# jhuggins/viabel

Hardware: AMD Instinct MI355X
Metric: ELBO-gradient evals/sec (D=1024, N_mc=4096) (higher is better)
Workload: dtype f64

## Files before the change

include/viabel_hip.h:

```cpp
#ifndef VIABEL_HIP_H
#define VIABEL_HIP_H

#include <stddef.h>
#include <stdint.h>

#ifdef __cplusplus
extern "C" {
#endif

typedef struct vb_ctx vb_ctx;

#define VB_OK 0
#define VB_ERR_INVALID 1
#define VB_ERR_HIP 2
#define VB_ERR_UNSUPPORTED 3
#define VB_ERR_STATE 4
#define VB_ERR_NUMERIC 5
#define VB_ERR_COMM 6
#define VB_ERR_CALLBACK 7

#define VB_FAMILY_MF_GAUSSIAN 0
#define VB_FAMILY_MF_STUDENT_T 1
#define VB_FAMILY_FULLRANK_GAUSSIAN 2
#define VB_FAMILY_MULTIVARIATE_T 3
#define VB_FAMILY_LOWRANK_GAUSSIAN 4

#define VB_MODEL_GAUSS_DIAG 0
#define VB_MODEL_FUNNEL 1
#define VB_MODEL_GAUSS_FULL 2
#define VB_MODEL_LOGISTIC 3

#define VB_MODEL_SOURCE 4
#define VB_MODEL_SOFTMAX 5
#define VB_MODEL_MULTILEVEL 6
#define VB_MODEL_LOCSCALE 7
#define VB_MODEL_SPARSE_GLM 8
#define VB_MODEL_MINIBATCH_GLM 9
#define VB_MODEL_NEURALNET 10
#define VB_LOCSCALE_GAUSSIAN 0
#define VB_LOCSCALE_STUDENT_T 1

#define VB_GLM_BERNOULLI_LOGIT 0
#define VB_GLM_POISSON 1
#define VB_GLM_GAUSSIAN 2

#define VB_NOISE_NORMAL 0
#define VB_NOISE_STUDENT_T 1

#define VB_FLAG_PATH_DERIV 1u
#define VB_CV_NONE 0
#define VB_CV_FULL 1
#define VB_CV_MEAN_ONLY 2
#define VB_CV_LOO_DIAG 3
#define VB_CV_LOO_DIRECT 4

#define VB_MAX_SLOTS 64

const char* vb_version(void);
int vb_device_count(int* count);
int vb_create(int device_id, vb_ctx** out);
int vb_destroy(vb_ctx* ctx);
const char* vb_last_error(vb_ctx* ctx);
int vb_device_info(vb_ctx* ctx, char* name, size_t name_len, int* n_cu, uint64_t* hbm_bytes);
int vb_sync(vb_ctx* ctx);

int vb_noise_set_host(vb_ctx* ctx, int slot, const double* host, int64_t n, int64_t d);
int vb_noise_generate(vb_ctx* ctx, int slot, int kind, double df, uint64_t seed,
                      uint64_t stream, int64_t row_offset, int64_t n, int64_t d);
int vb_noise_get_host(vb_ctx* ctx, int slot, double* host, int64_t n, int64_t d);
int vb_noise_moments(vb_ctx* ctx, int slot, int64_t n, int64_t d, double* colsum, double* gram);

int vb_chisq_generate(vb_ctx* ctx, double df, uint64_t seed, uint64_t stream, int64_t row_offset, int64_t n);
int vb_chisq_get_host(vb_ctx* ctx, double* host, int64_t n);
int vb_noise_hint_seed(vb_ctx* ctx, uint64_t slot_mask , int with_chi, uint64_t seed);
int vb_noise_ahead_stats(vb_ctx* ctx, uint64_t* generated, uint64_t* adopted);

int vb_set_model(vb_ctx* ctx, int model_id, int64_t dim, const double* dparams,
                 size_t n_dparams, const int64_t* iparams, size_t n_iparams);
int vb_set_model_source(vb_ctx* ctx, int64_t dim, const char* source, const double* params, size_t n_params);
typedef int (*vb_model_callback)(void* user, const double* z, int64_t n, int64_t d, double* f, double* grad);
int vb_set_model_callback(vb_ctx* ctx, int64_t dim, vb_model_callback fn, void* user);
int vb_model_logp(vb_ctx* ctx, const double* x_host, int64_t n, int64_t d, double* out_host);
int vb_model_grad(vb_ctx* ctx, const double* x_host, int64_t n, int64_t d, double* f_host, double* g_host);

int vb_elbo_grad_meanfield(vb_ctx* ctx, int slot, int64_t n, int64_t d, int64_t n_total,
                           int family, double df, const double* theta, unsigned flags,
                           int cv_mode, double* value, double* grad);
int vb_elbo_grad_meanfield_philox(vb_ctx* ctx, int slot, int64_t n, int64_t d, int64_t n_total, int64_t row_offset,
                                  int family, double df, const double* theta, unsigned flags, int cv_mode,
                                  uint64_t seed, uint64_t stream, double* value, double* grad);
int vb_elbo_grad_meanfield_async(vb_ctx* ctx, int slot, int64_t n, int64_t d, int64_t n_total,
                                 int family, double df, const double* theta, unsigned flags,
                                 int cv_mode, int rslot);
int vb_elbo_grad_meanfield_batch_async(vb_ctx* ctx, int count, const int* slots, int64_t n, int64_t d,
                                       int64_t n_total, int family, double df, const double* thetas,
                                       unsigned flags, int cv_mode, const int* rslots);
int vb_result_get(vb_ctx* ctx, int rslot, double* value, double* grad, int64_t p);

int vb_alpha_grad_meanfield(vb_ctx* ctx, int slot, int64_t n, int64_t d, int64_t n_total, int family, double df,
                            const double* theta, double alpha, double* value, double* grad);

#define VB_PRIOR_DIAG_GAUSSIAN 0
#define VB_PRIOR_DIAG_STUDENT_T 1
#define VB_PRIOR_DENSE 2
int vb_dis_set_temper_prior(vb_ctx* ctx, int kind, int64_t d, double df, const double* loc, const double* scale,
                            double log_det_l);
int vb_dis_refresh_meanfield(vb_ctx* ctx, int slot, int64_t n, int64_t d, int64_t n_total, int family, double df,
                             const double* theta, const double* prior_theta, double eps_prev,
                             double ess_target, int max_bisection_its, double* eps, double* ess,
                             double* w, double* log_p, double* log_q);
int vb_dis_grad_meanfield(vb_ctx* ctx, int slot, int64_t n, int64_t d, int family, double df,
                          const double* theta, const double* weights, double scale, double* value,
                          double* grad);

int vb_alpha_grad_fullrank(vb_ctx* ctx, int slot, int64_t n, int64_t d, int64_t n_total, const double* theta,
                           double alpha, double* value, double* grad);
int vb_alpha_grad_mvt_chol(vb_ctx* ctx, int slot, int64_t n, int64_t d, int64_t n_total, double df, const double* theta,
                           double alpha, double* value, double* grad);

int vb_dis_refresh_mvt(vb_ctx* ctx, int slot, int64_t n, int64_t d, int64_t n_total, double df, const double* theta,
                       const double* chi, const double* sqrt_sigma, const double* l_inv,
                       const double* prior_theta, double eps_prev, double ess_target, int max_bisection_its,
                       double* eps, double* ess, double* w, double* log_p, double* log_q);
int vb_elbo_grad_mvt_symroot(vb_ctx* ctx, int slot, int64_t n, int64_t d, int64_t n_total, double df, const double* theta,
                             double* value, double* grad, double* info);
int vb_elbo_grad_mvt_symroot_path(vb_ctx* ctx, int slot, int64_t n, int64_t d, int64_t n_total, double df,
                                  const double* theta, double* value, double* grad, double* info);
int vb_alpha_grad_mvt_symroot(vb_ctx* ctx, int slot, int64_t n, int64_t d, int64_t n_total, double df, double alpha,
                              const double* theta, double* value, double* grad, double* info);

int vb_dis_refresh_mvt_symroot(vb_ctx* ctx, int slot, int64_t n, int64_t d, int64_t n_total, double df, const double* theta,
                               const double* prior_theta, double eps_prev, double ess_target, int max_bisection_its,
                               double* root_info);
int vb_dis_grad_mvt_packed(vb_ctx* ctx, int64_t n, int64_t d, double df, const double* theta, const double* weights,
                           double scale, double* value, double* grad);
int vb_dis_step_mvt_packed(vb_ctx* ctx, int64_t n, int64_t d, double df, const double* theta, int64_t resample_m,
                           uint64_t seed, uint64_t stream, double scale, double* eps, double* ess,
                           double* khat , double* value, double* grad);
int vb_dis_psis_mvt(vb_ctx* ctx, int64_t n_total, double reff);
int vb_dis_clip_mvt(vb_ctx* ctx, int64_t n_total, double threshold);
int vb_dis_weights_get(vb_ctx* ctx, double* w, int64_t n_total, int resampled );
int vb_dis_scalars_get(vb_ctx* ctx, double out[4]);
int vb_host_alloc(size_t bytes, void** ptr);
int vb_host_free(void* ptr);
int vb_resource_counts(uint64_t out[4]);
int vb_dis_generation(vb_ctx* ctx, int kind, uint64_t* generation);
int vb_dis_state_park(vb_ctx* ctx, int kind, int slot, void** handle);
int vb_dis_state_unpark(vb_ctx* ctx, void* handle);
int vb_dis_state_drop(void* handle);
int vb_dis_state_get(vb_ctx* ctx, int dense, double* log_p, double* log_q, int64_t n_total);
int vb_dis_grad_mvt(vb_ctx* ctx, int64_t n, int64_t d, double df, const double* theta, const double* l_inv,
                    const double* weights, double* w_sum, double* w_logq, double* d_mu, double* gram);

int vb_elbo_grad_lowrank(vb_ctx* ctx, int slot_eps, int slot_z, int64_t n, int64_t d, int64_t k,
                         int64_t n_total, const double* theta, unsigned flags, double* value,
                         double* grad);

int vb_elbo_sums_lowrank(vb_ctx* ctx, int slot_eps, int slot_z, int64_t n, int64_t d, int64_t k, const double* theta,
                         double* out);

typedef struct vb_flow vb_flow;
int vb_flow_create(vb_ctx* ctx, int64_t d, int64_t k, const double* masks, int64_t n_t, const int64_t* widths_t,
                   int64_t n_s, const int64_t* widths_s, vb_flow** out);
int vb_flow_destroy(vb_ctx* ctx, vb_flow* flow);
int vb_flow_param_dim(vb_ctx* ctx, const vb_flow* flow, int64_t* p);
int vb_flow_elbo_grad(vb_ctx* ctx, vb_flow* flow, int slot, int64_t n, int64_t n_total, int prior_family,
                      double prior_df, const double* prior_param, const double* theta, unsigned flags, double* out);
int vb_flow_sample(vb_ctx* ctx, vb_flow* flow, int slot, int64_t n, int prior_family, double prior_df,
                   const double* prior_param, const double* theta, double* x, double* log_q, double* log_p);
int vb_flow_fit(vb_ctx* ctx, vb_flow* flow, int slot, int64_t n, int64_t n_total, int64_t row_offset, int prior_family,
                double prior_df, const double* prior_param, unsigned flags, int noise_kind, double noise_df, uint64_t seed,
                uint64_t first_stream, int opt_kind, const double hyper[4], int64_t n_iters, double* theta, double* state,
                int has_state, double* values, double* history, int64_t hist_len, double* directions, double* gradients);

int vb_log_weights_meanfield(vb_ctx* ctx, int slot, int64_t n, int64_t d, int family, double df,
                             const double* theta, double* lw);
int vb_psis_smooth(vb_ctx* ctx, const double* lw_in, int64_t n, double reff, double* lw_out,
                   double* khat);

int vb_psis_smooth_batch(vb_ctx* ctx, const double* lw, int64_t n, int64_t m, int64_t ld, double reff,
                         double* out, double* khat);
int vb_glm_pointwise(vb_ctx* ctx, const double* x, int64_t s, int64_t d, double* ll_out);
int vb_softmax_pointwise(vb_ctx* ctx, const double* x, int64_t s, int64_t d, double* ll_out);
int vb_multilevel_pointwise(vb_ctx* ctx, const double* x, int64_t s, int64_t d, double* ll_out);
int vb_locscale_pointwise(vb_ctx* ctx, const double* x, int64_t s, int64_t d, double* ll_out);
int vb_sparse_glm_pointwise(vb_ctx* ctx, const double* x, int64_t s, int64_t d, double* ll_out);
int vb_minibatch_pointwise(vb_ctx* ctx, const double* x, int64_t s, int64_t d, double* ll_out);
int vb_minibatch_set_batch(vb_ctx* ctx, int64_t t);
int vb_minibatch_get_batch(vb_ctx* ctx, int64_t* t);
int vb_minibatch_indices(vb_ctx* ctx, int64_t t, int64_t* out);
int vb_glm_psis_loo(vb_ctx* ctx, const double* x, int64_t s, int64_t d, const double* log_ratios,
                    const double* log_w, double reff, double* loo, double* khat, double* lpd);
int vb_glm_predict(vb_ctx* ctx, const double* x, int64_t s, int64_t d, const double* log_w, const double* x_new,
                   int64_t m, const double* y_new, double* mean, double* var, double* eta_mean, double* eta_var,
                   double* lpd);
int vb_nn_pointwise(vb_ctx* ctx, const double* x, int64_t s, int64_t d, double* ll_out);
int vb_nn_predict(vb_ctx* ctx, const double* x, int64_t s, int64_t d, const double* log_w, const double* x_new, int64_t m,
                  const double* y_new, double* mean, double* var, double* eta_mean, double* eta_var, double* lpd);
int vb_glm_value_grad_hessian(vb_ctx* ctx, const double* x, int64_t d, double* f, double* grad, double* hess);

int vb_ksd(vb_ctx* ctx, const double* x, int64_t s, int64_t d, const double* scores, const double* log_w,
           const double* scale, double c, double beta, double* ksd2, double* rowsums);
int vb_ksd_plan(int64_t s, int n_cu, int out[2]);

int vb_svgd_direction(vb_ctx* ctx, const double* x, int64_t n, int64_t d, const double* scores, const double* scale,
                      double bandwidth, double* phi, double* logp, double* h_used);
int vb_svgd_run(vb_ctx* ctx, const double* x0, int64_t n, int64_t d, const double* scale, double bandwidth, int opt_kind,
                const double hyper[4], int64_t n_iters, double* state, int has_state, double* x, double* logp,
                double* h_hist, double* rms_hist, double* logp_hist);

int vb_hmc_run(vb_ctx* ctx, const double* x0, const double* inv_mass, int64_t n_chains, int64_t d, int64_t n_warmup,
               int64_t n_draws, int64_t thin, int n_leapfrog, double step_size, double target_accept, double jitter,
               uint64_t seed, uint64_t stream_offset, double* draws, double* logp, double* last_x, double* chain_mean,
               double* chain_m2, double* accept_rate, double* step_hist, double* accept_hist, double* final_step,
               int64_t* n_divergent);

#define VB_HMC_METRIC_DIAG 0
#define VB_HMC_METRIC_DENSE 1
int vb_hmc_run_metric(vb_ctx* ctx, const double* x0, int metric_kind, const double* metric, int64_t n_chains, int64_t d,
                      int64_t n_warmup, int64_t n_draws, int64_t thin, int n_leapfrog, double step_size, double target_accept,
                      double jitter, uint64_t seed, uint64_t stream_offset, const double* moment_shift, double* moment_sum,
                      double* moment_m2, double* draws, double* logp, double* last_x, double* chain_mean, double* chain_m2,
                      double* accept_rate, double* step_hist, double* accept_hist, double* final_step, int64_t* n_divergent);

int vb_hmc_run_chees(vb_ctx* ctx, const double* x0, int metric_kind, const double* metric, int64_t n_chains, int64_t d,
                     int64_t n_warmup, int64_t n_draws, int64_t thin, int max_leapfrog, double trajectory_lr, double step_size,
                     double target_accept, double jitter, uint64_t seed, uint64_t stream_offset, const double* moment_shift,
                     double* moment_sum, double* moment_m2, double* draws, double* logp, double* last_x, double* chain_mean,
                     double* chain_m2, double* accept_rate, double* step_hist, double* accept_hist, double* final_step,
                     int64_t* n_divergent, double* traj_state, double* traj_hist, int64_t* leap_hist);

int vb_elbo_sums_mvt(vb_ctx* ctx, int slot, int64_t n, int64_t d, int64_t n_total, const double* mu,
                     const double* sqrt_sigma, const double* inv_s, double* f_sum, double* g_sum,
                     double* c_full);

int vb_elbo_grad_fullrank(vb_ctx* ctx, int slot, int64_t n, int64_t d, int64_t n_total,
                          const double* theta, unsigned flags, double* value, double* grad);
int vb_fullrank_set_theta(vb_ctx* ctx, const double* theta, int64_t d);
int vb_elbo_grad_fullrank_enqueue(vb_ctx* ctx, int slot, int64_t n, int64_t d, int64_t n_total,
                                  unsigned flags);
int vb_fullrank_get(vb_ctx* ctx, double* value, double* grad, int64_t p);
int vb_fullrank_fold_get_m(vb_ctx* ctx, double* M_host, int64_t d);
int vb_fold_m_team_plan(int d, int pair, int* out8);

int vb_elbo_grad_mvt_chol(vb_ctx* ctx, int slot, int64_t n, int64_t d, int64_t n_total, double df, const double* theta,
                          double* value, double* grad);

int vb_sym_sqrt(vb_ctx* ctx, const double* a, const double* e, int64_t d, double* root, double* x, double* info);
int vb_sym_sqrt_inv(vb_ctx* ctx, const double* a, const double* e, int64_t d, double* root, double* x, double* info,
                    double* inv_root);

int vb_lowrank_path_terms(vb_ctx* ctx, int slot_eps, int slot_z, int64_t n, int64_t d, int64_t k, int64_t n_total,
                          const double* sw, double* out);

int vb_mvt_path_terms(vb_ctx* ctx, int slot, int64_t n, int64_t d, int64_t n_total, double df, const double* inv_s,
                      double* m_w, double* e_w, double* log1p_sum);

int vb_alpha_sums_mvt(vb_ctx* ctx, int slot, int64_t n, int64_t d, int64_t n_total, double df, double alpha,
                      const double* mu, const double* sqrt_sigma, const double* inv_s, double sum_log_diag,
                      double* value, double* w_sum, double* g_sum, double* c_full);

#define VB_OPT_SGD 0
#define VB_OPT_RMSPROP 1
#define VB_OPT_ADAM 2
#define VB_OPT_ADAGRAD 3
int vb_fit(vb_ctx* ctx, int slot, int slot_aux, int64_t n, int64_t d, int64_t n_total, int64_t row_offset, int family,
           double df, unsigned flags, int cv_mode, int noise_kind, double noise_df, uint64_t seed,
           uint64_t first_stream, int opt_kind, const double hyper[4], int64_t n_iters, double* theta, int64_t p,
           double* state, int has_state, double* values, double* history, int64_t hist_len, double* directions,
           double* gradients);
int vb_fit_history_mean(vb_ctx* ctx, int64_t rows, int64_t p, double* mean);

int vb_chain_open(vb_ctx* ctx, int64_t p, int64_t capacity_rows);
int vb_chain_close(vb_ctx* ctx);
int vb_chain_rows(vb_ctx* ctx, int64_t* rows);
int vb_chain_append(vb_ctx* ctx, const double* rows_host, int64_t n_rows);
int vb_chain_fetch(vb_ctx* ctx, int64_t first_row, int64_t n_rows, double* out);
int vb_chain_mean(vb_ctx* ctx, int64_t w, double* mean);
int vb_chain_rhat(vb_ctx* ctx, const int64_t* windows, int n_windows, double jitter, double* max_rhat, double* rhat);
int vb_chain_ess_mcse(vb_ctx* ctx, int64_t w, double* ess, double* mcse);
int vb_mvt_route_stats(vb_ctx* ctx, uint64_t* epilogue_rows, uint64_t* chain_fetch);

int vb_dis_refresh_lowrank(vb_ctx* ctx, int slot_eps, int slot_z, int64_t n, int64_t d, int64_t k, int64_t n_total,
                           const double* mu, const double* log_sigma, const double* b, const double* m_inv,
                           double log_q_const, const double* prior_theta, double eps_prev, double ess_target,
                           int max_bisection_its, double* eps, double* ess, double* w, double* log_p, double* log_q);
int vb_dis_grad_lowrank(vb_ctx* ctx, int64_t n, int64_t d, int64_t k, const double* mu, const double* log_sigma,
                        const double* b, const double* m_inv, double log_q_const, const double* weights, double* out);
int vb_alpha_sums_lowrank(vb_ctx* ctx, int slot_eps, int slot_z, int64_t n, int64_t d, int64_t k, int64_t n_total,
                          double alpha, const double* mu, const double* log_sigma, const double* b, const double* m_inv,
                          double log_q_const, double* value, double* w_sum, double* out);

#define VB_COMM_ID_BYTES 128
int vb_comm_unique_id(char id[VB_COMM_ID_BYTES]);
int vb_comm_init(vb_ctx* ctx, const char id[VB_COMM_ID_BYTES], int n_ranks, int rank);
int vb_comm_destroy(vb_ctx* ctx);
int vb_comm_info(vb_ctx* ctx, int* n_ranks, int* rank);
#define VB_HOST_SUM 0
#define VB_HOST_MAX 1
typedef int (*vb_host_collective_fn)(void* user, double* buf, size_t count, int op);
int vb_comm_init_host(vb_ctx* ctx, vb_host_collective_fn fn, void* user, int n_ranks, int rank);
#define VB_IPC_HANDLE_BYTES 64
int vb_comm_ipc_window(vb_ctx* ctx, size_t cap_doubles, char handle[VB_IPC_HANDLE_BYTES]);
int vb_comm_init_ipc(vb_ctx* ctx, const char* handles, int n_ranks, int rank);
int vb_comm_check(vb_ctx* ctx);
int vb_comm_allreduce_time(vb_ctx* ctx, size_t count, int warm, int reps, double* us_per_collective);

typedef struct vb_legacy_rng vb_legacy_rng;
int vb_legacy_rng_create(uint32_t seed, vb_legacy_rng** out);
void vb_legacy_rng_destroy(vb_legacy_rng* rng);
int vb_legacy_rng_randn(vb_legacy_rng* rng, double* out, int64_t n, int threads);
int vb_legacy_rng_standard_t(vb_legacy_rng* rng, double df, double* out, int64_t n);
int vb_legacy_rng_chisquare(vb_legacy_rng* rng, double df, double* out, int64_t n);
int vb_legacy_rng_random_sample(vb_legacy_rng* rng, double* out, int64_t n);
int vb_legacy_rng_get_state(const vb_legacy_rng* rng, uint32_t key[624], int* pos, int* has_gauss, double* gauss);
int vb_legacy_rng_set_state(vb_legacy_rng* rng, const uint32_t key[624], int pos, int has_gauss, double gauss);
int vb_legacy_rng_randn_device(vb_ctx* ctx, vb_legacy_rng* rng, int slot, int64_t n_total, int64_t d, int64_t row_begin,
                               int64_t rows);
int vb_legacy_rng_standard_t_device(vb_ctx* ctx, vb_legacy_rng* rng, double df, int slot, int64_t n_total, int64_t d,
                                    int64_t row_begin, int64_t rows);
int vb_legacy_rng_chisquare_device(vb_ctx* ctx, vb_legacy_rng* rng, double df, int64_t n, double* host_out);
int vb_legacy_round_end(vb_ctx* ctx, vb_legacy_rng* rng);
int vb_legacy_ahead_stats(vb_ctx* ctx, uint64_t* launched, uint64_t* adopted, uint64_t* discarded);
int vb_legacy_rng_log_proven(void);
uint64_t vb_legacy_rng_uid(const vb_legacy_rng* rng);

#define VB_PROF_MF_ACCUM 0
#define VB_PROF_FR_SAMPLE_GEMM 1
#define VB_PROF_FR_MODEL_GEMM 2
#define VB_PROF_FR_GRAD_GEMM 3
#define VB_PROF_NUM 4

#define VB_FR_FOLD_MIN_D 1024
#define VB_FR_FOLD_MIN_ROWS_PER_D 3
int vb_profile_enable(vb_ctx* ctx, int on);
int vb_profile_read(vb_ctx* ctx, int64_t* launches, int64_t* evals, double* total_ms, int reset);
int vb_profile_read_kernel(vb_ctx* ctx, int kernel_id, int64_t* launches, int64_t* evals, double* total_ms,
                           int reset);

#ifdef __cplusplus
}
#endif
#endif
```

viabel_amd/csrc/vb_common.h:

```cpp
#pragma once

#include <hip/hip_runtime.h>
#include <hip/hip_ext.h>

#include <cstdarg>
#include <cstdint>
#include <cstdio>
#include <cstring>
#include <functional>
#include <memory>
#include <string>
#include <vector>

#include "../../include/viabel_hip.h"
#include "vb_resource.h"

namespace vb {

constexpr int kWave = 64;
constexpr int kMfThreads = 256;
constexpr int kMfWaves = kMfThreads / kWave;
constexpr int kMfCols = 128;
constexpr int kMfChunk = 16;
constexpr int kMaxBatch = 32;
constexpr int kModelLogQ = 99;

template <int BYTES>
__device__ __forceinline__ void kernarg_warm() {
#if defined(__HIP_DEVICE_COMPILE__)
  typedef const uint32_t __attribute__((address_space(4))) * KernargPtr;
  KernargPtr p = (KernargPtr)__builtin_amdgcn_kernarg_segment_ptr();
  uint32_t t = 0;
#pragma unroll
  for (int off = 0; off < BYTES; off += 64) asm volatile("s_load_dword %0, %1, %2" : "+s"(t) : "s"(p), "s"(off));
  asm volatile("s_waitcnt lgkmcnt(0)" : "+s"(t));
#endif
}

enum ColField { CF_G = 0, CF_GE, CF_E, CF_EE, CF_EK, CF_SC, CF_SCE, CF_NUM };

__host__ __device__ __forceinline__ int64_t partial_index(int64_t rb, int f, int64_t col, int64_t n_rb) {
  return (((col >> 6) * n_rb + rb) * CF_NUM + f) * 64 + (col & 63);
}
enum ScalField { SF_F = 0, SF_W, SF_Q, SF_QE, SF_L1P, SF_EE, SF_FK, SF_GK, SF_GEK, SF_NUM = 12 };
enum KScal { KS_F = 0, KS_Q, KS_QE, KS_L1P, KS_EE, KS_NUM };
enum PScal { PS_W = 0, PS_FK, PS_GK, PS_GEK, PS_NUM };

struct ModelDev {
  int id = -1;
  int dim = 0;
  int k = 0;
  double tau = 1.0;
  double c0 = 0.0;
  const double* p0 = nullptr;
  const double* p1 = nullptr;
  int64_t ldp = 0;
  const double* p2 = nullptr;
  int64_t ldq = 0;
  int64_t n_data = 0;
  int link = 0;
  double aux = 1.0;
  int n_classes = 0;
  int n_feat = 0;
  double f0 = 0.0;
  int n_groups = 0;
  double hyper_sd = 1.0;
  const int* grp_off = nullptr;
  const int* grp_of = nullptr;
  const double* w0 = nullptr;
  const double* w1 = nullptr;
  int64_t ldw = 0;
  int n_scale = 0;
  int const_scale = 0;
  double scale_sd = 1.0;
  double df = 0.0;
  const double* sp_val[2] = {nullptr, nullptr};
  const int* sp_ptr[2] = {nullptr, nullptr};
  const int* sp_idx[2] = {nullptr, nullptr};
  const int* sp_seg[2] = {nullptr, nullptr};
  const int* sp_split[2] = {nullptr, nullptr};
  int sp_n_seg[2] = {0, 0};
  int sp_n_split[2] = {0, 0};
  int64_t nnz = 0;
  int64_t mb_size = 0;
  int mb_shuffle = 0;
  int mb_half_bits = 0;
  uint64_t mb_seed = 0;
  int n_hidden = 0;
};

__host__ __device__ __forceinline__ bool model_has_rows(int id) {
  return id == VB_MODEL_SOURCE || id == VB_MODEL_SOFTMAX || id == VB_MODEL_MULTILEVEL || id == VB_MODEL_LOCSCALE ||
         id == VB_MODEL_SPARSE_GLM || id == VB_MODEL_MINIBATCH_GLM || id == VB_MODEL_NEURALNET;
}

__device__ __forceinline__ double glm_term(int link, double aux, double y, double eta, double* dl) {
  if (link == VB_GLM_POISSON) {
    const double mu = exp(eta);
    *dl = y - mu;
    return y * eta - mu;
  }
  if (link == VB_GLM_GAUSSIAN) {
    const double r = (y - eta) / (aux * aux);
    *dl = r;
    return -0.5 * r * (y - eta);
  }
  const double t = exp(-fabs(eta));
  const double p = eta >= 0.0 ? 1.0 / (1.0 + t) : t / (1.0 + t);
  *dl = y - p;
  return y * eta - (fmax(eta, 0.0) + log1p(t));
}

__device__ __forceinline__ double glm_predict_term(int link, double aux, double y, double eta, double* mu, double* var) {
  if (link == VB_GLM_POISSON) {
    const double m = exp(eta);
    *mu = m;
    *var = m;
    return y * eta - m;
  }
  if (link == VB_GLM_GAUSSIAN) {
    const double r = (y - eta) / (aux * aux);
    *mu = eta;
    *var = aux * aux;
    return -0.5 * r * (y - eta);
  }
  const double t = exp(-fabs(eta));
  const double q = 1.0 / (1.0 + t);
  *mu = eta >= 0.0 ? q : t * q;
  *var = t * q * q;
  return y * eta - (fmax(eta, 0.0) + log1p(t));
}

struct NoiseReq {
  int kind = 0;
  double df = 0.0;
  uint64_t seed = 0, stream = 0;
  int64_t row_offset = 0, n = 0, d = 0;
  bool valid = false;
};
struct NoiseAhead {
  DeviceBuffer shadow;
  DeviceBuffer shadow_norms;
  bool pre_norms = false;
  int64_t shadow_d = 0, shadow_ld = 0;
  NoiseReq last, pre;
  NoiseReq hint;
  int64_t delta = 0;
  int streak = 0;
};
struct NoiseSlot {
  DeviceBuffer buf;
  int64_t n = 0, d = 0, ld = 0;
  NoiseAhead ahead;
  DeviceBuffer norms;
  NoiseReq norms_req;
  bool want_norms = false;
};
const double* noise_row_norms(vb_ctx* ctx, NoiseSlot& s, hipStream_t st);
int rng_row_norms(vb_ctx* ctx, hipStream_t st, const double* src, int64_t ld, int64_t n, int64_t d, double* norms);

constexpr int kPipeSets = 4;
struct Pipeline {
  Stream post;
  Event ev_k1[kPipeSets], ev_fin[kPipeSets];
  bool fin_valid[kPipeSets] = {};
  uint64_t seq = 0;
  int last_set = 0;
  bool post_pending = false;
};

struct ResultSlot {
  PinnedBuffer pin;
  double* host() const { return pin.host_as<double>(); }
  double* dev() const { return pin.dev_as<double>(); }
  int64_t p = 0;
  bool pending = false;
  uint64_t batch_id = 0;
};

}

namespace vb {
struct LegacySpec;
struct LegacySpecDelete { void operator()(LegacySpec* s) const; };
}

struct vb_ctx {
  int device = 0;
  vb::Stream stream;
  hipDeviceProp_t prop;
  std::string last_error;

  vb::NoiseSlot noise[VB_MAX_SLOTS];
  vb::NoiseSlot gen_geom;
  vb::ResultSlot results[VB_MAX_SLOTS];
  vb::ResultSlot sync_result;
  vb::PinnedBuffer done_pin;
  unsigned long long done_seq = 0;
  int done_groups = 0;

  vb::ModelDev model;
  vb::DeviceBuffer model_params;
  std::vector<double> model_host;

  vb::DeviceBuffer theta;
  vb::DeviceBuffer workspace;
  vb::DeviceBuffer sums;
  vb::DeviceBuffer mf_one;
  unsigned mf_one_epoch = 0;
  vb::DeviceBuffer out;
  vb::DeviceBuffer scratch;
  vb::DeviceBuffer scratch2;
  vb::DeviceBuffer rowvec;
  vb::DeviceBuffer fr_work;
  vb::DeviceBuffer lg_work;
  hipModule_t user_module = nullptr;
  hipFunction_t user_fn = nullptr;
  struct UserModule {
    uint64_t hash;
    hipModule_t module;
    hipFunction_t fn;
    int parts;
  };
  int user_parts = 1;
  vb_model_callback user_host_fn = nullptr;
  void* user_host_arg = nullptr;
  vb::PinnedBuffer user_host_pin;
  std::vector<UserModule> user_modules;
  vb::DeviceBuffer user_params;
  vb::DeviceBuffer glm_work;
  vb::DeviceBuffer target_work;
  int64_t mb_batch = 0, mb_held = -1;
  const void* mb_held_at = nullptr;
  size_t mb_held_bytes = 0;
  vb::DeviceBuffer hess_work;
  vb::DeviceBuffer hmc_work;
  vb::DeviceBuffer mvt_state;
  int64_t mvt_n = 0, mvt_d = 0, mvt_n_total = 0;
  int64_t mvt_lq_off = 0;
  vb::DeviceBuffer mvt_ekl_state;
  std::vector<double> mvt_theta;
  bool mvt_dev_factors = false;
  const double* mvt_e_noise = nullptr;
  int64_t mvt_e_noise_ld = 0;
  std::vector<double> mvt_stage;
  vb::PinnedBuffer mvt_pin;
  size_t mvt_pin_doubles = 0;
  int mvt_pin_slot = 0;
  vb::Event mvt_pin_ev[2];
  vb::PinnedBuffer push_pin;
  size_t push_bytes = 0;
  int push_slot = 0;
  vb::Event push_ev[2];
  vb::PinnedBuffer fetch_pin;
  unsigned long long fetch_seq = 0;
  vb::DeviceBuffer fetch_ticket;
  vb::Stream mvt_side;
  hipEvent_t mvt_ev_fork = nullptr;
  vb::Event mvt_ev_join;
  vb::Event done_ev;
  uint64_t ahead_generated = 0, ahead_adopted = 0;
  bool mvt_inv_pending = false;
  bool mvt_inv_queued = false;
  struct {
    double* base = nullptr;
    int64_t o_theta = 0, o_lt = 0, o_wt = 0, o_tscr = 0, o_mu = 0, o_li = 0, o_lfull = 0, o_c = 0, ld = 0;
    int d = 0;
    bool clean = false;
    bool lfull_here = false;
  } mvt_inv_args;
  std::vector<double> mvt_prior;
  int64_t mvt_inv_key[4] = {0, 0, 0, 0};
  vb::DeviceBuffer dis_state;
  int64_t dis_n = 0, dis_d = 0;
  int64_t dis_n_total = 0;
  vb::DeviceBuffer chi_dev;
  vb::DeviceBuffer mvt_invs;
  vb::NoiseAhead chi_ahead;
  int64_t chi_n = 0;
  double chi_df = 0.0;
  vb::DeviceBuffer bisect_work;
  unsigned long long bisect_bar_base = 0;
  size_t bisect_bar_words = 0;
  void* bisect_bar_ptr = nullptr;
  vb::DeviceBuffer mvt_elbo;
  vb::DeviceBuffer lr_work;
  vb::DeviceBuffer lr_obj;
  std::vector<vb_flow*> flows;
  int64_t lr_n = 0, lr_d = 0, lr_k = 0, lr_n_total = 0;
  struct TemperPrior {
    int kind = 0;
    int64_t d = 0, ld = 0;
    double df = 0.0, c0 = 0.0;
    vb::DeviceBuffer buf;
    vb::DeviceBuffer work;
  } temper;
  uint64_t dis_gen[3] = {0, 0, 0};
  vb::DeviceBuffer rows_work;
  vb::DeviceBuffer psis_lw;
  int64_t psis_n = 0;
  vb::DeviceBuffer psis_work;
  unsigned long long psis_bar_base = 0;
  vb::DeviceBuffer loo_work;
  vb::DeviceBuffer ksd_work;
  vb::DeviceBuffer svgd_work;
  vb::PinnedBuffer pin;
  vb::DeviceBuffer fit_work;
  int64_t fit_out_off = 0;
  uint64_t mvt_epi_rows_calls = 0, mvt_chain_fetch_calls = 0;
  int ns_hint_m[2] = {0, 0}, ns_hint_steps[2] = {0, 0};
  int64_t fit_hist_off = 0, fit_hist_len = 0, fit_hist_p = 0;
  vb::DeviceBuffer chain;
  vb::DeviceBuffer chain_work;
  int64_t chain_p = 0, chain_cap = 0, chain_rows = 0;
  bool chain_open = false;
  static constexpr int kFitRing = 4;
  vb::Stream fit_copy_st;
  vb::PinnedBuffer fit_ring;
  size_t fit_ring_doubles = 0;
  vb::Event fit_ev_step[kFitRing], fit_ev_copy[kFitRing];
  vb::DeviceBuffer tri_map;
  int tri_map_key[3] = {0, 0, 0};
  int tri_map_blocks = 0;
  vb::DeviceBuffer fr_lt;
  int64_t fr_lt_d = 0;
  const double* fr_lt_owner = nullptr;
  vb::DeviceBuffer fr_theta;
  vb::DeviceBuffer fr_out;
  int64_t fr_p = 0;
  const double* fr_fold_m = nullptr;
  int64_t fr_fold_d = 0, fr_fold_ld = 0;
  vb::DeviceBuffer alpha_g;
  vb::DeviceBuffer legacy_work;
  const void* legacy_poly_at = nullptr;
  size_t legacy_poly_bytes = 0;
  bool legacy_table_ready = false;
  std::unique_ptr<vb::LegacySpec, vb::LegacySpecDelete> legacy_spec;
  vb::PinnedBuffer legacy_pin;
  vb::DeviceBuffer fz_words, fz_items;
  int64_t fz_key[5] = {0, 0, 0, 0, 0};
  int fz_n_items = 0;
  unsigned fz_epoch = 0;
  int fr_fused_mode = -1;
  uint64_t fr_seq = 0;

  void* comm = nullptr;
  int n_ranks = 1, rank = 0;
  vb_host_collective_fn host_fn = nullptr;
  void* host_user = nullptr;
  vb::PinnedBuffer host_stage;
  struct IpcComm {
    double* win[16] = {};
    size_t cap = 0;
    unsigned long long seq = 0;
    unsigned* ticket = nullptr;
    unsigned* err_host = nullptr;
    unsigned* err_dev = nullptr;
    int poll_log2 = 32;
    double timeout_s = 20.0;
    bool on = false;
  } ipc;

  bool profile = false;
  struct ProfLog {
    std::vector<std::pair<vb::Event, vb::Event>> events;
    size_t used = 0;
    int64_t evals = 0;
  } prof[VB_PROF_NUM];

  std::vector<vb::Event> batch_events;
  uint64_t batch_id = 0, batch_done = 0;

  vb::Pipeline pipe;
  hipStream_t result_stream = nullptr;
};

namespace vb {

int fail(vb_ctx* ctx, int code, const char* fmt, ...);
int ensure(vb_ctx* ctx, DeviceBuffer& b, size_t bytes);
int ensure_pinned(vb_ctx* ctx, PinnedBuffer& b, size_t bytes, bool mapped);
int ensure_pinned(vb_ctx* ctx, size_t bytes);

#define VB_HIP(ctx, expr)                                                              \
  do {                                                                                 \
    hipError_t e__ = (expr);                                                           \
    if (e__ != hipSuccess)                                                             \
      return vb::fail((ctx), VB_ERR_HIP, "%s failed: %s (%s:%d)", #expr,               \
                      hipGetErrorString(e__), __FILE__, __LINE__);                     \
  } while (0)

#define VB_TRY(expr)                   \
  do {                                 \
    int rc__ = (expr);                 \
    if (rc__ != VB_OK) return rc__;    \
  } while (0)

struct MfCall {
  int count = 0;
  const NoiseSlot* noise[kMaxBatch] = {};
  const double* theta_src[kMaxBatch] = {};
  double* out[kMaxBatch] = {};
  const double* roww[kMaxBatch] = {};
  int64_t n = 0, d = 0, n_total = 0;
  int family = 0;
  double df = 0.0;
  unsigned flags = 0;
  int cv_mode = 0;
  int mode = 0;
  bool overlap_comm = false;
  double scale = 0.0;
  const double* value_src = nullptr;
  const ModelDev* model = nullptr;
  int gen = 0;
  uint64_t gen_seed = 0, gen_stream = 0;
  int64_t gen_row_offset = 0;
  const struct FitStep* step = nullptr;
  bool* step_done = nullptr;
  bool prep_next = false, skip_prep = false;
  bool* prep_done = nullptr;
  bool theta_on_device = false;
  unsigned long long* done_dev = nullptr;
  unsigned long long done_seq = 0;
  int* done_groups = nullptr;
};
int mf_enqueue(vb_ctx* ctx, const MfCall& call);
int user_model_set(vb_ctx* ctx, int64_t dim, const char* source, const double* params, size_t n_params);
int user_rows_enqueue(vb_ctx* ctx, hipStream_t st, const double* Z, int64_t ldz, int64_t n, int d, double* G,
                      int64_t ldg, double* f);
void user_model_release(vb_ctx* ctx);
int softmax_rows_enqueue(vb_ctx* ctx, hipStream_t st, const double* Z, int64_t ldz, int64_t n, int d, double* G,
                         int64_t ldg, double* f);
int model_rows_enqueue(vb_ctx* ctx, hipStream_t st, const double* Z, int64_t ldz, int64_t n, int d, double* G,
                       int64_t ldg, double* f);
constexpr int64_t kSoftmaxChunkDoubles = (int64_t)16 << 20;
int multilevel_rows_enqueue(vb_ctx* ctx, hipStream_t st, const double* Z, int64_t ldz, int64_t n, int d, double* G,
                            int64_t ldg, double* f);
constexpr int64_t kMultilevelChunkDoubles = (int64_t)16 << 20;
int locscale_rows_enqueue(vb_ctx* ctx, hipStream_t st, const double* Z, int64_t ldz, int64_t n, int d, double* G,
                          int64_t ldg, double* f);
constexpr int64_t kLocScaleChunkDoubles = (int64_t)16 << 20;
int sparse_rows_enqueue(vb_ctx* ctx, hipStream_t st, const double* Z, int64_t ldz, int64_t n, int d, double* G, int64_t ldg,
                        double* f);
constexpr int kSparseSegment = 256;
constexpr int64_t kSparseChunkDoubles = (int64_t)16 << 20;
inline int64_t sparse_chunk_rows(int64_t n_data, int64_t p) {
  const int64_t rows = kSparseChunkDoubles / (2 * (n_data + p)) / 64 * 64;
  return rows < 64 ? 64 : rows > 8192 ? 8192 : rows;
}
int minibatch_rows_enqueue(vb_ctx* ctx, hipStream_t st, const double* Z, int64_t ldz, int64_t n, int d, double* G, int64_t ldg,
                           double* f);
constexpr int64_t kMinibatchChunkDoubles = (int64_t)16 << 20;
inline int64_t minibatch_chunk_rows(int64_t batch_size) {
  const int64_t rows = kMinibatchChunkDoubles / (2 * ((batch_size + 15) / 16 * 16));
  return rows < 8 ? 8 : rows;
}
int neuralnet_rows_enqueue(vb_ctx* ctx, hipStream_t st, const double* Z, int64_t ldz, int64_t n, int d, double* G, int64_t ldg,
                           double* f);
constexpr int64_t kNeuralNetChunkDoubles = (int64_t)16 << 20;
constexpr int64_t kNeuralNetPredictDoubles = (int64_t)16 << 20;
struct PredictArgs {
  const double* eta;
  int64_t ld;
  int n;
  const double* w;
  const double* log_w;
  const double* y;
  double aux;
  double *mean, *var, *eta_mean, *eta_var, *lpd;
};
int glm_predict_enqueue(vb_ctx* ctx, hipStream_t st, int link, const PredictArgs& a, int64_t rows);
bool predict_weights(const double* log_w, int64_t s, std::vector<double>& out);
struct RowsPointwisePlan {
  int64_t chunk = 0, total = 0;
  int64_t o_x = 0, o_ll = 0, ldl = 0;
  int64_t width = 0;
};
using RowsPointwiseBody = std::function<int(int64_t rows, const double* X, int64_t ldx, double* LL, int64_t ldl)>;
int rows_pointwise(vb_ctx* ctx, const char* api_name, int model_id, const char* target_name, const double* x, int64_t s,
                   int64_t d, double* ll_out, const std::function<int(RowsPointwisePlan*)>& plan,
                   const RowsPointwiseBody& body);
int upload_model_params(vb_ctx* ctx, const std::vector<double>& dev, const double** base);
using SetModelFn = int(vb_ctx* ctx, int64_t dim, const double* dparams, size_t n_dparams, const int64_t* iparams,
                       size_t n_iparams);
SetModelFn softmax_set_model, multilevel_set_model, locscale_set_model, sparse_set_model, minibatch_set_model,
    neuralnet_set_model;
struct LegacyFinish;
int legacy_dev_randn(vb_ctx* ctx, uint32_t key[624], int* pos, int* has_gauss, double* gauss, double* dst, int64_t ld,
                     int64_t n_total, int64_t d, int64_t row_begin, int64_t rows, LegacyFinish* defer = nullptr);
struct FetchSeg {
  const void* src;
  size_t bytes;
  void* dst;
};
struct LegacyWords {
  const uint32_t* words = nullptr;
  int64_t* scal = nullptr;
  uint32_t* extra = nullptr;
  const void* logtab = nullptr;
  int64_t pre = 0, n_words = 0;
  uint32_t* key_io = nullptr;
  int64_t* meta = nullptr;
};
struct LegacyFinish {
  LegacyWords lw;
  const int64_t* src_dev = nullptr;
  int64_t mult = 0, add = 0;
  const void* extra_src[2] = {nullptr, nullptr};
  int extra_words[2] = {0, 0};
  int kind = 0;
  int64_t pairs = 0, n_vals = 0;
  int pos_in = 0;
};
constexpr int kLegacyFinishWords = 352;
int legacy_finish_launch(vb_ctx* ctx, hipStream_t st, const LegacyFinish& f, unsigned long long* landing_dev, unsigned long long seq);
int legacy_finish_complete(vb_ctx* ctx, const LegacyFinish& f, const unsigned long long* landing, uint32_t key[624], int* pos,
                           int* has_gauss, double* gauss);
// ... 253 lines not shown
```

viabel_amd/csrc/vb_fullrank.hip:

```cpp
#include "vb_gemm_f64.h"
#include "vb_fit.h"

namespace vb {

constexpr double kLog2PiFr = 1.8378770664093454835606594728112;

__device__ __forceinline__ double fr_wave_sum(double x) {
#pragma unroll
  for (int off = 32; off > 0; off >>= 1) x += __shfl_down(x, off, 64);
  return x;
}

__device__ __forceinline__ double fr_block_sum(double x, double* sh) {
  x = fr_wave_sum(x);
  const int lane = threadIdx.x & 63, wave = threadIdx.x >> 6;
  __syncthreads();
  if (lane == 0) sh[wave] = x;
  __syncthreads();
  return (sh[0] + sh[1]) + (sh[2] + sh[3]);
}

__global__ void __launch_bounds__(256) fr_unpack_kernel(const double* __restrict__ theta, int d,
                                                        int64_t ldl, double* __restrict__ Lt,
                                                        double* __restrict__ mu, double* __restrict__ copy = nullptr) {
// ... 136 lines not shown

struct EpiNegateF {
  double* G;
  int64_t ldz;
  const double* Zc;
  double* part;
  __device__ double operator()(int, int row, int col, double acc) const {
    G[(int64_t)row * ldz + col] = -acc;
    return -0.5 * acc * Zc[(int64_t)row * ldz + col];
  }
  __device__ d2v pair(int, int row, int col, double a0, double a1) const {
    const d2v z = *reinterpret_cast<const d2v*>(Zc + (int64_t)row * ldz + col);
    *reinterpret_cast<d2v*>(G + (int64_t)row * ldz + col) = (d2v){-a0, -a1};
    return (d2v){-0.5 * a0 * z.x, -0.5 * a1 * z.y};
  }
};

struct EpiSplitSlabCs {
  double* C;
  int64_t ldc, slab;
  double* colsum;
  int64_t colsum_ld;
  __device__ void operator()(int split, int row, int col, double acc) const {
    C[split * slab + (int64_t)row * ldc + col] = acc;
  }
  __device__ d2v pair(int split, int row, int col, double a0, double a1) const {
    const d2v v = (d2v){a0, a1};
    *reinterpret_cast<d2v*>(C + split * slab + (int64_t)row * ldc + col) = v;
    return v;
  }
};

struct EpiFoldSlabF {
  double* C;
  int64_t ldc, slab;
  const double* b;
  const double* s;
  const double* Lt;
  int64_t ldl;
  double* part;
  __device__ double operator()(int split, int row, int col, double acc) const {
    const double v = split == 0 ? -acc - b[row] * s[col] : -acc;
    C[split * slab + (int64_t)row * ldc + col] = v;
    const double l = Lt[(int64_t)col * ldl + row];
    return col <= row ? l * v : 0.0;
  }
  __device__ d2v pair(int split, int row, int col, double a0, double a1) const {
    d2v v = (d2v){-a0, -a1};
    if (split == 0) {
      const double br = b[row];
      const d2v ss = *reinterpret_cast<const d2v*>(s + col);
      v.x -= br * ss.x, v.y -= br * ss.y;
    }
    *reinterpret_cast<d2v*>(C + split * slab + (int64_t)row * ldc + col) = v;
    const double l0 = Lt[(int64_t)col * ldl + row], l1 = Lt[(int64_t)(col + 1) * ldl + row];
    return (d2v){col <= row ? l0 * v.x : 0.0, col + 1 <= row ? l1 * v.y : 0.0};
  }
};

struct EpiSplitSlab {
  double* C;
  int64_t ldc, slab;
  __device__ void operator()(int split, int row, int col, double acc) const {
    C[split * slab + (int64_t)row * ldc + col] = acc;
  }
  __device__ d2v pair(int split, int row, int col, double a0, double a1) const {
    const d2v v = (d2v){a0, a1};
    *reinterpret_cast<d2v*>(C + split * slab + (int64_t)row * ldc + col) = v;
    return v;
  }
};

}
#include "vb_fullrank_fused.h"
namespace vb {

__global__ void __launch_bounds__(256) fr_funnel_kernel(const double* __restrict__ Z, double* __restrict__ G,
                                                        int64_t ldz, int64_t n, int d, ModelDev m,
                                                        double* __restrict__ fpart, const double* __restrict__ roww) {
  __shared__ double sh[4];
  const int lane = threadIdx.x & 63;
  const int64_t row = (int64_t)blockIdx.x * 4 + (threadIdx.x >> 6);
  double f = 0.0;
  if (row < n) {
    const double* z = Z + row * ldz;
    double* g = G + row * ldz;
    const double v = z[m.k];
    const double w = exp(-2.0 * v);
    const double rw = roww ? roww[row] : 1.0;
    double ss = 0.0;
    for (int c = lane; c < d; c += 64) {
      if (c == m.k) continue;
      const double zc = z[c];
      const double gc = -zc * w;
      g[c] = roww ? gc * rw : gc;
      ss = fma(zc, zc, ss);
    }
    ss = fr_wave_sum(ss);
    if (lane == 0) {
      const double it2 = 1.0 / (m.tau * m.tau), dm1 = (double)(d - 1);
      const double gk = fma(-v, it2, -dm1) + w * ss;
      g[m.k] = roww ? gk * rw : gk;
      f = v * fma(-0.5 * v, it2, -dm1) - 0.5 * w * ss;
    }
  }
  f = fr_block_sum(f, sh);
  if (threadIdx.x == 0) fpart[blockIdx.x] = f;
}

typedef double fr_d2 __attribute__((ext_vector_type(2)));
__global__ void __launch_bounds__(256) fr_colsum_kernel(const double* __restrict__ G,
                                                        const double* __restrict__ Zc, int64_t ldz,
                                                        int64_t n, int d, int fmode,
                                                        const double* __restrict__ ivar,
                                                        double* __restrict__ colpart,
                                                        double* __restrict__ fpart, double scal = 0.0,
                                                        const double* __restrict__ roww = nullptr,
                                                        int square = 0, double* __restrict__ Gscaled = nullptr,
                                                        const double* __restrict__ rs_out = nullptr) {
  __shared__ double sh[4];
  __shared__ fr_d2 cs[4][64];
  const int c = threadIdx.x & 63, q = threadIdx.x >> 6;
  const int col = blockIdx.x * 128 + 2 * c;
  const int64_t r0 = (int64_t)blockIdx.y * 128;
  const int64_t r1 = r0 + 128 < n ? r0 + 128 : n;
  const bool ok0 = col < d, ok1 = col + 1 < d;
  fr_d2 s = (fr_d2){0.0, 0.0};
  double f = 0.0;
  if (ok0) {
    fr_d2 hiv = (fr_d2){0.0, 0.0};
    if (fmode == 1) hiv = (fr_d2){-0.5 / ivar[col], ok1 ? -0.5 / ivar[col + 1] : 0.0};
    for (int64_t rb = r0 + q; rb < r1; rb += 64) {
      fr_d2 g[16], z[16];
      double rw[16], rs[16];
#pragma unroll
      for (int i = 0; i < 16; ++i) {
        const int64_t r = rb + 4 * i < r1 ? rb + 4 * i : r1 - 1;
        g[i] = *reinterpret_cast<const fr_d2*>(G + r * ldz + col);
        z[i] = fmode >= 2 ? *reinterpret_cast<const fr_d2*>(Zc + r * ldz + col) : (fr_d2){0.0, 0.0};
        rw[i] = roww ? roww[r] : 1.0;
        rs[i] = Gscaled ? rs_out[r] : 1.0;
      }
#pragma unroll
      for (int i = 0; i < 16; ++i) {
        const int64_t r = rb + 4 * i;
        const bool in = r < r1;
        if (roww) g[i] *= rw[i];
        if (square) g[i] *= g[i];
        if (!in) g[i] = (fr_d2){0.0, 0.0}, z[i] = (fr_d2){0.0, 0.0};
        if (!ok1) g[i].y = 0.0, z[i].y = 0.0;
        if (Gscaled && in) *reinterpret_cast<fr_d2*>(Gscaled + r * ldz + col) = g[i] * rs[i];
        s += g[i];
        if (fmode == 1) f = fma(hiv.x * g[i].x, g[i].x, fma(hiv.y * g[i].y, g[i].y, f));
        if (fmode == 2) f = fma(0.5 * z[i].x, g[i].x, fma(0.5 * z[i].y, g[i].y, f));
        if (fmode == 3) f = fma(-0.5 * scal * z[i].x, z[i].x, fma(-0.5 * scal * z[i].y, z[i].y, f));
      }
    }
  }
  cs[q][c] = s;
  __syncthreads();
  if (q == 0 && ok0) {
    const fr_d2 tot = (cs[0][c] + cs[1][c]) + (cs[2][c] + cs[3][c]);
    colpart[(int64_t)blockIdx.y * ldz + col] = tot.x;
    if (ok1) colpart[(int64_t)blockIdx.y * ldz + col + 1] = tot.y;
  }
  f = fr_block_sum(f, sh);
  if (threadIdx.x == 0) fpart[(int64_t)blockIdx.y * gridDim.x + blockIdx.x] = f;
}


template <int THREADS>
__device__ __forceinline__ void fr_fold_sum_blocks(const int blk, double* fold_lds, const double* __restrict__ Spart, int gsplits,
                                                   int64_t slab, int d, int64_t ldl, const double* __restrict__ colpart,
                                                   int64_t ldz, const double* __restrict__ P, int64_t ldp,
                                                   const double* __restrict__ mu, const double* __restrict__ mean, int nb_b,
                                                   int nb_s, double* __restrict__ S, double* __restrict__ svec,
                                                   double* __restrict__ b) {
  static_assert(THREADS == 256 || THREADS == 512, "256 workers, with or without a second idle half");
  const bool worker = THREADS == 256 || threadIdx.x < 256;
  if (blk < nb_b) {
    fr_d2(*part)[4] = reinterpret_cast<fr_d2(*)[4]>(fold_lds);
    const int p = threadIdx.x & 3, kg = threadIdx.x >> 2;
    const int col = blk * 8 + 2 * p;
    if (worker) {
      const int colc = col < d ? col : 0;
      const int kper = (d + 63) / 64;
      const int k0 = kg * kper, k1 = k0 + kper < d ? k0 + kper : d;
      fr_d2 bacc = (fr_d2){0.0, 0.0};
      for (int kb = k0; kb < k1; kb += 16) {
        fr_d2 v[16];
        double c[16];
#pragma unroll
        for (int u = 0; u < 16; ++u) {
          const int k = kb + u < k1 ? kb + u : k1 - 1;
          v[u] = *reinterpret_cast<const fr_d2*>(P + (int64_t)k * ldp + colc);
          c[u] = mu[k] - mean[k];
        }
#pragma unroll
        for (int u = 0; u < 16; ++u)
          if (kb + u < k1) bacc += v[u] * c[u];
      }
      part[kg][p] = bacc;
    }
    __syncthreads();
    if (worker && kg == 0) {
      fr_d2 btot = part[0][p];
#pragma unroll 16
      for (int q = 1; q < 64; ++q) btot += part[q][p];
      if (col < d) b[col] = btot.x;
      if (col + 1 < d) b[col + 1] = btot.y;
    }
    return;
  }
  if (blk < nb_b + nb_s) {
    const int k = (blk - nb_b) * 256 + (int)threadIdx.x;
    if (!worker || k >= ldz) return;
    double s = 0.0;
    if (k < d) {
      s = colpart[k];
      for (int z = 1; z < gsplits; ++z) s += colpart[(int64_t)z * ldz + k];
    }
    svec[k] = s;
    return;
  }
  int bi = 0, bj = blk - nb_b - nb_s;
  while (bj > bi) bj -= ++bi;
  double(*tile)[33] = reinterpret_cast<double(*)[33]>(fold_lds);
  const int tx = threadIdx.x & 31, ty = (threadIdx.x >> 5) & 7;
  const int i0 = bi * 32, j0 = bj * 32;
  double v[4];
  if (worker) {
    int64_t idx[4];
#pragma unroll
    for (int q = 0; q < 4; ++q) {
      const int i = i0 + ty + 8 * q, j = j0 + tx;
      idx[q] = (i < d && j <= i) ? (int64_t)i * ldl + j : 0;
      v[q] = 0.0;
    }
    for (int zb = 0; zb < gsplits; zb += 8) {
      double w[8][4];
#pragma unroll
      for (int u = 0; u < 8; ++u)
#pragma unroll
        for (int q = 0; q < 4; ++q) w[u][q] = Spart[(zb + u < gsplits ? zb + u : gsplits - 1) * slab + idx[q]];
#pragma unroll
      for (int u = 0; u < 8; ++u)
        if (zb + u < gsplits) {
#pragma unroll
          for (int q = 0; q < 4; ++q) v[q] = (zb + u == 0) ? w[u][q] : v[q] + w[u][q];
        }
    }
#pragma unroll
    for (int q = 0; q < 4; ++q) tile[ty + 8 * q][tx] = v[q];
  }
  __syncthreads();
  if (!worker) return;
#pragma unroll
  for (int q = 0; q < 4; ++q) {
    const int r = ty + 8 * q;
    if (bi == bj) {
      const int i = i0 + r, j = j0 + tx;
      if (i < d && j < d) S[(int64_t)i * ldl + j] = tx <= r ? v[q] : tile[tx][r];
    } else {
      const int i = i0 + r, j = j0 + tx;
      if (i < d && j < d) S[(int64_t)i * ldl + j] = v[q];
      const int it = j0 + r, jt = i0 + tx;
      if (it < d && jt < d) S[(int64_t)it * ldl + jt] = tile[tx][r];
    }
  }
}

struct FoldMsumNoDep : GemmNoDep {};
struct FoldMsumTeamNoDep : GemmNoDep {};
constexpr int kFoldTeamStages = 2;

#define VB_FOLD_MSUM_PARAMS                                                                                                  \
  const GemmArgs gm, const EpiSplitSlab em, int nb_m, const double *__restrict__ Spart, int gsplits, int64_t slab, int d,     \
      int64_t ldl, const double *__restrict__ colpart, int64_t ldz, const double *__restrict__ P, int64_t ldp,                \
      const double *__restrict__ mu, const double *__restrict__ mean, int nb_b, int nb_s, double *__restrict__ S,             \
      double *__restrict__ svec, double *__restrict__ b
#define VB_FOLD_MSUM_SUM_ARGS Spart, gsplits, slab, d, ldl, colpart, ldz, P, ldp, mu, mean, nb_b, nb_s, S, svec, b

__global__ void __launch_bounds__(256) fr_fold_msum_kernel(VB_FOLD_MSUM_PARAMS) {
  extern __shared__ double fold_lds[];
  if ((int)blockIdx.x < nb_m) {
    gemm_f64_dma_pair_tiles<2, 4, 3, EpiSplitSlab, FoldMsumNoDep>(gm, em, FoldMsumNoDep{}, (int)blockIdx.x, nb_m);
    return;
  }
  fr_fold_sum_blocks<256>((int)blockIdx.x - nb_m, fold_lds, VB_FOLD_MSUM_SUM_ARGS);
}

__global__ void __launch_bounds__(512) fr_fold_msum_team_kernel(VB_FOLD_MSUM_PARAMS) {
  extern __shared__ double fold_lds[];
  if ((int)blockIdx.x < nb_m) {
    gemm_f64_dma_team_pair_tiles<2, 4, kFoldTeamStages, EpiSplitSlab, FoldMsumTeamNoDep>(gm, em, FoldMsumTeamNoDep{},
                                                                                         (int)blockIdx.x);
    return;
  }
  fr_fold_sum_blocks<512>((int)blockIdx.x - nb_m, fold_lds, VB_FOLD_MSUM_SUM_ARGS);
}
#undef VB_FOLD_MSUM_PARAMS
#undef VB_FOLD_MSUM_SUM_ARGS

template <int U>
__device__ __forceinline__ void fr_fold_csg_blocks(const int blk, fr_d2 (*part)[4], const double* __restrict__ colpart,
                                                   int gsplits, int64_t ldz, int d, const double* __restrict__ M,
                                                   const double* __restrict__ b, double n_rows, double* __restrict__ csg) {
  const int p = threadIdx.x & 3, kg = threadIdx.x >> 2;
  const int col = blk * 8 + 2 * p;
  const int colc = col < d ? col : 0;
  const int kper = (d + 63) / 64;
  const int k0 = kg * kper, k1 = k0 + kper < d ? k0 + kper : d;
  fr_d2 acc = (fr_d2){0.0, 0.0};
  for (int kb = k0; kb < k1; kb += U) {
    fr_d2 v[U];
    double c[U];
#pragma unroll
    for (int u = 0; u < U; ++u) {
      const int k = kb + u < k1 ? kb + u : k1 - 1;
      v[u] = *reinterpret_cast<const fr_d2*>(M + (int64_t)k * ldz + colc);
      c[u] = colpart[k];
    }
    for (int z = 1; z < gsplits; ++z)
#pragma unroll
      for (int u = 0; u < U; ++u) c[u] += colpart[(int64_t)z * ldz + (kb + u < k1 ? kb + u : k1 - 1)];
#pragma unroll
    for (int u = 0; u < U; ++u)
      if (kb + u < k1) acc += v[u] * c[u];
  }
  part[kg][p] = acc;
  __syncthreads();
  if (kg == 0) {
    fr_d2 tot = part[0][p];
#pragma unroll 16
    for (int q = 1; q < 64; ++q) tot += part[q][p];
    if (col < d) csg[col] = -tot.x - n_rows * b[col];
    if (col + 1 < d) csg[col + 1] = -tot.y - n_rows * b[col + 1];
  }
}

__global__ void __launch_bounds__(256) fr_fold_csg_kernel(const double* __restrict__ colpart, int gsplits, int64_t ldz, int d,
                                                          const double* __restrict__ M, const double* __restrict__ b,
                                                          double n_rows, double* __restrict__ csg) {
  __shared__ fr_d2 part[64][4];
  fr_fold_csg_blocks<16>((int)blockIdx.x, part, colpart, gsplits, ldz, d, M, b, n_rows, csg);
}

struct FoldCsgNoDep : GemmNoDep {};

__global__ void __launch_bounds__(256, 4) fr_fold_ctile_csg_kernel(const GemmArgs g, const EpiFoldSlabF epi, int gx, int nb_tiles,
                                                                   const double* __restrict__ colpart, int gsplits, int64_t ldz,
                                                                   int d, const double* __restrict__ M,
                                                                   const double* __restrict__ b, double n_rows,
                                                                   double* __restrict__ csg) {
  if ((int)blockIdx.x < nb_tiles) {
    const int bz = (int)blockIdx.x / gx, bx = (int)blockIdx.x - bz * gx;
    gemm_f64_dma_tile<false, 2, 8, 2, EpiFoldSlabF, FoldCsgNoDep>(g, epi, FoldCsgNoDep{}, bx, bz, gx);
    return;
  }
  extern __shared__ double fold_lds[];
  fr_fold_csg_blocks<8>((int)blockIdx.x - nb_tiles, reinterpret_cast<fr_d2(*)[4]>(fold_lds), colpart, gsplits, ldz, d, M, b,
                        n_rows, csg);
}

static int fr_fold_csplits(int d, int n_cu, int max_splits) {
  const GemmArgs sc = gemm_product(nullptr, 0, nullptr, 0, d, d, d, 2);
  const long tiles = gemm_count_blocks(sc, 64, 64);
  int s = d / (16 * kGemmBK);
  if ((long)s * tiles > 4L * n_cu) s = (int)(4L * n_cu / tiles);
  if (s > max_splits) s = max_splits;
  if (s > 16) s = 16;
  return s < 1 ? 1 : s;
}


template <int CHUNK>
__global__ void __launch_bounds__(256) fr_reduce_kernel(const double* __restrict__ Cpart, int splits,
                                                        int64_t slab, int d, int64_t ldl,
                                                        const double* __restrict__ colpart, int n_rb,
                                                        int64_t ldz, const double* __restrict__ fpart,
                                                        int n_fpart, FrSums S, int full,
                                                        const double* __restrict__ wpart, int nb_c) {
  __shared__ double sh[4];
  const int nb_col = (int)((ldz + 255) / 256);
  if ((int)blockIdx.x < nb_c) {
    const int64_t tid = (int64_t)blockIdx.x * 256 + threadIdx.x;
    const int64_t idx = 2 * tid;
    const int64_t nC = (int64_t)d * ldl;
    if (idx >= nC) return;
    const int i = (int)(idx / ldl), j = (int)(idx % ldl);
    fr_d2 s = (fr_d2){0.0, 0.0};
    if (full == 1 || j <= i) {
      for (int k0 = 0; k0 < splits; k0 += CHUNK) {
        fr_d2 v[CHUNK];
#pragma unroll
        for (int u = 0; u < CHUNK; ++u)
          v[u] = *reinterpret_cast<const fr_d2*>(Cpart + (k0 + u < splits ? k0 + u : splits - 1) * slab + idx);
#pragma unroll
        for (int u = 0; u < CHUNK; ++u)
          if (k0 + u < splits) s += v[u];
      }
      if (full != 1 && j + 1 > i) s.y = 0.0;
    }
    if (full == 2) {
      double* C = S.sums + S.off_c;
      if (j < d && j <= i) {
        C[idx] = s.x;
        if (j < i) C[(int64_t)j * ldl + i] = s.x;
      } else if (j >= d) {
        C[idx] = 0.0;
      }
      if (j + 1 < d && j + 1 <= i) {
        C[idx + 1] = s.y;
        if (j + 1 < i) C[(int64_t)(j + 1) * ldl + i] = s.y;
      } else if (j + 1 >= d) {
        C[idx + 1] = 0.0;
      }
    } else {
      *reinterpret_cast<fr_d2*>(S.sums + S.off_c + idx) = s;
    }
    return;
  }
  if ((int)blockIdx.x < nb_c + nb_col) {
    const int64_t tid = (int64_t)((int)blockIdx.x - nb_c) * 256 + threadIdx.x;
    if (tid >= ldz) return;
    double s = 0.0;
    if (tid < d) {
      for (int rb0 = 0; rb0 < n_rb; rb0 += 32) {
        double v[32];
#pragma unroll
        for (int u = 0; u < 32; ++u) v[u] = rb0 + u < n_rb ? colpart[(int64_t)(rb0 + u) * ldz + tid] : 0.0;
#pragma unroll
        for (int u = 0; u < 32; ++u) s += v[u];
      }
    }
    S.sums[S.off_col + tid] = s;
    return;
  }
  double f = 0.0;
  for (int e = threadIdx.x; e < n_fpart; e += 256) f += fpart[e];
  f = fr_block_sum(f, sh);
  if (threadIdx.x == 0) S.sums[0] = f;
  if (wpart) {
    for (int q = 0; q < 2; ++q) {
      double t = 0.0;
      for (int e = threadIdx.x; e < n_rb; e += 256) t += wpart[(int64_t)q * n_rb + e];
      t = fr_block_sum(t, sh);
      if (threadIdx.x == 0) S.sums[1 + q] = t;
    }
  }
}

static void fr_reduce_launch(vb_ctx* ctx, hipStream_t st, const double* Cpart, int splits, int64_t slab, int d, int64_t ldl,
                             const double* colpart, int n_rb, int64_t ldz, const double* fpart, int n_fpart, FrSums S, int full,
                             const double* wpart) {
  const int nb_c = (int)((slab / 2 + 255) / 256), nb_col = (int)((ldz + 255) / 256);
  const dim3 grid((unsigned)(nb_c + nb_col + 1));
  if (splits > 16 && nb_c <= 2 * ctx->prop.multiProcessorCount)
    hipLaunchKernelGGL(fr_reduce_kernel<64>, grid, dim3(256), 0, st, Cpart, splits, slab, d, ldl, colpart, n_rb, ldz, fpart, n_fpart,
                       S, full, wpart, nb_c);
  else
    hipLaunchKernelGGL(fr_reduce_kernel<16>, grid, dim3(256), 0, st, Cpart, splits, slab, d, ldl, colpart, n_rb, ldz, fpart, n_fpart,
                       S, full, wpart, nb_c);
}

template <bool FUSE>
__global__ void __launch_bounds__(256) fr_reduce_packed_kernel(
    const double* __restrict__ Cpart, int splits, int64_t slab, int d, int64_t ldl,
    const double* __restrict__ colpart, int n_rb, int64_t ldz, const double* __restrict__ fpart, int n_fpart,
    FrSums S, const double* __restrict__ theta, double n_local_w, double n_total, double c0,
    double* __restrict__ out, int pd, FrWeighted wm, const double* __restrict__ fold_mu,
    const double* __restrict__ fold_mean) {
  const double ent = pd ? 0.0 : 1.0;
  const bool weighted = wm.scale != 0.0;
  const double wsum = weighted ? wm.wsum[0] : 0.0;
  const int64_t tid = ((int64_t)blockIdx.x - (fold_mu ? 1 : 0)) * 256 + threadIdx.x;
  const int64_t idx = 2 * tid;
  const int64_t nC = (int64_t)d * ldl;
  const double invN = 1.0 / n_total;
  if (tid >= 0 && idx < nC) {
    const int i = (int)(idx / ldl), j = (int)(idx % ldl);
    if (j <= i) {
      fr_d2 s = (fr_d2){0.0, 0.0};
      for (int k0 = 0; k0 < splits; k0 += 16) {
        fr_d2 v[16];
#pragma unroll
        for (int u = 0; u < 16; ++u)
          v[u] = k0 + u < splits ? *reinterpret_cast<const fr_d2*>(Cpart + (k0 + u) * slab + idx) : (fr_d2){0.0, 0.0};
#pragma unroll
        for (int u = 0; u < 16; ++u) s += v[u];
      }
      const int64_t p = (int64_t)i * (i + 1) / 2 + j;
      if (FUSE && weighted) {
        double g0 = s.x;
        if (j == i) g0 = g0 * exp(theta[d + p]) + wsum;
        out[1 + d + p] = wm.scale * g0;
        if (j + 1 <= i) {
          double g1 = s.y;
          if (j + 1 == i) g1 = g1 * exp(theta[d + p + 1]) + wsum;
          out[1 + d + p + 1] = wm.scale * g1;
        }
      } else if (FUSE) {
        double g0 = -s.x * invN;
        if (j == i) g0 = g0 * exp(theta[d + p]) - ent;
        out[1 + d + p] = g0;
        if (j + 1 <= i) {
          double g1 = -s.y * invN;
          if (j + 1 == i) g1 = g1 * exp(theta[d + p + 1]) - ent;
          out[1 + d + p + 1] = g1;
        }
      } else {
        S.sums[S.off_c + p] = s.x;
        if (j + 1 <= i) S.sums[S.off_c + p + 1] = s.y;
      }
    }
  }
  if (tid >= 0 && tid < ldz) {
    double s = 0.0;
    if (tid < d) {
      for (int rb0 = 0; rb0 < n_rb; rb0 += 32) {
        double v[32];
#pragma unroll
        for (int u = 0; u < 32; ++u) v[u] = rb0 + u < n_rb ? colpart[(int64_t)(rb0 + u) * ldz + tid] : 0.0;
#pragma unroll
        for (int u = 0; u < 32; ++u) s += v[u];
      }
    }
    if (FUSE) {
      if (tid < d) out[1 + tid] = weighted ? wm.scale * s : -s * invN;
    } else {
      S.sums[S.off_col + tid] = s;
    }
  }
  if (blockIdx.x == 0) {
    const int tx = threadIdx.x;
    double f = 0.0, t = 0.0;
    for (int e0 = 0; e0 < n_fpart; e0 += 4 * 256) {
      double v[4];
#pragma unroll
      for (int u = 0; u < 4; ++u) {
        const int e = e0 + u * 256 + tx;
        v[u] = e < n_fpart ? fpart[e] : 0.0;
      }
#pragma unroll
      for (int u = 0; u < 4; ++u) f += v[u];
    }
    for (int c0 = 0; c0 < d; c0 += 4 * 256) {
      double dg[4];
#pragma unroll
      for (int u = 0; u < 4; ++u) {
        const int c = c0 + u * 256 + tx, cc = c < d ? c : 0;
        dg[u] = FUSE ? theta[d + (int64_t)cc * (cc + 1) / 2 + cc] : 0.0;
      }
#pragma unroll
      for (int u = 0; u < 4; ++u)
        if (c0 + u * 256 + tx < d) t += dg[u];
    }
    double dot = 0.0;
    if (fold_mu) {
      for (int c0 = 0; c0 < d; c0 += 4 * 256) {
        double s[4] = {0.0, 0.0, 0.0, 0.0}, cc[4];
#pragma unroll
        for (int q = 0; q < 4; ++q) {
          const int c = c0 + q * 256 + tx, cl = c < d ? c : d - 1;
          cc[q] = c < d ? fold_mu[cl] - fold_mean[cl] : 0.0;
        }
        for (int rb0 = 0; rb0 < n_rb; rb0 += 8) {
          double v[4][8];
#pragma unroll
          for (int q = 0; q < 4; ++q) {
            const int c = c0 + q * 256 + tx, cl = c < d ? c : d - 1;
#pragma unroll
            for (int u = 0; u < 8; ++u) v[q][u] = colpart[(int64_t)(rb0 + u < n_rb ? rb0 + u : n_rb - 1) * ldz + cl];
          }
#pragma unroll
          for (int q = 0; q < 4; ++q)
#pragma unroll
            for (int u = 0; u < 8; ++u)
              if (rb0 + u < n_rb) s[q] += v[q][u];
        }
#pragma unroll
        for (int q = 0; q < 4; ++q) dot += cc[q] * s[q];
      }
    }
    __shared__ double sh3[12];
    f = fr_wave_sum(f), t = fr_wave_sum(t), dot = fr_wave_sum(dot);
    if ((tx & 63) == 0) sh3[tx >> 6] = f, sh3[4 + (tx >> 6)] = t, sh3[8 + (tx >> 6)] = dot;
    __syncthreads();
    if (tx == 0) {
      f = (sh3[0] + sh3[1]) + (sh3[2] + sh3[3]);
      if (fold_mu) f = 0.5 * (f + ((sh3[8] + sh3[9]) + (sh3[10] + sh3[11])));
      const double sum_logdiag = (sh3[4] + sh3[5]) + (sh3[6] + sh3[7]);
      if (FUSE) {
        const double F = f + n_local_w * c0;
        const double half_sq = pd ? 0.5 * S.sums[1] * invN : 0.5 * d;
        const double H = half_sq + 0.5 * d * kLog2PiFr + sum_logdiag;
        out[0] = weighted ? wm.value[0] : -(F * invN + H);
      } else {
        S.sums[0] = f;
      }
    }
  }
}

__global__ void __launch_bounds__(256) fr_epilogue_packed_kernel(FrSums S, const double* __restrict__ theta,
                                                                 int d, double n_local_w, double n_total,
                                                                 double c0, double* __restrict__ out, int pd,
                                                                 FrWeighted wm) {
  __shared__ double sh[4];
  const int64_t np = (int64_t)d * (d + 1) / 2;
  const double invN = 1.0 / n_total;
  for (int64_t p = (int64_t)blockIdx.x * 256 + threadIdx.x; p < np; p += (int64_t)gridDim.x * 256) {
    int i = (int)((sqrt(8.0 * (double)p + 1.0) - 1.0) * 0.5);
    while ((int64_t)(i + 1) * (i + 2) / 2 <= p) ++i;
    while ((int64_t)i * (i + 1) / 2 > p) --i;
    const bool diag = p == (int64_t)i * (i + 1) / 2 + i;
    if (wm.scale != 0.0) {
      double g = S.sums[S.off_c + p];
      if (diag) g = g * exp(theta[d + p]) + wm.wsum[0];
      out[1 + d + p] = wm.scale * g;
    } else {
      double g = -S.sums[S.off_c + p] * invN;
      if (diag) g = g * exp(theta[d + p]) - (pd ? 0.0 : 1.0);
      out[1 + d + p] = g;
    }
  }
  for (int64_t p = (int64_t)blockIdx.x * 256 + threadIdx.x; p < d; p += (int64_t)gridDim.x * 256)
    out[1 + p] = wm.scale != 0.0 ? wm.scale * S.sums[S.off_col + p] : -S.sums[S.off_col + p] * invN;
  if (blockIdx.x == 0) {
    double t = 0.0;
    for (int i = threadIdx.x; i < d; i += 256) t += theta[d + (int64_t)i * (i + 1) / 2 + i];
    const double sum_logdiag = fr_block_sum(t, sh);
    if (threadIdx.x == 0) {
      const double F = S.sums[0] + n_local_w * c0;
      const double half_sq = pd ? 0.5 * S.sums[1] * invN : 0.5 * d;
      const double H = half_sq + 0.5 * d * kLog2PiFr + sum_logdiag;
      out[0] = wm.scale != 0.0 ? wm.value[0] : -(F * invN + H);
    }
  }
}

__global__ void __launch_bounds__(256) fr_rowscale_kernel(double* __restrict__ G, int64_t ldz, int64_t n, int d,
                                                          const double* __restrict__ rs) {
  const int64_t row = blockIdx.x;
  const int c = blockIdx.y * 256 + threadIdx.x;
  if (c < d) G[row * ldz + c] *= rs[row];
}

struct EpiStoreD {
  double* C;
  int64_t ld;
  double sign;
  int64_t batch_c;
  __device__ void operator()(int z, int row, int col, double acc) const {
    C[z * batch_c + (int64_t)row * ld + col] = sign * acc;
  }
};

constexpr int kTriLeaf = 128;
__device__ __forceinline__ double fr_readlane(double v, int l) {
  const int lo = __builtin_amdgcn_readlane(__double2loint(v), l);
  const int hi = __builtin_amdgcn_readlane(__double2hiint(v), l);
  return __hiloint2double(hi, lo);
}
__global__ void __launch_bounds__(256) fr_triinv_leaf_kernel(const double* __restrict__ theta,
                                                             const double* __restrict__ U, int d, int64_t ld,
                                                             double* __restrict__ X) {
  extern __shared__ double ls[];
  const int lane = threadIdx.x & 63;
  const int c0 = blockIdx.x * 4;
  const int s = c0 / kTriLeaf * kTriLeaf;
  const int jmax = (c0 + 3 < d ? c0 + 3 : d - 1) - s;
  const int total = (jmax + 1) * kTriLeaf;
  for (int e0 = threadIdx.x; e0 < total; e0 += 256 * 16) {
    double v[16];
#pragma unroll
    for (int k = 0; k < 16; ++k) {
      const int e = e0 + 256 * k < total ? e0 + 256 * k : total - 1;
      const int i = e / kTriLeaf, r = e % kTriLeaf;
      const int64_t gi = s + i;
      v[k] = theta[d + gi * (gi + 1) / 2 + s + (r < i ? r : 0)];
    }
#pragma unroll
    for (int k = 0; k < 16; ++k) {
      const int e = e0 + 256 * k;
      if (e < total) ls[e] = (e % kTriLeaf) < (e / kTriLeaf) ? v[k] : 0.0;
    }
  }
  __syncthreads();
  const int c = __builtin_amdgcn_readfirstlane(c0 + (threadIdx.x >> 6));
  if (c >= d) return;
  const int j = c - s;
  double p0 = 0.0, p1 = 0.0, x0 = 0.0, x1 = 0.0;
  double q0 = 1.0, q1 = 1.0;
  if (lane <= j) q0 = 1.0 / U[(int64_t)(s + lane) * ld + s + lane];
  if (lane + 64 <= j) q1 = 1.0 / U[(int64_t)(s + lane + 64) * ld + s + lane + 64];
  int i = j;
  double l0 = ls[i * kTriLeaf + lane], l1 = ls[i * kTriLeaf + lane + 64];
  for (; i >= 64; --i) {
    const int in = i > 0 ? i - 1 : 0;
    const double l0n = ls[in * kTriLeaf + lane], l1n = ls[in * kTriLeaf + lane + 64];
    const double xi = ((i == j ? 1.0 : 0.0) - fr_readlane(p1, i - 64)) * fr_readlane(q1, i - 64);
    if (lane + 64 == i) x1 = xi;
    p0 = fma(l0, xi, p0);
    p1 = fma(l1, xi, p1);
    l0 = l0n;
    l1 = l1n;
  }
  for (; i >= 0; --i) {
    const int in = i > 0 ? i - 1 : 0;
    const double l0n = ls[in * kTriLeaf + lane];
    const double xi = ((i == j ? 1.0 : 0.0) - fr_readlane(p0, i)) * fr_readlane(q0, i);
    if (lane == i) x0 = xi;
    p0 = fma(l0, xi, p0);
    l0 = l0n;
  }
  double* Xb = X + (int64_t)s * ld + s;
  if (lane <= j) Xb[(int64_t)lane * ld + j] = x0;
  if (lane + 64 <= j) Xb[(int64_t)(lane + 64) * ld + j] = x1;
}

__global__ void __launch_bounds__(256) fr_transpose_kernel(const double* __restrict__ in, double* __restrict__ out, int d,
                                                           int64_t ld) {
  __shared__ double tile[32][33];
  const int tx = threadIdx.x & 31, ty = threadIdx.x >> 5;
  const int i0 = blockIdx.y * 32, j0 = blockIdx.x * 32;
  for (int r = ty; r < 32; r += 8) {
    const int i = i0 + r, j = j0 + tx;
    tile[r][tx] = (i < d && j < d) ? in[(int64_t)i * ld + j] : 0.0;
  }
  __syncthreads();
  for (int r = ty; r < 32; r += 8) {
    const int j = j0 + r, i = i0 + tx;
    if (i < d && j < d) out[(int64_t)j * ld + i] = tile[tx][r];
  }
}

__global__ void __launch_bounds__(256) fr_sumsq_kernel(const double* __restrict__ E, int64_t ld, int64_t n, int d,
                                                       double* __restrict__ part) {
  __shared__ double sh[4];
  double s = 0.0;
  for (int64_t r = blockIdx.x; r < n; r += gridDim.x) {
    const double* e = E + r * ld;
    for (int c = 2 * threadIdx.x; c < d; c += 512) {
      const fr_d2 v = *reinterpret_cast<const fr_d2*>(e + c);
      s = fma(v.x, v.x, s);
      if (c + 1 < d) s = fma(v.y, v.y, s);
    }
  }
#pragma unroll
  for (int off = 32; off > 0; off >>= 1) s += __shfl_down(s, off, 64);
  if ((threadIdx.x & 63) == 0) sh[threadIdx.x >> 6] = s;
  __syncthreads();
  if (threadIdx.x == 0) part[blockIdx.x] = (sh[0] + sh[1]) + (sh[2] + sh[3]);
}
__global__ void __launch_bounds__(256) fr_sumsq_final_kernel(const double* __restrict__ part, int count,
                                                             double* __restrict__ out) {
  __shared__ double sh[4];
  double s = 0.0;
  for (int i = threadIdx.x; i < count; i += 256) s += part[i];
#pragma unroll
  for (int off = 32; off > 0; off >>= 1) s += __shfl_down(s, off, 64);
  if ((threadIdx.x & 63) == 0) sh[threadIdx.x >> 6] = s;
  __syncthreads();
  if (threadIdx.x == 0) out[0] = (sh[0] + sh[1]) + (sh[2] + sh[3]);
}

int fr_unpack_enqueue(vb_ctx* ctx, hipStream_t st, const double* theta_dev, int D, int64_t ldl, double* Lt, double* mu,
                      double* theta_copy) {
  hipLaunchKernelGGL(fr_unpack_kernel, dim3((unsigned)((D + 31) / 32), (unsigned)((D + 31) / 32)), dim3(256), 0, st,
                     theta_dev, D, ldl, Lt, mu, theta_copy);
  VB_HIP(ctx, hipGetLastError());
  return VB_OK;
}

__global__ void __launch_bounds__(256) fr_step_unpack_kernel(FitStep a, int d, int64_t ldl, double* __restrict__ Lt,
                                                             double* __restrict__ mu) {
  __shared__ double tile[32][33];
  const int tx = threadIdx.x & 31, ty = threadIdx.x >> 5;
  const int k0 = blockIdx.x * 32, j0 = blockIdx.y * 32;
  if (blockIdx.y == 0) {
    const int i = k0 + (int)threadIdx.x;
    if (threadIdx.x < 32 && i < d) {
      double s1, s2, th;
      fit_step_load(a, i, &s1, &s2, &th);
      mu[i] = fit_step_apply_vals(a, i, a.out[1 + i], s1, s2, th);
    }
    if (blockIdx.x == 0 && threadIdx.x == 32) a.values[a.k] = a.out[0];
  }
  if (k0 > j0 + 31) return;
#pragma unroll
  for (int r = ty; r < 32; r += 8) {
    const int j = j0 + r, k = k0 + tx;
    double v = 0.0;
    if (j < d && k <= j) {
      const int64_t p = d + (int64_t)j * (j + 1) / 2 + k;
      double s1, s2, th;
      fit_step_load(a, p, &s1, &s2, &th);
      v = fit_step_apply_vals(a, p, a.out[1 + p], s1, s2, th);
      if (k == j) v = exp(v);
    }
    tile[r][tx] = v;
  }
  __syncthreads();
#pragma unroll
  for (int r = ty; r < 32; r += 8) {
    const int k = k0 + r, j = j0 + tx;
    if (k < d && j < d && k <= j) Lt[(int64_t)k * ldl + j] = tile[tx][r];
  }
}

int fr_step_unpack_enqueue(vb_ctx* ctx, const FitStep& a, int64_t d) {
  const int64_t ldl = round_up(d, 16);
  if (!ctx->fr_lt.ptr || ctx->fr_lt.bytes < (size_t)(ldl + d * ldl) * sizeof(double))
    return fail(ctx, VB_ERR_STATE, "no unpacked parameter buffer (the first evaluation makes it)");
  double* mu = (double*)ctx->fr_lt.ptr;
  hipLaunchKernelGGL(fr_step_unpack_kernel, dim3((unsigned)((d + 31) / 32), (unsigned)((d + 31) / 32)), dim3(256), 0,
                     ctx->stream, a, (int)d, ldl, mu + ldl, mu);
  VB_HIP(ctx, hipGetLastError());
  ctx->fr_lt_owner = a.theta;
  ctx->fr_lt_d = d;
  return VB_OK;
}

int fr_tri_inverse_enqueue(vb_ctx* ctx, hipStream_t st, const double* theta_dev, const double* Lt, int D, int64_t ldl,
                           double* Xa, double* T, bool clean) {
  const int n_cu = ctx->prop.multiProcessorCount;
  const int64_t slab = (int64_t)D * ldl;
  if (!clean) {
    VB_HIP(ctx, hipMemsetAsync(Xa, 0, (size_t)slab * sizeof(double), st));
    VB_HIP(ctx, hipMemsetAsync(T, 0, (size_t)slab * sizeof(double), st));
  }
  static const hipError_t leaf_attr = hipFuncSetAttribute(
      reinterpret_cast<const void*>(fr_triinv_leaf_kernel), hipFuncAttributeMaxDynamicSharedMemorySize,
      kTriLeaf * kTriLeaf * (int)sizeof(double));
  VB_HIP(ctx, leaf_attr);
  hipLaunchKernelGGL(fr_triinv_leaf_kernel, dim3((unsigned)((D + 3) / 4)), dim3(256),
                     kTriLeaf * kTriLeaf * sizeof(double), st, theta_dev, Lt, D, ldl, Xa);
  VB_HIP(ctx, hipGetLastError());
  GemmArgs gn;
  gn.lda = ldl;
  gn.ldb = ldl;
  gn.tri_mode = 0;
  for (int b = kTriLeaf; b < D; b *= 2) {
    const int full = D / (2 * b);
    const int64_t pair_stride = (int64_t)2 * b * ldl + 2 * b;
    for (int pass = 0; pass < 2; ++pass) {
      const int s0 = pass == 0 ? 0 : full * 2 * b;
      const int count = pass == 0 ? full : (s0 + b < D ? 1 : 0);
      if (count == 0) continue;
      const int b2 = pass == 0 ? b : D - s0 - b;
      const int64_t oa = (int64_t)s0 * ldl + s0, ob = (int64_t)s0 * ldl + s0 + b,
                    oc = (int64_t)(s0 + b) * ldl + s0 + b;
      gn.batch = 1;
      gn.batch_a = pair_stride;
      gn.batch_b = pair_stride;
      gn.A = Lt + ob;
      gn.B = Xa + oc;
      gn.M = b;
      gn.N = b2;
      gn.K = b2;
      gemm_f64_launch<true>(st, gn, count, n_cu, EpiStoreD{T + ob, ldl, 1.0, pair_stride});
      gn.A = Xa + oa;
      gn.B = T + ob;
      gn.K = b;
      gemm_f64_launch<true>(st, gn, count, n_cu, EpiStoreD{Xa + ob, ldl, -1.0, pair_stride});
    }
  }
  VB_HIP(ctx, hipGetLastError());
  return VB_OK;
}

int fr_colsum_enqueue(vb_ctx* ctx, const double* G, const double* Zc, int64_t ldz, int64_t n, int d, int fmode,
                      const double* ivar, double* colpart, double* fpart, const double* roww, int square) {
  const int n_rb = (int)((n + 127) / 128);
  hipLaunchKernelGGL(fr_colsum_kernel, dim3((unsigned)((d + 127) / 128), (unsigned)n_rb), dim3(256), 0, ctx->stream,
                     G, Zc, ldz, n, d, fmode, ivar, colpart, fpart, 0.0, roww, square);
  VB_HIP(ctx, hipGetLastError());
  return VB_OK;
}

int fr_reduce_enqueue(vb_ctx* ctx, const double* Cpart, int splits, int64_t slab, int d, int64_t ldl,
                      const double* colpart, int n_rb, int64_t ldz, const double* fpart, int n_fpart, FrSums S, bool mirror,
                      const double* wpart) {
  fr_reduce_launch(ctx, ctx->stream, Cpart, splits, slab, d, ldl, colpart, n_rb, ldz, fpart, n_fpart, S, mirror ? 2 : 0, wpart);
  VB_HIP(ctx, hipGetLastError());
  return VB_OK;
}

int gram_lower_enqueue(vb_ctx* ctx, const double* A, const double* B, int64_t ld, int d, int64_t n, int splits,
                       double* Cpart, int64_t ldc, int64_t slab) {
  GemmArgs g3 = gemm_product(A, ld, B, ld, d, d, (int)n, 2);
  const char* xcd_env = getenv("VB_GRAM_XCD");
  g3.xcd_group = xcd_env ? atoi(xcd_env) : 1;
  gemm_f64_launch<false>(ctx->stream, g3, splits, ctx->prop.multiProcessorCount, EpiSplitSlab{Cpart, ldc, slab});
  VB_HIP(ctx, hipGetLastError());
  return VB_OK;
}

int gram_lower_colsum_enqueue(vb_ctx* ctx, const double* A, const double* B, int64_t ld, int d, int64_t n, int splits,
                              double* Cpart, int64_t ldc, int64_t slab, double* colsum, int64_t colsum_ld,
                              int colsum_rows, bool* fused) {
  const GemmArgs g3 = gemm_product(A, ld, B, ld, d, d, (int)n, 2);
  *fused = n % kGemmBK == 0 && gemm_uses_dma(g3) && splits <= colsum_rows;
  if (*fused)
    gemm_f64_launch<false>(ctx->stream, g3, splits, ctx->prop.multiProcessorCount,
                           EpiSplitSlabCs{Cpart, ldc, slab, colsum, colsum_ld});
  else
    gemm_f64_launch<false>(ctx->stream, g3, splits, ctx->prop.multiProcessorCount, EpiSplitSlab{Cpart, ldc, slab});
  VB_HIP(ctx, hipGetLastError());
  return VB_OK;
}

int noise_moments(vb_ctx* ctx, const NoiseSlot& ns, int64_t n, int64_t d, double* colsum_host, double* gram_host) {
  if (n <= 0 || n > ns.n || d != ns.d) return fail(ctx, VB_ERR_INVALID, "noise slot shape mismatch");
  const int D = (int)d;
  const int64_t ld = ns.ld, ldl = round_up(d, 16), slab = d * ldl;
  const int n_rb = (int)((n + 127) / 128), cs_gx = (D + 127) / 128;
  const int splits = gram_host ? gram_splits(ctx, D, n) : 0;
  int64_t off = 0;
  auto carve = [&off](int64_t doubles) {
    const int64_t o = off;
    off += round_up(doubles, 16);
    return o;
  };
  const int64_t o_col = carve((int64_t)n_rb * ld), o_f = carve((int64_t)n_rb * cs_gx), o_cpart = carve((int64_t)splits * slab),
                o_sums = carve(16 + ld + slab);
  VB_TRY(ensure(ctx, ctx->scratch, (size_t)off * sizeof(double)));
  double* base = (double*)ctx->scratch.ptr;
  const double* E = (const double*)ns.buf.ptr;
  hipStream_t st = ctx->stream;
  VB_TRY(fr_colsum_enqueue(ctx, E, E, ld, n, D, 0, nullptr, base + o_col, base + o_f, nullptr, 0));
  if (gram_host) VB_TRY(gram_lower_enqueue(ctx, E, E, ld, D, n, splits, base + o_cpart, ldl, slab));
  FrSums S;
  S.sums = base + o_sums;
  S.off_col = 16;
  S.off_c = 16 + ld;
  S.len = 16 + ld + slab;
  VB_TRY(fr_reduce_enqueue(ctx, base + o_cpart, splits, slab, D, ldl, base + o_col, n_rb, ld, base + o_f, 0, S));
  if (ctx->comm) VB_TRY(comm_allreduce_sum(ctx, st, S.sums, (size_t)(gram_host ? S.len : 16 + ld)));
  VB_HIP(ctx, hipMemcpyAsync(colsum_host, S.sums + S.off_col, (size_t)d * sizeof(double), hipMemcpyDeviceToHost, st));
  if (gram_host)
    VB_HIP(ctx, hipMemcpy2DAsync(gram_host, (size_t)d * sizeof(double), S.sums + S.off_c, (size_t)ldl * sizeof(double),
                                 (size_t)d * sizeof(double), (size_t)d, hipMemcpyDeviceToHost, st));
  VB_HIP(ctx, hipStreamSynchronize(st));
  if (gram_host)
    for (int64_t i = 0; i < d; ++i)
      for (int64_t j = i + 1; j < d; ++j) gram_host[i * d + j] = gram_host[j * d + i];
  return VB_OK;
}

int gram_splits(vb_ctx* ctx, int d, int64_t n) {
  const int tiles = gemm_tiles(d, 128);
  const int lower_tiles = tiles * (tiles + 1) / 2;
  int splits = ctx->prop.multiProcessorCount / lower_tiles;
  const int max_splits = (int)(n / 256) > 0 ? (int)(n / 256) : 1;
  if (splits > max_splits) splits = max_splits;
  return splits < 1 ? 1 : splits;
}

static int tri2_tile_map(vb_ctx* ctx, int d, int bm_rows, int bn_cols, const int** map_out, int* blocks_out) {
  if (ctx->tri_map.ptr && ctx->tri_map_key[0] == d && ctx->tri_map_key[1] == bm_rows && ctx->tri_map_key[2] == bn_cols) {
    *map_out = (const int*)ctx->tri_map.ptr;
    *blocks_out = ctx->tri_map_blocks;
    return VB_OK;
  }
  const int tm = gemm_tiles(d, bm_rows), tn = gemm_tiles(d, bn_cols);
  std::vector<std::pair<int, int>> order;
  for (int band = 0; band < tm; band += 2)
    for (int bn = 0; bn < tn; ++bn)
      for (int bm = band; bm < band + 2 && bm < tm; ++bm)
        if (bn * bn_cols <= bm * bm_rows + bm_rows - 1) order.push_back({bm, bn});
  const int total = (int)order.size(), per = (total + 7) / 8, blocks = per * 8;
  std::vector<int> host((size_t)2 * blocks, -1);
  for (int c = 0; c < 8; ++c)
    for (int i = 0; i < per; ++i) {
      const int src = c * per + i;
      if (src >= total) break;
      host[2 * (8 * i + c)] = order[src].first;
      host[2 * (8 * i + c) + 1] = order[src].second;
    }
  VB_TRY(ensure(ctx, ctx->tri_map, host.size() * sizeof(int)));
  VB_HIP(ctx, hipMemcpyAsync(ctx->tri_map.ptr, host.data(), host.size() * sizeof(int), hipMemcpyHostToDevice,
                             ctx->stream));
  VB_HIP(ctx, hipStreamSynchronize(ctx->stream));
  ctx->tri_map_key[0] = d;
  ctx->tri_map_key[1] = bm_rows;
  ctx->tri_map_key[2] = bn_cols;
  ctx->tri_map_blocks = blocks;
  *map_out = (const int*)ctx->tri_map.ptr;
  *blocks_out = blocks;
  return VB_OK;
}

__global__ void __launch_bounds__(256) fr_zsum_kernel(const double* __restrict__ P, int parts, int64_t pslab, int64_t n,
                                                      int d, int64_t ldz, const double* __restrict__ mu,
                                                      const double* __restrict__ shift, double* __restrict__ Z) {
  const int64_t idx = 2 * ((int64_t)blockIdx.x * 256 + threadIdx.x);
  if (idx >= n * ldz) return;
  const int c = (int)(idx % ldz);
  fr_d2 s = (fr_d2){0.0, 0.0};
  for (int k = 0; k < parts; ++k) s += *reinterpret_cast<const fr_d2*>(P + k * pslab + idx);
  if (c < d) s.x += mu[c] - (shift ? shift[c] : 0.0);
  else s.x = 0.0;
  if (c + 1 < d) s.y += mu[c + 1] - (shift ? shift[c + 1] : 0.0);
  else s.y = 0.0;
  *reinterpret_cast<fr_d2*>(Z + idx) = s;
}

__global__ void __launch_bounds__(256) fr_gsum_kernel(const double* __restrict__ P, int parts, int64_t pslab, int64_t n,
                                                      int d, int64_t ldz, const double* __restrict__ Zc,
                                                      double* __restrict__ G, double* __restrict__ fpart) {
  __shared__ double sh[4];
  const int64_t idx = 2 * ((int64_t)blockIdx.x * 256 + threadIdx.x);
  double f = 0.0;
  if (idx < n * ldz) {
    const int c = (int)(idx % ldz);
    fr_d2 s = (fr_d2){0.0, 0.0};
    for (int k = 0; k < parts; ++k) s += *reinterpret_cast<const fr_d2*>(P + k * pslab + idx);
    const fr_d2 z = *reinterpret_cast<const fr_d2*>(Zc + idx);
    if (c >= d) s.x = 0.0;
    if (c + 1 >= d) s.y = 0.0;
    *reinterpret_cast<fr_d2*>(G + idx) = (fr_d2){-s.x, -s.y};
    f = -0.5 * s.x * z.x - 0.5 * s.y * z.y;
  }
  f = fr_wave_sum(f);
  if ((threadIdx.x & 63) == 0) sh[threadIdx.x >> 6] = f;
  __syncthreads();
  if (threadIdx.x == 0) fpart[blockIdx.x] = (sh[0] + sh[1]) + (sh[2] + sh[3]);
}

static int fr_fused_enqueue(vb_ctx* ctx, hipStream_t st, int phases, GemmArgs g1, GemmArgs g2, GemmArgs g3, int splits,
                            double* Z, double* G, int64_t ldz, const double* mu, const double* shift, double* fpart,
                            const EpiSplitSlabCs& e3, unsigned* tiles2_out) {
  const int n_cu = ctx->prop.multiProcessorCount;
  const int n = g1.M, D = g1.N;
  auto fill = [](GemmArgs& g, int splits_) {
    const int ks = gemm_tiles(g.K, splits_);
    g.k_split = gemm_tiles(ks, kGemmBK) * kGemmBK;
    g.tiles_m = gemm_tiles(g.M, 128);
    g.tiles_n = gemm_tiles(g.N, 64);
    g.prio_div = 0;
    g.ev0 = g.ev1 = nullptr;
  };
  fill(g1, 1);
  fill(g2, 1);
  fill(g3, splits);
  const int tm = g1.tiles_m, tn = g1.tiles_n;
  const int n_p1 = tm * tn, n_p2 = tm * tn;
  const int n_p3 = g3.tile_map ? g3.tile_blocks : (int)gemm_count_blocks(g3, 128, 64);
  const size_t words = 16 + 2 * (size_t)tm * tn;
  VB_TRY(ensure(ctx, ctx->fz_words, words * sizeof(unsigned)));
  unsigned* wbase = (unsigned*)ctx->fz_words.ptr;
  const int64_t key[5] = {n, D, splits, phases, n_p3};
  if (memcmp(key, ctx->fz_key, sizeof key) != 0 || !ctx->fz_items.ptr) {
    std::vector<int> host;
    auto push = [&host](int phase, int bx, int bz) {
      host.push_back(phase), host.push_back(bx), host.push_back(bz), host.push_back(0);
    };
    std::vector<int> map;
    if (phases == 3 && g3.tile_map) {
      map.resize((size_t)2 * n_p3);
      VB_HIP(ctx, hipMemcpy(map.data(), g3.tile_map, map.size() * sizeof(int), hipMemcpyDeviceToHost));
    }
    for (int idx = 0; idx < tn; ++idx)
      for (int rb = 0; rb < tm; ++rb) push(0, idx * tm + rb, 0);
    int z_next = 0;
    for (int rb = 0; rb < tm; ++rb) {
      for (int cb = 0; cb < tn; ++cb) push(1, cb * tm + rb, 0);
      while (phases == 3 && z_next < splits) {
        const int64_t last_row = std::min<int64_t>(n, (int64_t)(z_next + 1) * g3.k_split) - 1;
        if (last_row / 128 > rb) break;
        for (int bx = 0; bx < n_p3; ++bx)
          if (map.empty() || map[2 * bx] >= 0) push(2, bx, z_next);
        ++z_next;
      }
    }
    VB_TRY(ensure(ctx, ctx->fz_items, host.size() * sizeof(int)));
    VB_HIP(ctx, hipMemcpyAsync(ctx->fz_items.ptr, host.data(), host.size() * sizeof(int), hipMemcpyHostToDevice, st));
    VB_HIP(ctx, hipStreamSynchronize(st));
    memcpy(ctx->fz_key, key, sizeof key);
    ctx->fz_n_items = (int)(host.size() / 4);
  }
  if (++ctx->fz_epoch == 0) ctx->fz_epoch = 1;
  FzArgs a;
  a.g1 = g1, a.g2 = g2, a.g3 = g3;
  a.e1 = EpiStoreZPub{Z, ldz, mu, shift};
  a.G = G, a.ldz = ldz, a.Zc = Z, a.fpart = fpart;
  a.e3 = e3;
  a.s.head = wbase, a.s.err = wbase + 1, a.s.zflag = wbase + 16, a.s.gflag = wbase + 16 + (size_t)tm * tn;
  a.s.epoch = ctx->fz_epoch, a.s.tiles_n = tn;
  a.items = (const int4*)ctx->fz_items.ptr;
  a.n_items = ctx->fz_n_items, a.n_p1 = n_p1, a.n_p2 = n_p2, a.n_p3 = n_p3;
  a.clk = nullptr;
#ifdef VB_FUSED_CLOCK
  VB_TRY(ensure(ctx, ctx->scratch2, (size_t)4 * a.n_items * sizeof(long long)));
  a.clk = (long long*)ctx->scratch2.ptr;
#endif
  constexpr size_t lds = (size_t)3 * (128 * kGemmBK + kGemmBK * 64) * sizeof(double) + 16;
  static bool configured = false;
  if (!configured) {
    (void)hipFuncSetAttribute(reinterpret_cast<const void*>(&fr_fused_kernel<2>), hipFuncAttributeMaxDynamicSharedMemorySize, (int)lds);
    (void)hipFuncSetAttribute(reinterpret_cast<const void*>(&fr_fused_kernel<3>), hipFuncAttributeMaxDynamicSharedMemorySize, (int)lds);
    configured = true;
  }
  const unsigned grid = (unsigned)(2 * n_cu);
  if (phases == 3) hipLaunchKernelGGL(fr_fused_kernel<3>, dim3(grid), dim3(256), lds, st, a);
  else hipLaunchKernelGGL(fr_fused_kernel<2>, dim3(grid), dim3(256), lds, st, a);
  VB_HIP(ctx, hipGetLastError());
#ifdef VB_FUSED_CLOCK
  if (const char* path = getenv("VB_FUSED_CLOCK_DUMP")) {
    VB_HIP(ctx, hipStreamSynchronize(st));
    std::vector<long long> h((size_t)4 * a.n_items);
    VB_HIP(ctx, hipMemcpy(h.data(), a.clk, h.size() * sizeof(long long), hipMemcpyDeviceToHost));
    if (FILE* f = fopen(path, "wb")) {
      fwrite(h.data(), sizeof(long long), h.size(), f);
      fclose(f);
    }
  }
#endif
  *tiles2_out = (unsigned)n_p2;
  return VB_OK;
}


enum FrDense {
  kDenseNoG,
  kDenseCallerG,
  kDensePersistent,
  kDenseChain
};

struct FrRoute {
  bool mvt = false, pd = false, glm = false, source = false, overlap = false;
  int n_cu = 0;
  int64_t n = 0, d = 0, ldl = 0, ldz = 0, ldr = 0, slab = 0, pslab = 0, np = 0, glm_part = 0;
  int D = 0, n_rb = 0, cs_gx = 0, n_fpart = 0;
  int tri1 = 0, tri3 = 0;
  int splits = 1;
  int kparts = 1;
  unsigned sum_blocks = 0;
  bool fold_shape = false;
  bool fold = false;
  int csplits = 1;
  int cfgc = 0;
  int fz_mode = 0;
  FrDense dense = kDenseChain;
  bool model_ksplit = false;
  bool caller_z = false;
  bool fused_sums = false;
  bool diag_f = false;
  bool cs_only = false;
  bool g_prescaled = false;
  bool scale_rows_w = false;
  bool two_passes = false;
  bool colpass = false;
  bool colpass_keeps_f = false;
  int fmode = 0;
  bool grad_colsums = false;
  bool grad_launch = true;
  int cfg3 = 0;
  bool f_per_tile = false;
};

static FrRoute fr_route(const vb_ctx* ctx, const ModelDev& m, int64_t n, int64_t d, bool mvt, bool pd, bool row_scaled,
                        const FrWeighted& wm) {
  FrRoute r;
  const bool gauss_diag = m.id == VB_MODEL_GAUSS_DIAG, gauss_full = m.id == VB_MODEL_GAUSS_FULL,
             funnel = m.id == VB_MODEL_FUNNEL;
  r.mvt = mvt;
  r.pd = pd;
  r.glm = m.id == VB_MODEL_LOGISTIC;
  r.source = model_has_rows(m.id);
  r.overlap = !mvt && ctx->comm != nullptr;
  r.n_cu = ctx->prop.multiProcessorCount;
  r.n = n;
  r.d = d;
  r.D = (int)d;
  r.ldl = r.ldz = round_up(d, 16);
  r.slab = d * r.ldl;
  r.pslab = n * r.ldz;
  r.np = d * (d + 1) / 2;
  r.tri1 = mvt ? 0 : 1;
  r.tri3 = mvt ? 0 : 2;
  const int D = r.D, n_cu = r.n_cu;
  const GemmArgs s1 = gemm_product(nullptr, 0, nullptr, 0, (int)n, D, D, r.tri1);
  const GemmArgs s3 = gemm_product(nullptr, 0, nullptr, 0, D, D, (int)n, r.tri3);

  const int tiles = gemm_tiles(D, 128);
  const int lower_tiles = mvt ? tiles * tiles : tiles * (tiles + 1) / 2;
  r.splits = n_cu / lower_tiles;
  const int max_splits = (int)(n / 192) > 0 ? (int)(n / 192) : 1;
  if (r.splits > max_splits) r.splits = max_splits;
  if (r.splits < 1) r.splits = 1;
  r.n_rb = (int)((n + 127) / 128);
  r.cs_gx = (D + 127) / 128;
  r.glm_part = r.glm ? gemm_max_blocks(n, m.n_data) : 0;
  r.ldr = r.glm ? round_up(m.n_data, 16) : 0;
  r.n_fpart = funnel ? (int)((n + 3) / 4) : r.source ? (int)n : r.n_rb * r.cs_gx + (int)r.glm_part;

  const bool sums_in_gemms = !mvt && !wm.roww && !row_scaled && n % kGemmBK == 0 && gemm_uses_dma(s1) &&
                             (int64_t)r.splits <= r.n_rb;
  r.fused_sums = gauss_full && sums_in_gemms;
  r.diag_f = gauss_diag && sums_in_gemms;

  if (!row_scaled && !pd && !gauss_diag) {
    const long tiles64 = gemm_count_blocks(s1, 64, 64);
    if (tiles64 < 2L * n_cu && D >= 48 * kGemmBK) r.kparts = (int)((2L * n_cu + tiles64 - 1) / tiles64);
    if (r.kparts > 4) r.kparts = 4;
    while (r.kparts > 1 && (D % (kGemmBK * r.kparts) != 0 || D / r.kparts < 16 * kGemmBK)) --r.kparts;
    if ((int64_t)r.kparts * r.pslab > (int64_t)(r.splits + 1) * r.slab) r.kparts = 1;
  }
  r.sum_blocks = (unsigned)((r.pslab / 2 + 255) / 256);

  r.fold_shape = !mvt && gauss_full && !pd && d >= VB_FR_FOLD_MIN_D && n >= (int64_t)VB_FR_FOLD_MIN_ROWS_PER_D * d;
  r.fold = r.fold_shape && r.fused_sums && r.kparts == 1 && !wm.z_ready && !wm.g_ready && n >= d + 2;

  r.fz_mode = ctx->fr_fused_mode;
  if (r.fz_mode < 0) {
    const char* e = getenv("VB_FR_FUSED");
    r.fz_mode = e ? atoi(e) : 0;
  }
  if (!(r.fused_sums && r.kparts == 1 && n % 128 == 0 && D % 64 == 0 && (int64_t)n * r.ldz * 8 < ((int64_t)1 << 31)))
    r.fz_mode = 0;
  if ((r.fz_mode != 2 && r.fz_mode != 3) || pd || r.fold || wm.g_ready) r.fz_mode = 0;
  r.dense = r.fold ? kDenseNoG : wm.g_ready ? kDenseCallerG : r.fz_mode >= 2 ? kDensePersistent : kDenseChain;
  r.model_ksplit = r.kparts > 1 && r.fused_sums;
  r.caller_z = wm.z_ready != nullptr && (funnel || r.source || r.glm);

  r.g_prescaled = funnel && wm.roww != nullptr;
  r.scale_rows_w = wm.roww != nullptr && !r.g_prescaled;
  r.cs_only = r.diag_f || (!r.fused_sums && !mvt && (funnel || r.source) && (!wm.roww || r.g_prescaled) && !row_scaled &&
                           n % kGemmBK == 0 && gemm_uses_dma(s3) && (int64_t)r.splits <= r.n_rb);
  const bool f_from_pass = !(funnel || r.source);
  r.colpass = !r.fused_sums && !r.cs_only;
  r.two_passes = pd && r.colpass && f_from_pass;
  r.colpass_keeps_f = f_from_pass && !r.two_passes;
  r.fmode = gauss_diag ? 1 : r.glm ? 3 : (gauss_full && !wm.g_ready) ? 2 : 0;

  r.grad_launch = r.fz_mode != 3;
  r.grad_colsums = r.fused_sums || r.cs_only;
  if (r.grad_launch && r.grad_colsums && gemm_count_blocks(s3, 128, 64) * r.splits * 100 >= 190L * n_cu) r.cfg3 = 2;
  r.f_per_tile = r.fused_sums || r.diag_f;
  if (r.fold) {
    r.csplits = fr_fold_csplits(D, n_cu, r.splits + 1);
    const GemmArgs sc = gemm_product(nullptr, 0, nullptr, 0, D, D, D, 2);
    if (gemm_count_blocks(sc, 64, 64) * r.csplits <= 4L * n_cu) r.cfgc = 4;
    else r.cfgc = gemm_count_blocks(sc, 128, 64) * r.csplits * 100 >= 190L * n_cu ? 2 : 3;
  }
  return r;
}

struct FrBufs {
  const double* E = nullptr;
  int64_t lde = 0;
  double *mu = nullptr, *Lt = nullptr;
  double *Z = nullptr, *G = nullptr, *Cpart = nullptr, *colpart = nullptr, *fpart = nullptr;
  double* Rm = nullptr;
  double *Mf = nullptr, *bvec = nullptr;
  double *Sg = nullptr, *svec = nullptr, *csg = nullptr;
  double *Xa = nullptr, *T = nullptr, *sq = nullptr;
  FrSums S;
};

static int fr_carve(vb_ctx* ctx, const FrRoute& r, const NoiseSlot& ns, int set, FrBufs* out) {
  const int64_t n = r.n, ldz = r.ldz, slab = r.slab;
  int64_t off = 0;
  auto carve = [&off](int64_t doubles) {
    const int64_t o = off;
    off += round_up(doubles, 16);
    return o;
  };
  const int64_t o_mu = carve(ldz), o_lt = carve(slab), o_z = carve(n * ldz), o_g = carve(n * ldz),
                o_cpart = carve((int64_t)(r.splits + 1) * slab), o_col = carve((int64_t)(r.n_rb + 1) * ldz),
                o_fpart = carve((int64_t)r.n_fpart + (int64_t)r.n_rb * r.cs_gx + gemm_max_blocks(n, r.D) + (n * ldz) / 512 + 1),
                o_r = carve(r.glm ? n * r.ldr : 0);
  const int64_t o_mf = r.fold_shape ? carve(slab) : 0, o_bvec = r.fold_shape ? carve(ldz) : 0;
  const int64_t o_xa = r.pd ? carve(slab) : 0, o_t = r.pd ? carve(slab) : 0, o_m2 = r.pd ? carve(256) : 0;
  FrBufs b;
  b.S.off_col = 16;
  b.S.off_c = 16 + ldz;
  b.S.len = 16 + ldz + (r.mvt ? slab : round_up(r.np, 16));
  const int64_t o_sums = carve(b.S.len * (r.overlap ? 2 : 1));
  VB_TRY(ensure(ctx, ctx->fr_work, (size_t)off * sizeof(double)));
  double* base = (double*)ctx->fr_work.ptr;
  b.E = (const double*)ns.buf.ptr;
  b.lde = ns.ld;
  b.mu = base + o_mu, b.Lt = base + o_lt, b.Z = base + o_z, b.G = base + o_g, b.Cpart = base + o_cpart;
  b.colpart = base + o_col, b.fpart = base + o_fpart, b.Rm = base + o_r;
  b.Mf = base + o_mf, b.bvec = base + o_bvec;
  if (r.fold) b.Sg = b.G, b.svec = b.G + slab, b.csg = b.G + slab + ldz;
  b.Xa = base + o_xa, b.T = base + o_t, b.sq = base + o_m2;
  b.S.sums = base + o_sums + (int64_t)set * b.S.len;
  *out = b;
  return VB_OK;
}

static int fr_stream_plan(vb_ctx* ctx, const FrRoute& r, int* set) {
  Pipeline& P = ctx->pipe;
  hipStream_t st = ctx->stream;
  *set = 0;
  if (r.overlap) {
    VB_TRY(pipe_init(ctx));
    *set = (int)(ctx->fr_seq++ & 1);
    if (P.fin_valid[*set]) VB_HIP(ctx, hipStreamWaitEvent(st, P.ev_fin[*set], 0));
  } else if (P.post_pending) {
    VB_HIP(ctx, hipStreamWaitEvent(st, P.ev_fin[P.last_set], 0));
    P.post_pending = false;
  }
  return VB_OK;
}

static int fr_prepare_mvt(vb_ctx* ctx, const FrRoute& r, const FrBufs& b, const double* mu_dev, const double* root_dev) {
  hipStream_t st = ctx->stream;
  VB_HIP(ctx, hipMemcpyAsync(b.mu, mu_dev, (size_t)r.d * sizeof(double), hipMemcpyDeviceToDevice, st));
  VB_HIP(ctx, hipMemcpy2DAsync(b.Lt, (size_t)r.ldl * sizeof(double), root_dev, (size_t)r.ldl * sizeof(double),
                               (size_t)r.d * sizeof(double), (size_t)r.d, hipMemcpyDeviceToDevice, st));
  return VB_OK;
}

static int fr_prepare_dense(vb_ctx* ctx, const FrRoute& r, FrBufs* b, const double* theta_dev) {
  const int64_t d = r.d;
  VB_TRY(ensure(ctx, ctx->fr_lt, (size_t)(r.ldz + r.slab) * sizeof(double)));
  b->mu = (double*)ctx->fr_lt.ptr;
  b->Lt = b->mu + r.ldz;
  const bool resident = theta_dev == (const double*)ctx->fr_theta.ptr;
  const bool stepped = ctx->fr_lt_owner != nullptr && ctx->fr_lt_owner == theta_dev;
  const bool lt_cached = (resident || stepped) && ctx->fr_lt_d == d;
  if (!stepped) ctx->fr_lt_owner = nullptr;
  ctx->fr_lt_d = (resident || stepped) ? d : 0;
  if (!lt_cached) {
    hipLaunchKernelGGL(fr_unpack_kernel, dim3((unsigned)((d + 31) / 32), (unsigned)((d + 31) / 32)), dim3(256), 0, ctx->stream,
                       theta_dev, r.D, r.ldl, b->Lt, b->mu);
    VB_HIP(ctx, hipGetLastError());
  }
  return VB_OK;
}

static int fr_score_prologue(vb_ctx* ctx, const FrRoute& r, const FrBufs& b, const double* theta_dev) {
  hipStream_t st = ctx->stream;
  const int D = r.D;
  VB_TRY(fr_tri_inverse_enqueue(ctx, st, theta_dev, b.Lt, D, r.ldl, b.Xa, b.T));
  VB_HIP(ctx, hipGetLastError());
  hipLaunchKernelGGL(fr_transpose_kernel, dim3((unsigned)((D + 31) / 32), (unsigned)((D + 31) / 32)), dim3(256), 0, st,
                     (const double*)b.Xa, b.T, D, r.ldl);
  const int sq_blocks = (int)(r.n < 256 ? r.n : 256);
  hipLaunchKernelGGL(fr_sumsq_kernel, dim3((unsigned)sq_blocks), dim3(256), 0, st, b.E, b.lde, r.n, D, b.sq);
  hipLaunchKernelGGL(fr_sumsq_final_kernel, dim3(1), dim3(256), 0, st, (const double*)b.sq, sq_blocks, b.S.sums + 1);
  VB_HIP(ctx, hipGetLastError());
  return VB_OK;
}

static GemmArgs fr_sample_product(vb_ctx* ctx, const FrRoute& r, const FrBufs& b) {
  GemmArgs g1 = gemm_product(b.E, b.lde, b.Lt, r.ldl, (int)r.n, r.D, r.D, r.tri1);
  prof_events(ctx, &g1.ev0, &g1.ev1, 1, VB_PROF_FR_SAMPLE_GEMM);
  return g1;
}

static const double* fr_sample(vb_ctx* ctx, const FrRoute& r, const FrBufs& b, const double* shift, const double* row_scale,
                               const double* z_ready) {
  if (r.caller_z) return z_ready;
  hipStream_t st = ctx->stream;
  const GemmArgs g1 = fr_sample_product(ctx, r, b);
  if (r.kparts > 1) {
    gemm_f64_launch<true>(st, g1, r.kparts, r.n_cu, EpiSplitSlab{b.Cpart, r.ldz, r.pslab});
    hipLaunchKernelGGL(fr_zsum_kernel, dim3(r.sum_blocks), dim3(256), 0, st, (const double*)b.Cpart, r.kparts, r.pslab, r.n,
                       r.D, r.ldz, (const double*)b.mu, shift, b.Z);
  } else {
    gemm_f64_launch<true>(st, g1, 1, r.n_cu, EpiStoreZ{b.Z, r.ldz, b.mu, shift, row_scale});
  }
  return b.Z;
}

static unsigned fr_model_gauss_diag(vb_ctx* ctx, const FrRoute& r, const FrBufs& b, const ModelDev& m,
                                    const double* row_scale) {
  const GemmArgs g1 = fr_sample_product(ctx, r, b);
  if (r.diag_f)
    return gemm_f64_launch<true>(ctx->stream, g1, 1, r.n_cu, EpiGaussDiagF{b.G, r.ldz, b.mu, m.p0, m.p1, b.fpart});
  gemm_f64_launch<true>(ctx->stream, g1, 1, r.n_cu, EpiGaussDiag{b.G, r.ldz, b.mu, m.p0, m.p1, row_scale});
  return 0;
}

static int fr_model_funnel(vb_ctx* ctx, const FrRoute& r, const FrBufs& b, const ModelDev& m, const double* Z,
                           const double* roww) {
  hipLaunchKernelGGL(fr_funnel_kernel, dim3((unsigned)((r.n + 3) / 4)), dim3(256), 0, ctx->stream, Z, b.G, r.ldz, r.n, r.D, m,
                     b.fpart, roww);
  return VB_OK;
}

static int fr_model_source(vb_ctx* ctx, const FrRoute& r, const FrBufs& b, const double* Z) {
  return model_rows_enqueue(ctx, ctx->stream, Z, r.ldz, r.n, r.D, b.G, r.ldz, b.fpart);
}

static int fr_model_glm(vb_ctx* ctx, const FrRoute& r, const FrBufs& b, const ModelDev& m, const double* Z) {
  hipStream_t st = ctx->stream;
  double* part = b.fpart + (int64_t)r.n_rb * r.cs_gx;
  VB_HIP(ctx, hipMemsetAsync(part, 0, (size_t)r.glm_part * sizeof(double), st));
  const GemmArgs gh = gemm_product(Z, r.ldz, m.p1, m.ldq, (int)r.n, (int)m.n_data, r.D, 0);
  gemm_f64_launch<true>(st, gh, 1, r.n_cu, EpiGlm{b.Rm, r.ldr, m.p2, part, m.link, m.aux});
  VB_HIP(ctx, hipGetLastError());
  return glm_grad_enqueue(ctx, st, m, b.Rm, r.ldr, Z, b.G, r.ldz, r.n, r.D);
}

static int fr_grad_folded(vb_ctx* ctx, const FrRoute& r, const FrBufs& b, const ModelDev& m, unsigned* tiles3) {
  hipStream_t st = ctx->stream;
  const int D = r.D;
  const double* M = b.Mf;
  GemmArgs gs = gemm_product(b.E, b.lde, b.E, b.lde, D, D, (int)r.n, 2);
  prof_events(ctx, &gs.ev0, &gs.ev1, 1, VB_PROF_FR_GRAD_GEMM);
  if (r.cfg3 == 2) VB_TRY(tri2_tile_map(ctx, D, 128, 64, &gs.tile_map, &gs.tile_blocks));
  gemm_f64_launch<false>(st, gs, r.splits, r.n_cu, EpiSplitSlabCs{b.Cpart, r.ldl, r.slab, b.colpart, r.ldz}, r.cfg3);
  VB_HIP(ctx, hipGetLastError());
  GemmArgs gm = gemm_product(b.Lt, r.ldl, m.p1, m.ldp, D, D, D, 4);
  const unsigned nb_team = gemm_f64_team_pair_plan(&gm, r.n_cu);
  const unsigned nb_m = nb_team ? nb_team : gemm_f64_pair_plan(&gm);
  if (nb_m == 0) return fail(ctx, VB_ERR_STATE, "folded evaluation: D = %d does not go to the LDS-DMA product", D);
  const int nb_cs = (D + 7) / 8, nb_s = (int)((r.ldz + 255) / 256), tiles = (D + 31) / 32;
  constexpr size_t pair_lds = gemm_f64_dma_pair_lds<2, 4, 3>(), team_lds = gemm_f64_dma_team_pair_lds<2, 4, kFoldTeamStages>();
  static_assert(pair_lds >= 64 * 4 * sizeof(fr_d2) && pair_lds >= 32 * 33 * sizeof(double) && team_lds >= pair_lds,
                "the sum blocks' LDS is the tiles'");
  static bool configured = false;
  if (!configured) {
    (void)hipFuncSetAttribute(reinterpret_cast<const void*>(&fr_fold_msum_kernel), hipFuncAttributeMaxDynamicSharedMemorySize,
                              (int)pair_lds);
    (void)hipFuncSetAttribute(reinterpret_cast<const void*>(&fr_fold_msum_team_kernel),
                              hipFuncAttributeMaxDynamicSharedMemorySize, (int)team_lds);
    configured = true;
  }
  const dim3 msum_grid(nb_m + (unsigned)(nb_cs + nb_s + tiles * (tiles + 1) / 2));
  const EpiSplitSlab em{b.Mf, r.ldz, r.slab};
  if (nb_team)
    hipLaunchKernelGGL(fr_fold_msum_team_kernel, msum_grid, dim3(512), team_lds, st, gm, em, (int)nb_m, (const double*)b.Cpart,
                       r.splits, r.slab, D, r.ldl, (const double*)b.colpart, r.ldz, m.p1, (int64_t)m.ldp, (const double*)b.mu,
                       m.p0, nb_cs, nb_s, b.Sg, b.svec, b.bvec);
  else
    hipLaunchKernelGGL(fr_fold_msum_kernel, msum_grid, dim3(256), pair_lds, st, gm, em, (int)nb_m, (const double*)b.Cpart,
                       r.splits, r.slab, D, r.ldl, (const double*)b.colpart, r.ldz, m.p1, (int64_t)m.ldp, (const double*)b.mu,
                       m.p0, nb_cs, nb_s, b.Sg, b.svec, b.bvec);
  VB_HIP(ctx, hipGetLastError());
  GemmArgs gc = gemm_product(M, r.ldz, b.Sg, r.ldl, D, D, D, 2);
  const EpiFoldSlabF ec{b.Cpart, r.ldl, r.slab, b.bvec, b.svec, b.Lt, r.ldl, b.fpart};
  if (r.cfgc == 4) {
    const int gx = (int)gemm_f64_tri2_small_plan(&gc, r.csplits, r.n_cu), nb_tiles = gx * r.csplits;
    if (gx == 0) return fail(ctx, VB_ERR_STATE, "folded evaluation: D = %d does not go to the LDS-DMA product", D);
    constexpr size_t lds = (size_t)2 * (64 * kGemmBK + kGemmBK * 64) * sizeof(double);
    static_assert(lds >= 64 * 4 * sizeof(fr_d2), "the colsum(G) blocks' LDS is the tiles'");
    static bool configured_c = false;
    if (!configured_c) {
      (void)hipFuncSetAttribute(reinterpret_cast<const void*>(&fr_fold_ctile_csg_kernel), hipFuncAttributeMaxDynamicSharedMemorySize,
                                (int)lds);
      configured_c = true;
    }
    hipLaunchKernelGGL(fr_fold_ctile_csg_kernel, dim3((unsigned)(nb_tiles + nb_cs)), dim3(256), lds, st, gc, ec, gx, nb_tiles,
                       (const double*)b.colpart, r.splits, r.ldz, D, M, (const double*)b.bvec, (double)r.n, b.csg);
    VB_HIP(ctx, hipGetLastError());
    *tiles3 = (unsigned)gx;
    return VB_OK;
  }
  if (r.cfgc == 2) VB_TRY(tri2_tile_map(ctx, D, 128, 64, &gc.tile_map, &gc.tile_blocks));
  *tiles3 = gemm_f64_launch<false>(st, gc, r.csplits, r.n_cu, ec, r.cfgc);
  VB_HIP(ctx, hipGetLastError());
  hipLaunchKernelGGL(fr_fold_csg_kernel, dim3((unsigned)nb_cs), dim3(256), 0, st, (const double*)b.colpart, r.splits, r.ldz, D, M,
                     (const double*)b.bvec, (double)r.n, b.csg);
  VB_HIP(ctx, hipGetLastError());
  return VB_OK;
}

static int fr_model_gauss_full(vb_ctx* ctx, const FrRoute& r, const FrBufs& b, const ModelDev& m, const double* row_scale,
                               const double* g_ready, double** G, unsigned* tiles2) {
  hipStream_t st = ctx->stream;
  const int D = r.D;
  *G = b.G;
  GemmArgs g2 = gemm_product(b.Z, r.ldz, m.p1, m.ldp, (int)r.n, D, D, 0);
  switch (r.dense) {
    case kDenseNoG:
      return VB_OK;
    case kDenseCallerG:
      *G = const_cast<double*>(g_ready);
      return VB_OK;
    case kDensePersistent: {
      const GemmArgs g1 = gemm_product(b.E, b.lde, b.Lt, r.ldl, (int)r.n, D, D, r.tri1);
      GemmArgs g3f = gemm_product(b.G, r.ldz, b.E, b.lde, D, D, (int)r.n, 2);
      if (r.fz_mode == 3) VB_TRY(tri2_tile_map(ctx, D, 128, 64, &g3f.tile_map, &g3f.tile_blocks));
      return fr_fused_enqueue(ctx, st, r.fz_mode, g1, g2, g3f, r.splits, b.Z, b.G, r.ldz, b.mu, m.p0, b.fpart,
                              EpiSplitSlabCs{b.Cpart, r.ldl, r.slab, b.colpart, r.ldz}, tiles2);
    }
    case kDenseChain:
      break;
  }
  fr_sample(ctx, r, b, m.p0, row_scale, nullptr);
  VB_HIP(ctx, hipGetLastError());
  if (r.model_ksplit) {
    gemm_f64_launch<true>(st, g2, r.kparts, r.n_cu, EpiSplitSlab{b.Cpart, r.ldz, r.pslab});
    hipLaunchKernelGGL(fr_gsum_kernel, dim3(r.sum_blocks), dim3(256), 0, st, (const double*)b.Cpart, r.kparts, r.pslab, r.n, D,
                       r.ldz, (const double*)b.Z, b.G, b.fpart);
    *tiles2 = r.sum_blocks;
    return VB_OK;
  }
  prof_events(ctx, &g2.ev0, &g2.ev1, 1, VB_PROF_FR_MODEL_GEMM);
  if (r.fused_sums) *tiles2 = gemm_f64_launch<true>(st, g2, 1, r.n_cu, EpiNegateF{b.G, r.ldz, b.Z, b.fpart});
  else gemm_f64_launch<true>(st, g2, 1, r.n_cu, EpiNegate{b.G, r.ldz});
  return VB_OK;
}

static int fr_colpass(vb_ctx* ctx, const FrRoute& r, const FrBufs& b, const ModelDev& m, double* G, const double* Z, int fmode,
                      double* fpart, const double* row_scale) {
  hipLaunchKernelGGL(fr_colsum_kernel, dim3((unsigned)r.cs_gx, (unsigned)r.n_rb), dim3(256), 0, ctx->stream, (const double*)G, Z,
                     r.ldz, r.n, r.D, fmode, m.p1, b.colpart, fpart, r.glm ? 1.0 / (m.tau * m.tau) : 0.0,
                     (const double*)nullptr, 0, row_scale ? G : (double*)nullptr, row_scale);
  VB_HIP(ctx, hipGetLastError());
  return VB_OK;
}

static int fr_rowscale(vb_ctx* ctx, const FrRoute& r, double* G, const double* w) {
  hipLaunchKernelGGL(fr_rowscale_kernel, dim3((unsigned)r.n, (unsigned)((r.D + 255) / 256)), dim3(256), 0, ctx->stream, G, r.ldz,
                     r.n, r.D, w);
  VB_HIP(ctx, hipGetLastError());
  return VB_OK;
}

static int fr_score(vb_ctx* ctx, const FrRoute& r, const FrBufs& b, const ModelDev& m, double* G, const double* Z) {
  if (r.two_passes) VB_TRY(fr_colpass(ctx, r, b, m, G, Z, r.fmode, b.fpart, nullptr));
  const GemmArgs gy = gemm_product(b.E, b.lde, b.T, r.ldl, (int)r.n, r.D, r.D, 3);
  gemm_f64_launch<true>(ctx->stream, gy, 1, r.n_cu, EpiAccumulate{G, r.ldz});
  VB_HIP(ctx, hipGetLastError());
  return VB_OK;
}

static int fr_grad_product(vb_ctx* ctx, const FrRoute& r, const FrBufs& b, const ModelDev& m, const double* G,
                           unsigned* tiles3) {
  hipStream_t st = ctx->stream;
  *tiles3 = 0;
  if (r.fold) return fr_grad_folded(ctx, r, b, m, tiles3);
  if (!r.grad_launch) return VB_OK;
  GemmArgs g3 = gemm_product(G, r.ldz, b.E, b.lde, r.D, r.D, (int)r.n, r.tri3);
  prof_events(ctx, &g3.ev0, &g3.ev1, 1, VB_PROF_FR_GRAD_GEMM);
  if (r.cfg3 == 2) VB_TRY(tri2_tile_map(ctx, r.D, 128, 64, &g3.tile_map, &g3.tile_blocks));
  if (r.grad_colsums)
    *tiles3 = gemm_f64_launch<false>(st, g3, r.splits, r.n_cu, EpiSplitSlabCs{b.Cpart, r.ldl, r.slab, b.colpart, r.ldz}, r.cfg3);
  else
    *tiles3 = gemm_f64_launch<false>(st, g3, r.splits, r.n_cu, EpiSplitSlab{b.Cpart, r.ldl, r.slab});
  VB_HIP(ctx, hipGetLastError());
  return VB_OK;
}

static int fr_finish_mvt(vb_ctx* ctx, const FrRoute& r, const FrBufs& b, FrSums* sums_out) {
  fr_reduce_launch(ctx, ctx->stream, (const double*)b.Cpart, r.splits, r.slab, r.D, r.ldl, (const double*)b.colpart, r.n_rb, r.ldz,
                   (const double*)b.fpart, r.n_fpart, b.S, 1, nullptr);
  VB_HIP(ctx, hipGetLastError());
  if (ctx->comm) VB_TRY(comm_allreduce_sum(ctx, ctx->stream, b.S.sums, (size_t)b.S.len));
  *sums_out = b.S;
  return VB_OK;
}

static int fr_finish_dense(vb_ctx* ctx, const FrRoute& r, const FrBufs& b, const ModelDev& m, int set, int n_fpart_red,
                           const double* theta_dev, double* out_dev, int64_t n_total, const FrWeighted& wm) {
  hipStream_t st = ctx->stream;
  const int D = r.D, n_rb_red = r.fold ? 1 : (r.grad_colsums || !r.grad_launch) ? r.splits : r.n_rb;
  const int splits = r.fold ? r.csplits : r.splits;
  const double* colpart = r.fold ? b.csg : b.colpart;
  const int64_t red_items = r.slab / 2 > r.ldz ? r.slab / 2 : r.ldz;
  const dim3 red_grid((unsigned)((red_items + 255) / 256) + (r.fold ? 1u : 0u));
  const double *fold_mu = r.fold ? (const double*)b.mu : nullptr, *fold_m = r.fold ? m.p0 : nullptr;
  if (!ctx->comm) {
    hipLaunchKernelGGL(fr_reduce_packed_kernel<true>, red_grid, dim3(256), 0, st, (const double*)b.Cpart, splits, r.slab, D,
                       r.ldl, colpart, n_rb_red, r.ldz, (const double*)b.fpart, n_fpart_red, b.S, theta_dev,
                       (double)n_total, (double)n_total, m.c0, out_dev, r.pd ? 1 : 0, wm, fold_mu, fold_m);
    VB_HIP(ctx, hipGetLastError());
    return VB_OK;
  }
  hipLaunchKernelGGL(fr_reduce_packed_kernel<false>, red_grid, dim3(256), 0, st, (const double*)b.Cpart, splits, r.slab, D,
                     r.ldl, colpart, n_rb_red, r.ldz, (const double*)b.fpart, n_fpart_red, b.S, theta_dev,
                     (double)n_total, (double)n_total, m.c0, out_dev, r.pd ? 1 : 0, wm, fold_mu, fold_m);
  VB_HIP(ctx, hipGetLastError());
  Pipeline& P = ctx->pipe;
  hipStream_t st_post = st;
  if (r.overlap) {
    VB_HIP(ctx, hipEventRecord(P.ev_k1[set], st));
    st_post = P.post;
    VB_HIP(ctx, hipStreamWaitEvent(st_post, P.ev_k1[set], 0));
  }
  VB_TRY(comm_allreduce_sum(ctx, st_post, b.S.sums, (size_t)b.S.len));
  const int64_t epi_full = (r.np + 255) / 256;
  const unsigned epi_grid = (unsigned)((r.overlap && epi_full > r.n_cu) ? r.n_cu : epi_full);
  hipLaunchKernelGGL(fr_epilogue_packed_kernel, dim3(epi_grid), dim3(256), 0, st_post, b.S, theta_dev, D, (double)n_total,
                     (double)n_total, m.c0, out_dev, r.pd ? 1 : 0, wm);
  VB_HIP(ctx, hipGetLastError());
  if (r.overlap) {
    VB_HIP(ctx, hipEventRecord(P.ev_fin[set], st_post));
    P.fin_valid[set] = true;
    P.post_pending = true;
    P.last_set = set;
  }
  return VB_OK;
}

int fr_pipeline_enqueue(vb_ctx* ctx, const NoiseSlot& ns, int64_t n, int64_t d, int64_t n_total,
                        const double* theta_dev, double* out_dev, const double* mu_dev, const double* root_dev,
                        const double* row_scale, FrSums* sums_out, unsigned flags, const FrWeighted* weighted) {
  const ModelDev& m = ctx->model;
  const bool mvt = theta_dev == nullptr;
  FrWeighted wm;
  wm.roww = nullptr;
  wm.scale = 0.0;
  wm.wsum = wm.value = nullptr;
  if (weighted) {
    if (flags & VB_FLAG_PATH_DERIV)
      return fail(ctx, VB_ERR_UNSUPPORTED, "weighted sums: entropy-form pipeline only");
    wm = *weighted;
  }
  const bool pd = (flags & VB_FLAG_PATH_DERIV) != 0;
  if (pd && mvt) return fail(ctx, VB_ERR_UNSUPPORTED, "path derivative: dense Gaussian family only");
  if (m.id != VB_MODEL_GAUSS_DIAG && m.id != VB_MODEL_FUNNEL && m.id != VB_MODEL_GAUSS_FULL && m.id != VB_MODEL_LOGISTIC &&
      !model_has_rows(m.id))
    return fail(ctx, VB_ERR_UNSUPPORTED, "full-rank path: unsupported model id %d", m.id);
  if (m.dim != d)
    return fail(ctx, VB_ERR_INVALID, "model dimension %d != family dimension %lld", m.dim, (long long)d);
  if (n <= 0 || d <= 0 || n > ns.n || d != ns.d)
    return fail(ctx, VB_ERR_INVALID, "noise slot holds %lld x %lld, evaluation asks %lld x %lld",
                (long long)ns.n, (long long)ns.d, (long long)n, (long long)d);

  const FrRoute r = fr_route(ctx, m, n, d, mvt, pd, row_scale != nullptr, wm);
  int set = 0;
  FrBufs b;
  VB_TRY(fr_stream_plan(ctx, r, &set));
  VB_TRY(fr_carve(ctx, r, ns, set, &b));
  ctx->fr_fold_m = r.fold ? b.Mf : nullptr;
  ctx->fr_fold_d = r.fold ? d : 0, ctx->fr_fold_ld = r.fold ? r.ldz : 0;

  if (mvt) VB_TRY(fr_prepare_mvt(ctx, r, b, mu_dev, root_dev));
  else VB_TRY(fr_prepare_dense(ctx, r, &b, theta_dev));
  if (pd) VB_TRY(fr_score_prologue(ctx, r, b, theta_dev));

  const double* Z = b.Z;
  double* G = b.G;
  unsigned tiles2 = 0, tiles3 = 0;
  if (m.id == VB_MODEL_GAUSS_DIAG) {
    tiles2 = fr_model_gauss_diag(ctx, r, b, m, row_scale);
  } else if (m.id == VB_MODEL_GAUSS_FULL) {
    VB_TRY(fr_model_gauss_full(ctx, r, b, m, row_scale, wm.g_ready, &G, &tiles2));
  } else {
    Z = fr_sample(ctx, r, b, nullptr, row_scale, wm.z_ready);
    VB_HIP(ctx, hipGetLastError());
    if (m.id == VB_MODEL_FUNNEL) VB_TRY(fr_model_funnel(ctx, r, b, m, Z, wm.roww));
    else if (r.source) VB_TRY(fr_model_source(ctx, r, b, Z));
    else VB_TRY(fr_model_glm(ctx, r, b, m, Z));
  }
  VB_HIP(ctx, hipGetLastError());

  if (r.scale_rows_w) VB_TRY(fr_rowscale(ctx, r, G, wm.roww));
  if (pd) VB_TRY(fr_score(ctx, r, b, m, G, Z));
  if (r.colpass)
    VB_TRY(fr_colpass(ctx, r, b, m, G, Z, r.two_passes ? 0 : r.fmode, r.colpass_keeps_f ? b.fpart : b.fpart + r.n_fpart,
                      row_scale));
  else if (row_scale) VB_TRY(fr_rowscale(ctx, r, G, row_scale));
  VB_TRY(fr_grad_product(ctx, r, b, m, G, &tiles3));

  if (mvt) return fr_finish_mvt(ctx, r, b, sums_out);
  const int n_fpart_red = r.fold ? (int)tiles3 * r.csplits : r.f_per_tile ? (int)tiles2 : r.n_fpart;
  return fr_finish_dense(ctx, r, b, m, set, n_fpart_red, theta_dev, out_dev, n_total, wm);
}

int fr_sample_enqueue(vb_ctx* ctx, const NoiseSlot& ns, int64_t n, int64_t d, const double* theta_dev, double* Z,
                      const double* mu_dev, const double* root_dev, const double* row_scale) {
  if (n <= 0 || d <= 0 || n > ns.n || d != ns.d) return fail(ctx, VB_ERR_INVALID, "noise slot shape mismatch");
  const int D = (int)d;
  const int64_t ldl = round_up(d, 16), ldz = ldl;
  hipStream_t st = ctx->stream;
  const double* E = (const double*)ns.buf.ptr;
  const int n_cu = ctx->prop.multiProcessorCount;
  ctx->fr_fold_m = nullptr, ctx->fr_fold_d = ctx->fr_fold_ld = 0;
  if (theta_dev) {
    VB_TRY(ensure(ctx, ctx->fr_work, (size_t)(ldz + d * ldl) * sizeof(double)));
    double* mu = (double*)ctx->fr_work.ptr;
    double* Lt = mu + ldz;
    hipLaunchKernelGGL(fr_unpack_kernel, dim3((unsigned)((d + 31) / 32), (unsigned)((d + 31) / 32)), dim3(256), 0, st, theta_dev, D, ldl,
                       Lt, mu);
    gemm_f64_launch<true>(st, gemm_product(E, ns.ld, Lt, ldl, (int)n, D, D, 1), 1, n_cu, EpiStoreZ{Z, ldz, mu, nullptr, row_scale});
  } else {
    gemm_f64_launch<true>(st, gemm_product(E, ns.ld, root_dev, ldl, (int)n, D, D, 0), 1, n_cu,
                          EpiStoreZ{Z, ldz, mu_dev, nullptr, row_scale});
  }
  VB_HIP(ctx, hipGetLastError());
  return VB_OK;
}

int fr_elbo_grad_enqueue(vb_ctx* ctx, const NoiseSlot& ns, int64_t n, int64_t d, int64_t n_total,
                         const double* theta_dev, double* out_dev, unsigned flags, const FrWeighted* weighted) {
  return fr_pipeline_enqueue(ctx, ns, n, d, n_total, theta_dev, out_dev, nullptr, nullptr, nullptr, nullptr, flags,
                             weighted);
}

}

int vb_fullrank_fold_get_m(vb_ctx* ctx, double* M_host, int64_t d) {
  using namespace vb;
  if (!ctx || !M_host) return fail(ctx, VB_ERR_INVALID, "NULL argument");
  if (!ctx->fr_fold_m || ctx->fr_fold_d != d)
    return fail(ctx, VB_ERR_STATE, "the last full-rank evaluation was no folded one of dimension %lld", (long long)d);
  VB_HIP(ctx, hipSetDevice(ctx->device));
  VB_TRY(main_stream_write(ctx));
  VB_HIP(ctx, hipMemcpy2DAsync(M_host, (size_t)d * sizeof(double), ctx->fr_fold_m, (size_t)ctx->fr_fold_ld * sizeof(double),
                               (size_t)d * sizeof(double), (size_t)d, hipMemcpyDeviceToHost, ctx->stream));
  VB_HIP(ctx, hipStreamSynchronize(ctx->stream));
  return VB_OK;
}

int vb_fold_m_team_plan(int d, int pair, int* out8) {
  using namespace vb;
  if (!out8 || d <= 0 || d % kGemmBK != 0) return VB_ERR_INVALID;
  const int tiles_m = gemm_tiles(d, 64);
  if (pair < 0 || pair >= (tiles_m + 1) / 2) return VB_ERR_INVALID;
  const GemmTeamPlan p = gemm_f64_team_plan(d, d, tiles_m, pair);
  const int out[8] = {p.H, p.n_h, p.n_l, p.cnt0, p.cnt1, p.sw, gemm_f64_team_barriers(p, 0), gemm_f64_team_barriers(p, 1)};
  for (int i = 0; i < 8; ++i) out8[i] = out[i];
  return VB_OK;
}
```

viabel_amd/csrc/vb_gemm_f64_dma.h:

```cpp
#pragma once

namespace vb {

typedef __attribute__((address_space(1))) const void* gemm_gptr;
typedef __attribute__((address_space(3))) void* gemm_lptr;

struct GemmNoDep {
  static constexpr int kAuxA = 0;
  __device__ __forceinline__ void before_slab(int, int, int, bool) const {}
  __device__ __forceinline__ void publish(int, int, int) const {}
};

template <bool A_KCONTIG, int AF, int NB, int STAGES, class Epi, class Dep>
__device__ __forceinline__ void gemm_f64_dma_tile(const GemmArgs& g, const Epi& epi, const Dep& dep, const int bx,
                                                  const int bz, const int gx) {
  constexpr int BM = 32 * AF, BN = 8 * NB;
  constexpr int kStages = STAGES;
  static_assert(STAGES == 2 || STAGES == 3, "two or three LDS stages");
  constexpr int kATile = BM * kGemmBK, kBTile = kGemmBK * BN;
  constexpr int kAUnits = kATile / 128, kBUnits = kBTile / 128;
  constexpr int UPW = (kAUnits + kBUnits) / 4;
  static_assert((kAUnits + kBUnits) % 4 == 0, "units must divide over the 4 waves");
  extern __shared__ double gemm_lds[];
  double* As = gemm_lds;
// ... 381 lines not shown
            epi((int)bz, row, col + q, acc[a][r + q]);
        }
      }
    }
  if constexpr (EpiReduces<Epi>::value) {
#pragma unroll
    for (int off = 32; off > 0; off >>= 1) local += __shfl_down(local, off, 64);
    if (lane == 0) gemm_lds[wave] = local;
    __syncthreads();
    if (t == 0)
      epi.part[(int64_t)bz * gx + bx] = (gemm_lds[0] + gemm_lds[1]) + (gemm_lds[2] + gemm_lds[3]);
  }
  dep.publish(bm, bn, bz);
#ifdef VB_GEMM_CLOCK
  __builtin_amdgcn_s_waitcnt(0);
  if (lane == 0 && bx < 1024) {
    long long* o = vb_gemm_dbg + 8 * (4 * bx + wave);
    o[0] = dbg_t1 - dbg_t0;
    o[1] = dbg_t2 - dbg_t1;
    o[2] = clock64() - dbg_t2;
    o[3] = wall_clock64() - dbg_w0;
    o[4] = dbg_w0;
  }
#endif
}


template <bool A_KCONTIG, int AF, int NB, int STAGES, class Epi>
__global__ void __launch_bounds__(256, AF * NB > 32 ? (STAGES > 2 ? 1 : 2) : (AF * NB > 16 || STAGES > 2 ? 2 : 4))
    gemm_f64_dma_kernel(const GemmArgs g, const Epi epi) {
  int bx = (int)blockIdx.x, bz = (int)blockIdx.z;
  if (g.xcd_group) {
    const unsigned lin = blockIdx.x + gridDim.x * blockIdx.z, slot = lin >> 3;
    bz = (int)((lin & 7) + 8 * (slot / gridDim.x));
    bx = (int)(slot % gridDim.x);
  }
  gemm_f64_dma_tile<A_KCONTIG, AF, NB, STAGES, Epi, GemmNoDep>(g, epi, GemmNoDep{}, bx, bz, (int)gridDim.x);
}

template <bool A_KCONTIG, int AF, int NB, int STAGES, class Epi>
inline void gemm_f64_dma_launch(hipStream_t st, const GemmArgs& g, dim3 grid, const Epi& epi) {
  constexpr size_t lds = (size_t)STAGES * (32 * AF * kGemmBK + kGemmBK * 8 * NB) * sizeof(double);
  static bool configured = false;
  if (!configured) {
    (void)hipFuncSetAttribute(reinterpret_cast<const void*>(&gemm_f64_dma_kernel<A_KCONTIG, AF, NB, STAGES, Epi>),
                              hipFuncAttributeMaxDynamicSharedMemorySize, (int)lds);
    configured = true;
  }
  hipExtLaunchKernelGGL((gemm_f64_dma_kernel<A_KCONTIG, AF, NB, STAGES, Epi>), grid, dim3(256), lds, st, g.ev0, g.ev1,
                        0, g, epi);
}

template <int AF, int NB, int STAGES, class Epi, class Dep>
__device__ __forceinline__ void gemm_f64_dma_pair_tiles(const GemmArgs& g, const Epi& epi, const Dep& dep, const int block,
                                                        const int gx) {
  static_assert(!EpiReduces<Epi>::value && !EpiColsum<Epi>::value && !EpiRowSums<Epi>::value,
                "the epilogue between the passes must leave LDS alone");
  const int pair = block / g.tiles_n, bn = block % g.tiles_n;
  const int mirror = g.tiles_m - 1 - pair;
  const int passes = mirror > pair ? 2 : 1;
#pragma unroll 1
  for (int pass = 0; pass < passes; ++pass) {
    const int bm = pass == 0 ? pair : mirror;
    const int bx = bm * g.tiles_n + bn, bz = 0;
    gemm_f64_dma_tile<true, AF, NB, STAGES, Epi, Dep>(g, epi, dep, bx, bz, gx);
    __asm__ volatile("" ::: "memory");
    __builtin_amdgcn_s_waitcnt(0);
    __asm__ volatile("" ::: "memory");
  }
}

template <int AF, int NB, int STAGES>
constexpr size_t gemm_f64_dma_pair_lds() {
  return (size_t)STAGES * (32 * AF * kGemmBK + kGemmBK * 8 * NB) * sizeof(double);
}

template <int AF, int NB, int STAGES, class Epi, class Dep>
__device__ __forceinline__ void gemm_f64_dma_team_pair_tiles(const GemmArgs& g, const Epi& epi, const Dep&, const int block) {
  static_assert(!EpiReduces<Epi>::value && !EpiColsum<Epi>::value && !EpiRowSums<Epi>::value,
                "the epilogue inside the slab loop must leave LDS alone");
  static_assert(STAGES == 2 || STAGES == 3, "two or three LDS stages per team");
  static_assert(AF == 2, "gemm_f64_team_plan counts the slabs of 64-row blocks");
  static_assert(NB % 2 == 0, "fragments are read in pairs");
  constexpr int BM = 32 * AF, BN = 8 * NB;
  constexpr int kStages = STAGES, kAhead = STAGES - 1;
  constexpr int kATile = BM * kGemmBK, kBTile = kGemmBK * BN;
  constexpr int kAUnits = kATile / 128, kBUnits = kBTile / 128;
  static_assert(kAUnits % 4 == 0 && kBUnits % 4 == 0, "whole rounds of A and of B units over the 4 waves of a team");
  constexpr int UA = kAUnits / 4, UPW = (kAUnits + kBUnits) / 4;
  constexpr int kTeamLds = kStages * (kATile + kBTile);
  constexpr int KS = kGemmBK / 4;
  extern __shared__ double gemm_lds[];
  const int t = threadIdx.x & 255;
  const int lane = t & 63, wave = __builtin_amdgcn_readfirstlane(t >> 6);
  const int team = __builtin_amdgcn_readfirstlane((int)threadIdx.x >> 8);
  double* lds = gemm_lds + team * kTeamLds;
  double* As = lds;
  double* Bs = lds + kStages * kATile;
  const int wm = wave >> 1, wn = wave & 1;

  const int pair = block / g.tiles_n, bn = block % g.tiles_n;
  const GemmTeamPlan pl = gemm_f64_team_plan(g.M, g.K, g.tiles_m, pair);
  const int H = pl.H;
  if (H <= 0) return;
  const int cnt = team == 0 ? pl.cnt0 : pl.cnt1;
  const int sw = team == 0 ? pl.sw : 0;
  const int m0_h = pair * BM, m0_l = (g.tiles_m - 1 - pair) * BM, n0 = bn * BN;
  const int kb_h = (m0_h < g.K ? m0_h : g.K) / kGemmBK, kb_l = m0_l / kGemmBK;

  double acc[AF][NB];
#pragma unroll
  for (int i = 0; i < AF; ++i)
#pragma unroll
    for (int j = 0; j < NB; ++j) acc[i][j] = 0.0;

  const double* src[UPW];
  const int64_t step_b = (int64_t)kGemmBK * g.ldb;
  auto set_sources = [&](int m0, int ks) __attribute__((always_inline)) {
#pragma unroll
    for (int u = 0; u < UPW; ++u) {
      if (u < UA) {
        const int q = u * 4 + wave;
        const int row = q * 8 + (lane >> 3), p = lane & 7;
        const int kp = p ^ ((row >> 1) & 7);
        int m = m0 + row;
        m = m < g.M ? m : g.M - 1;
        src[u] = g.A + (int64_t)m * g.lda + (int64_t)ks * kGemmBK + 2 * kp;
      } else {
        const int qb = (u - UA) * 4 + wave;
        constexpr int PPR = BN / 2, RPU = 64 / PPR > 0 ? 64 / PPR : 1;
        constexpr int UPR = PPR >= 64 ? PPR / 64 : 1;
        const int krow = (PPR >= 64) ? qb / UPR : qb * RPU + lane / PPR;
        const int p = (PPR >= 64) ? (qb % UPR) * 64 + lane : lane % PPR;
        int64_t col = n0 + 2 * p;
        col = col < g.ldb - 1 ? col : g.ldb - 2;
        src[u] = g.B + ((int64_t)ks * kGemmBK + krow) * g.ldb + col;
      }
    }
  };
  if (team == 0) set_sources(sw > 0 ? m0_l : m0_h, sw > 0 ? kb_l : kb_h);
  else set_sources(m0_h, kb_h + (cnt > 0 ? pl.h0 : pl.n_h - 1));
  auto issue = [&](int st) __attribute__((always_inline)) {
#pragma unroll
    for (int u = 0; u < UPW; ++u) {
      if (u < UA) {
        double* dst = lds + (u * 4 + wave) * 128 + st * kATile;
        __builtin_amdgcn_global_load_lds((gemm_gptr)src[u], (gemm_lptr)dst, 16, 0, Dep::kAuxA);
      } else {
        double* dst = lds + kStages * kATile + ((u - UA) * 4 + wave) * 128 + st * kBTile;
        __builtin_amdgcn_global_load_lds((gemm_gptr)src[u], (gemm_lptr)dst, 16, 0, 0);
      }
    }
  };
  auto advance_to = [&](int next) __attribute__((always_inline)) {
    if (sw > 0 && next == sw) {
      set_sources(m0_h, kb_h);
    } else {
#pragma unroll
      for (int u = 0; u < UPW; ++u) src[u] += u < UA ? (int64_t)kGemmBK : step_b;
    }
  };

  const int fi = lane & 15, fk = lane >> 4;
  const int fblk = (lane >> 2) & 3, fj = lane & 3;
  auto frag_row = [&](int a, int i) __attribute__((always_inline)) { return wm * (16 * AF) + a * 16 + i; };
  auto frag_col = [&](int r, int blk, int j) __attribute__((always_inline)) {
    return wn * (4 * NB) + 8 * ((blk + (r >> 1)) & (NB / 2 - 1)) + 2 * j + (r & 1);
  };
  int a_off[KS], b_off[NB];
#pragma unroll
  for (int kk = 0; kk < KS; ++kk) {
    const int k = 4 * kk + fk;
    const int row = wm * (16 * AF) + fi;
    a_off[kk] = row * kGemmBK + 2 * ((k >> 1) ^ ((row >> 1) & 7)) + (k & 1);
  }
#pragma unroll
  for (int r = 0; r < NB; ++r) b_off[r] = fk * BN + frag_col(r, fblk, fj);

  double fa[2][AF], fb[2][NB];
  auto load_frags = [&](int st, int kk, int set) __attribute__((always_inline)) {
    const double* as = As + st * kATile;
    const double* bs = Bs + st * kBTile;
#pragma unroll
    for (int a = 0; a < AF; ++a) fa[set][a] = as[a_off[kk] + a * (16 * kGemmBK)];
#pragma unroll
    for (int r = 0; r < NB; r += 2) {
      const d2v v = *reinterpret_cast<const d2v*>(bs + b_off[r] + 4 * kk * BN);
      fb[set][r] = v.x, fb[set][r + 1] = v.y;
    }
  };
  auto mfma_step = [&](int set) __attribute__((always_inline)) {
#pragma unroll
    for (int a = 0; a < AF; ++a)
#pragma unroll
      for (int r = 0; r < NB; ++r)
        acc[a][r] = __builtin_amdgcn_mfma_f64_4x4x4f64(fa[set][a], fb[set][r], acc[a][r], 0, 0, 0);
  };
  constexpr int kReads = AF / 2 + NB / 2, kMfma = AF * NB, kPer = kMfma / kReads;
  auto interleave = [&]() __attribute__((always_inline)) {
#pragma unroll
    for (int i = 0; i < kReads; ++i) {
      __builtin_amdgcn_sched_group_barrier(0x100, 1, 0);
      __builtin_amdgcn_sched_group_barrier(0x008, kPer, 0);
    }
    __builtin_amdgcn_sched_group_barrier(0x008, kMfma - kPer * kReads, 0);
  };
  auto wait_vm = [&](auto n) __attribute__((always_inline)) {
    constexpr int N = decltype(n)::value;
    __builtin_amdgcn_s_waitcnt((N & 15) | (7 << 4) | (15 << 8) | ((N >> 4) << 14));
  };

  auto store_tile = [&](int m0) __attribute__((always_inline)) {
#pragma unroll
    for (int a = 0; a < AF; ++a)
#pragma unroll
      for (int r = 0; r < NB; r += 2) {
        const int row = m0 + frag_row(a, 4 * fblk + fk);
        const int col = n0 + frag_col(r, fblk, fj);
        if constexpr (EpiPairs<Epi>::value) {
          if (row < g.M && col + 1 < g.N) {
            epi.pair(0, row, col, acc[a][r], acc[a][r + 1]);
            continue;
          }
        }
#pragma unroll
        for (int q = 0; q < 2; ++q)
          if (row < g.M && col + q < g.N) epi(0, row, col + q, acc[a][r + q]);
      }
  };

  issue(0);
  if (kAhead == 2) {
    if (1 < cnt) advance_to(1);
    issue(1);
  }
  wait_vm(std::integral_constant<int, UPW*(kAhead - 1)>());
  __asm__ volatile("" ::: "memory");
  __builtin_amdgcn_s_barrier();
  __asm__ volatile("" ::: "memory");
  if (0 < cnt) load_frags(0, 0, 0);
  int st = 0;
  for (int s = 0; s < H; ++s) {
    const int st1 = st == kStages - 1 ? 0 : st + 1;
    const int st_new = kAhead == 2 ? (st1 == kStages - 1 ? 0 : st1 + 1) : st1;
    const bool switching = sw > 0 && s == sw;
    if (switching) {
      store_tile(m0_l);
#pragma unroll
      for (int i = 0; i < AF; ++i)
#pragma unroll
        for (int j = 0; j < NB; ++j) acc[i][j] = 0.0;
      __asm__ volatile("" ::: "memory");
    }
    if (s + kAhead < cnt) advance_to(s + kAhead);
    issue(st_new);
    const bool on = s < cnt;
    if (on) {
#pragma unroll
      for (int kk = 0; kk < KS - 1; ++kk) {
        load_frags(st, kk + 1, (kk + 1) & 1);
        mfma_step(kk & 1);
        interleave();
      }
    }
    if (switching) wait_vm(std::integral_constant<int, 0>());
    else wait_vm(std::integral_constant<int, UPW*(kAhead - 1)>());
    __builtin_amdgcn_s_waitcnt(0xC07F);
    __asm__ volatile("" ::: "memory");
    __builtin_amdgcn_s_barrier();
    __asm__ volatile("" ::: "memory");
    if (on) {
      load_frags(st1, 0, KS & 1);
      mfma_step((KS - 1) & 1);
      interleave();
    }
    st = st1;
  }
  __builtin_amdgcn_s_waitcnt(0);
  __builtin_amdgcn_s_barrier();
  __asm__ volatile("" ::: "memory");
  static_assert(4 * AF * NB * 64 <= kTeamLds, "the hand-off buffer fits a team's stages");
  double* xch = gemm_lds + kTeamLds + wave * (AF * NB * 64) + lane;
  if (team == 1) {
#pragma unroll
    for (int a = 0; a < AF; ++a)
#pragma unroll
      for (int r = 0; r < NB; ++r) xch[(a * NB + r) * 64] = acc[a][r];
  }
  __syncthreads();
  if (team == 0) {
#pragma unroll
    for (int a = 0; a < AF; ++a)
#pragma unroll
      for (int r = 0; r < NB; ++r) acc[a][r] = acc[a][r] + xch[(a * NB + r) * 64];
    store_tile(m0_h);
  }
}

template <int AF, int NB, int STAGES>
constexpr size_t gemm_f64_dma_team_pair_lds() {
  return (size_t)2 * STAGES * (32 * AF * kGemmBK + kGemmBK * 8 * NB) * sizeof(double);
}

}
```

Before: 6466.

## Fuse fold C-GEMM, column sums and scalar tail into one ticketed kernel

Adds a single fold kernel whose blocks split a lower-triangular GEMM tile grid (two-team K-split with an LDS hand-off), diagonal triangle blocks, and column-sum blocks. The packed-gradient epilogue is computed directly in the tile. A last-block ticket atomic then runs the scalar ELBO tail inside the same launch. This aims to remove separate launches and intermediate passes for the gradient fold and the final reduction. In exchange it relies on atomics and fences for cross-block visibility and adds more code paths and LDS pressure.

```diff
diff --git a/include/viabel_hip.h b/include/viabel_hip.h
--- a/include/viabel_hip.h
+++ b/include/viabel_hip.h
@@ -242,6 +242,7 @@
 int vb_fullrank_get(vb_ctx* ctx, double* value, double* grad, int64_t p);
 int vb_fullrank_fold_get_m(vb_ctx* ctx, double* M_host, int64_t d);
 int vb_fold_m_team_plan(int d, int pair, int* out8);
+int vb_fold_c_block_map(int t, int x, int* out3);
 
 int vb_elbo_grad_mvt_chol(vb_ctx* ctx, int slot, int64_t n, int64_t d, int64_t n_total, double df, const double* theta,
                           double* value, double* grad);
diff --git a/viabel_amd/csrc/vb_common.h b/viabel_amd/csrc/vb_common.h
--- a/viabel_amd/csrc/vb_common.h
+++ b/viabel_amd/csrc/vb_common.h
@@ -213,6 +213,7 @@
   vb::DeviceBuffer scratch2;
   vb::DeviceBuffer rowvec;
   vb::DeviceBuffer fr_work;
+  vb::DeviceBuffer fr_ticket;
   vb::DeviceBuffer lg_work;
   hipModule_t user_module = nullptr;
   hipFunction_t user_fn = nullptr;
diff --git a/viabel_amd/csrc/vb_fullrank.hip b/viabel_amd/csrc/vb_fullrank.hip
--- a/viabel_amd/csrc/vb_fullrank.hip
+++ b/viabel_amd/csrc/vb_fullrank.hip
@@ -462,40 +462,71 @@
 #undef VB_FOLD_MSUM_PARAMS
 #undef VB_FOLD_MSUM_SUM_ARGS
 
-template <int U>
+__device__ __forceinline__ void fr_store_wt(double* p, double v) {
+  __hip_atomic_store((fz_gu64*)p, __builtin_bit_cast(unsigned long long, v), __ATOMIC_RELAXED, __HIP_MEMORY_SCOPE_AGENT);
+}
+
+struct FoldColsumOut {
+  double* grad = nullptr;
+  double* sums = nullptr;
+  double invN = 0.0;
+  __device__ void operator()(int col, double c) const {
+    double s = 0.0;
+    s += c;
+    if (grad) grad[col] = -s * invN;
+    else sums[col] = s;
+  }
+};
+
+template <int U, int THREADS = 256, bool WT = false>
 __device__ __forceinline__ void fr_fold_csg_blocks(const int blk, fr_d2 (*part)[4], const double* __restrict__ colpart,
                                                    int gsplits, int64_t ldz, int d, const double* __restrict__ M,
-                                                   const double* __restrict__ b, double n_rows, double* __restrict__ csg) {
+                                                   const double* __restrict__ b, double n_rows, double* __restrict__ csg,
+                                                   const FoldColsumOut* fin = nullptr) {
+  static_assert(THREADS == 256 || THREADS == 512, "256 workers, with or without a second idle half");
+  const bool worker = THREADS == 256 || threadIdx.x < 256;
   const int p = threadIdx.x & 3, kg = threadIdx.x >> 2;
   const int col = blk * 8 + 2 * p;
-  const int colc = col < d ? col : 0;
-  const int kper = (d + 63) / 64;
-  const int k0 = kg * kper, k1 = k0 + kper < d ? k0 + kper : d;
-  fr_d2 acc = (fr_d2){0.0, 0.0};
-  for (int kb = k0; kb < k1; kb += U) {
-    fr_d2 v[U];
-    double c[U];
-#pragma unroll
-    for (int u = 0; u < U; ++u) {
-      const int k = kb + u < k1 ? kb + u : k1 - 1;
-      v[u] = *reinterpret_cast<const fr_d2*>(M + (int64_t)k * ldz + colc);
-      c[u] = colpart[k];
-    }
-    for (int z = 1; z < gsplits; ++z)
-#pragma unroll
-      for (int u = 0; u < U; ++u) c[u] += colpart[(int64_t)z * ldz + (kb + u < k1 ? kb + u : k1 - 1)];
-#pragma unroll
-    for (int u = 0; u < U; ++u)
-      if (kb + u < k1) acc += v[u] * c[u];
-  }
-  part[kg][p] = acc;
+  if (worker) {
+    const int colc = col < d ? col : 0;
+    const int kper = (d + 63) / 64;
+    const int k0 = kg * kper, k1 = k0 + kper < d ? k0 + kper : d;
+    fr_d2 acc = (fr_d2){0.0, 0.0};
+    for (int kb = k0; kb < k1; kb += U) {
+      fr_d2 v[U];
+      double c[U];
+#pragma unroll
+      for (int u = 0; u < U; ++u) {
+        const int k = kb + u < k1 ? kb + u : k1 - 1;
+        v[u] = *reinterpret_cast<const fr_d2*>(M + (int64_t)k * ldz + colc);
+        c[u] = colpart[k];
+      }
+      for (int z = 1; z < gsplits; ++z)
+#pragma unroll
+        for (int u = 0; u < U; ++u) c[u] += colpart[(int64_t)z * ldz + (kb + u < k1 ? kb + u : k1 - 1)];
+#pragma unroll
+      for (int u = 0; u < U; ++u)
+        if (kb + u < k1) acc += v[u] * c[u];
+    }
+    part[kg][p] = acc;
+  }
   __syncthreads();
-  if (kg == 0) {
+  if (worker && kg == 0) {
     fr_d2 tot = part[0][p];
 #pragma unroll 16
     for (int q = 1; q < 64; ++q) tot += part[q][p];
-    if (col < d) csg[col] = -tot.x - n_rows * b[col];
-    if (col + 1 < d) csg[col + 1] = -tot.y - n_rows * b[col + 1];
+    if (col < d) {
+      const double c = -tot.x - n_rows * b[col];
+      if (WT) fr_store_wt(csg + col, c);
+      else csg[col] = c;
+      if (fin) (*fin)(col, c);
+    }
+    if (col + 1 < d) {
+      const double c = -tot.y - n_rows * b[col + 1];
+      if (WT) fr_store_wt(csg + col + 1, c);
+      else csg[col + 1] = c;
+      if (fin) (*fin)(col + 1, c);
+    }
   }
 }
 
@@ -622,6 +653,84 @@
   else
     hipLaunchKernelGGL(fr_reduce_kernel<16>, grid, dim3(256), 0, st, Cpart, splits, slab, d, ldl, colpart, n_rb, ldz, fpart, n_fpart,
                        S, full, wpart, nb_c);
+}
+
+__device__ __forceinline__ void fr_packed_scalar_tail(const bool fuse, const int tx, const bool worker, double* sh3, int d,
+                                                      const double* __restrict__ colpart, int n_rb, int64_t ldz,
+                                                      const double* __restrict__ fpart, int n_fpart, FrSums S,
+                                                      const double* __restrict__ theta, double n_local_w, double n_total,
+                                                      double c0, double* __restrict__ out, int pd, const FrWeighted& wm,
+                                                      const double* __restrict__ fold_mu,
+                                                      const double* __restrict__ fold_mean) {
+  const bool weighted = wm.scale != 0.0;
+  const double invN = 1.0 / n_total;
+  if (worker) {
+    double f = 0.0, t = 0.0;
+    for (int e0 = 0; e0 < n_fpart; e0 += 4 * 256) {
+      double v[4];
+#pragma unroll
+      for (int u = 0; u < 4; ++u) {
+        const int e = e0 + u * 256 + tx;
+        v[u] = e < n_fpart ? fpart[e] : 0.0;
+      }
+#pragma unroll
+      for (int u = 0; u < 4; ++u) f += v[u];
+    }
+    for (int c0 = 0; c0 < d; c0 += 4 * 256) {
+      double dg[4];
+#pragma unroll
+      for (int u = 0; u < 4; ++u) {
+        const int c = c0 + u * 256 + tx, cc = c < d ? c : 0;
+        dg[u] = fuse ? theta[d + (int64_t)cc * (cc + 1) / 2 + cc] : 0.0;
+      }
+#pragma unroll
+      for (int u = 0; u < 4; ++u)
+        if (c0 + u * 256 + tx < d) t += dg[u];
+    }
+    double dot = 0.0;
+    if (fold_mu) {
+      for (int c0 = 0; c0 < d; c0 += 4 * 256) {
+        double s[4] = {0.0, 0.0, 0.0, 0.0}, cc[4];
+#pragma unroll
+        for (int q = 0; q < 4; ++q) {
+          const int c = c0 + q * 256 + tx, cl = c < d ? c : d - 1;
+          cc[q] = c < d ? fold_mu[cl] - fold_mean[cl] : 0.0;
+        }
+        for (int rb0 = 0; rb0 < n_rb; rb0 += 8) {
+          double v[4][8];
+#pragma unroll
+          for (int q = 0; q < 4; ++q) {
+            const int c = c0 + q * 256 + tx, cl = c < d ? c : d - 1;
+#pragma unroll
+            for (int u = 0; u < 8; ++u) v[q][u] = colpart[(int64_t)(rb0 + u < n_rb ? rb0 + u : n_rb - 1) * ldz + cl];
+          }
+#pragma unroll
+          for (int q = 0; q < 4; ++q)
+#pragma unroll
+            for (int u = 0; u < 8; ++u)
+              if (rb0 + u < n_rb) s[q] += v[q][u];
+        }
+#pragma unroll
+        for (int q = 0; q < 4; ++q) dot += cc[q] * s[q];
+      }
+    }
+    f = fr_wave_sum(f), t = fr_wave_sum(t), dot = fr_wave_sum(dot);
+    if ((tx & 63) == 0) sh3[tx >> 6] = f, sh3[4 + (tx >> 6)] = t, sh3[8 + (tx >> 6)] = dot;
+  }
+  __syncthreads();
+  if (worker && tx == 0) {
+    double f = (sh3[0] + sh3[1]) + (sh3[2] + sh3[3]);
+    if (fold_mu) f = 0.5 * (f + ((sh3[8] + sh3[9]) + (sh3[10] + sh3[11])));
+    const double sum_logdiag = (sh3[4] + sh3[5]) + (sh3[6] + sh3[7]);
+    if (fuse) {
+      const double F = f + n_local_w * c0;
+      const double half_sq = pd ? 0.5 * S.sums[1] * invN : 0.5 * d;
+      const double H = half_sq + 0.5 * d * kLog2PiFr + sum_logdiag;
+      out[0] = weighted ? wm.value[0] : -(F * invN + H);
+    } else {
+      S.sums[0] = f;
+    }
+  }
 }
 
 template <bool FUSE>
@@ -693,73 +802,9 @@
     }
   }
   if (blockIdx.x == 0) {
-    const int tx = threadIdx.x;
-    double f = 0.0, t = 0.0;
-    for (int e0 = 0; e0 < n_fpart; e0 += 4 * 256) {
-      double v[4];
-#pragma unroll
-      for (int u = 0; u < 4; ++u) {
-        const int e = e0 + u * 256 + tx;
-        v[u] = e < n_fpart ? fpart[e] : 0.0;
-      }
-#pragma unroll
-      for (int u = 0; u < 4; ++u) f += v[u];
-    }
-    for (int c0 = 0; c0 < d; c0 += 4 * 256) {
-      double dg[4];
-#pragma unroll
-      for (int u = 0; u < 4; ++u) {
-        const int c = c0 + u * 256 + tx, cc = c < d ? c : 0;
-        dg[u] = FUSE ? theta[d + (int64_t)cc * (cc + 1) / 2 + cc] : 0.0;
-      }
-#pragma unroll
-      for (int u = 0; u < 4; ++u)
-        if (c0 + u * 256 + tx < d) t += dg[u];
-    }
-    double dot = 0.0;
-    if (fold_mu) {
-      for (int c0 = 0; c0 < d; c0 += 4 * 256) {
-        double s[4] = {0.0, 0.0, 0.0, 0.0}, cc[4];
-#pragma unroll
-        for (int q = 0; q < 4; ++q) {
-          const int c = c0 + q * 256 + tx, cl = c < d ? c : d - 1;
-          cc[q] = c < d ? fold_mu[cl] - fold_mean[cl] : 0.0;
-        }
-        for (int rb0 = 0; rb0 < n_rb; rb0 += 8) {
-          double v[4][8];
-#pragma unroll
-          for (int q = 0; q < 4; ++q) {
-            const int c = c0 + q * 256 + tx, cl = c < d ? c : d - 1;
-#pragma unroll
-            for (int u = 0; u < 8; ++u) v[q][u] = colpart[(int64_t)(rb0 + u < n_rb ? rb0 + u : n_rb - 1) * ldz + cl];
-          }
-#pragma unroll
-          for (int q = 0; q < 4; ++q)
-#pragma unroll
-            for (int u = 0; u < 8; ++u)
-              if (rb0 + u < n_rb) s[q] += v[q][u];
-        }
-#pragma unroll
-        for (int q = 0; q < 4; ++q) dot += cc[q] * s[q];
-      }
-    }
     __shared__ double sh3[12];
-    f = fr_wave_sum(f), t = fr_wave_sum(t), dot = fr_wave_sum(dot);
-    if ((tx & 63) == 0) sh3[tx >> 6] = f, sh3[4 + (tx >> 6)] = t, sh3[8 + (tx >> 6)] = dot;
-    __syncthreads();
-    if (tx == 0) {
-      f = (sh3[0] + sh3[1]) + (sh3[2] + sh3[3]);
-      if (fold_mu) f = 0.5 * (f + ((sh3[8] + sh3[9]) + (sh3[10] + sh3[11])));
-      const double sum_logdiag = (sh3[4] + sh3[5]) + (sh3[6] + sh3[7]);
-      if (FUSE) {
-        const double F = f + n_local_w * c0;
-        const double half_sq = pd ? 0.5 * S.sums[1] * invN : 0.5 * d;
-        const double H = half_sq + 0.5 * d * kLog2PiFr + sum_logdiag;
-        out[0] = weighted ? wm.value[0] : -(F * invN + H);
-      } else {
-        S.sums[0] = f;
-      }
-    }
+    fr_packed_scalar_tail(FUSE, (int)threadIdx.x, true, sh3, d, colpart, n_rb, ldz, fpart, n_fpart, S, theta, n_local_w, n_total,
+                          c0, out, pd, wm, fold_mu, fold_mean);
   }
 }
 
@@ -798,6 +843,158 @@
       out[0] = wm.scale != 0.0 ? wm.value[0] : -(F * invN + H);
     }
   }
+}
+
+__host__ __device__ inline void fr_cunsplit_tile(int x, int* r, int* j) {
+  int q = 0;
+  while ((q + 1) * (q + 1) <= x) ++q;
+  *r = q;
+  *j = x - q * q;
+}
+
+struct EpiFoldPackedF {
+  const double* b;
+  const double* s;
+  const double* Lt;
+  int64_t ldl;
+  const double* theta;
+  double* grad;
+  double* sums;
+  int d;
+  double invN, ent;
+  __device__ double operator()(int, int row, int col, double acc) const {
+    if (col > row) return 0.0;
+    const double v = -acc - b[row] * s[col];
+    const int64_t p = (int64_t)row * (row + 1) / 2 + col;
+    if (grad) {
+      double g0 = -v * invN;
+      if (col == row) g0 = g0 * exp(theta[d + p]) - ent;
+      grad[p] = g0;
+    } else {
+      sums[p] = v;
+    }
+    return Lt[(int64_t)col * ldl + row] * v;
+  }
+  __device__ d2v pair(int z, int row, int col, double a0, double a1) const {
+    return (d2v){(*this)(z, row, col, a0), (*this)(z, row, col + 1, a1)};
+  }
+};
+
+__device__ __forceinline__ void fr_fold_block_part(double local, double* lds, double* dst) {
+#pragma unroll
+  for (int off = 32; off > 0; off >>= 1) local += __shfl_down(local, off, 64);
+  __syncthreads();
+  if (threadIdx.x < 256 && (threadIdx.x & 63) == 0) lds[threadIdx.x >> 6] = local;
+  __syncthreads();
+  if (threadIdx.x == 0) fr_store_wt(dst, (lds[0] + lds[1]) + (lds[2] + lds[3]));
+}
+
+__device__ __forceinline__ double fr_fold_ctri_block(const int q, double* lds, const double* __restrict__ M, int64_t ldm,
+                                                     const double* __restrict__ Sg, int64_t lds_g, int d,
+                                                     const EpiFoldPackedF& epi) {
+  constexpr int KC = 64;
+  const int t = (int)threadIdx.x;
+  const bool worker = t < 256;
+  const int c0 = 64 * q + 32;
+  fr_d2* Ms = reinterpret_cast<fr_d2*>(lds);
+  fr_d2* Ss = Ms + KC * 16;
+  const int ry = (t >> 4) & 15, cx = t & 15;
+  const bool active = worker && cx <= ry;
+  fr_d2 vm[4], vs[4];
+  auto fetch = [&](int k0) __attribute__((always_inline)) {
+#pragma unroll
+    for (int u = 0; u < 4; ++u) {
+      const int idx = (t & 255) + 256 * u, kr = idx >> 4, c = idx & 15;
+      vm[u] = *reinterpret_cast<const fr_d2*>(M + (int64_t)(k0 + kr) * ldm + c0 + 2 * c);
+      vs[u] = *reinterpret_cast<const fr_d2*>(Sg + (int64_t)(k0 + kr) * lds_g + c0 + 2 * c);
+    }
+  };
+  double a00 = 0.0, a01 = 0.0, a10 = 0.0, a11 = 0.0;
+  if (worker) fetch(0);
+  for (int k0 = 0; k0 < d; k0 += KC) {
+    __syncthreads();
+    if (worker) {
+#pragma unroll
+      for (int u = 0; u < 4; ++u) Ms[t + 256 * u] = vm[u], Ss[t + 256 * u] = vs[u];
+    }
+    __syncthreads();
+    if (worker && k0 + KC < d) fetch(k0 + KC);
+    if (active) {
+#pragma unroll 8
+      for (int k = 0; k < KC; ++k) {
+        const fr_d2 m = Ms[k * 16 + ry], s = Ss[k * 16 + cx];
+        a00 += m.x * s.x, a01 += m.x * s.y, a10 += m.y * s.x, a11 += m.y * s.y;
+      }
+    }
+  }
+  double local = 0.0;
+  if (active) {
+    const int row = c0 + 2 * ry, col = c0 + 2 * cx;
+    local += epi(0, row, col, a00);
+    local += epi(0, row, col + 1, a01);
+    local += epi(0, row + 1, col, a10);
+    local += epi(0, row + 1, col + 1, a11);
+  }
+  return local;
+}
+
+struct FoldCunsplitNoDep : GemmNoDep {};
+
+struct FoldTail {
+  double* fpart;
+  int n_fpart;
+  FrSums S;
+  const double* theta;
+  double n_local_w, n_total, c0;
+  double* out;
+  const double *mu, *mean;
+  unsigned* ticket;
+};
+
+__global__ void __launch_bounds__(512) fr_fold_cunsplit_kernel(const GemmArgs g, const EpiFoldPackedF epi, int T,
+                                                               const double* __restrict__ colpart, int gsplits, int64_t ldz,
+                                                               int d, const double* __restrict__ M,
+                                                               const double* __restrict__ b, double n_rows,
+                                                               double* __restrict__ csg, const FoldColsumOut fin,
+                                                               const FoldTail tl) {
+  extern __shared__ double fold_lds[];
+  __shared__ double sh3[12];
+  __shared__ unsigned last;
+  const int x = (int)blockIdx.x, nb_t = T * T;
+  if (x < nb_t) {
+    int r, j;
+    fr_cunsplit_tile(x, &r, &j);
+    const double local = gemm_f64_dma_team_split_tile<2, 4, kFoldTeamStages, EpiFoldPackedF, FoldCunsplitNoDep>(
+        g, epi, FoldCunsplitNoDep{}, 64 * r, 32 * j);
+    fr_fold_block_part(local, fold_lds, tl.fpart + x);
+  } else if (x < nb_t + T) {
+    const double local = fr_fold_ctri_block(x - nb_t, fold_lds, M, ldz, g.B, g.ldb, d, epi);
+    fr_fold_block_part(local, fold_lds, tl.fpart + x);
+  } else {
+    fr_fold_csg_blocks<8, 512, true>(x - nb_t - T, reinterpret_cast<fr_d2(*)[4]>(fold_lds), colpart, gsplits, ldz, d, M, b, n_rows,
+                               csg, &fin);
+  }
+  asm volatile("s_waitcnt vmcnt(0)" ::: "memory");
+  __syncthreads();
+  if (threadIdx.x == 0) {
+#ifdef VB_FOLD_TICKET_WBL2
+    __builtin_amdgcn_fence(__ATOMIC_RELEASE, "agent");
+    asm volatile("s_waitcnt vmcnt(0)" ::: "memory");
+#endif
+    const unsigned tk = __hip_atomic_fetch_add(tl.ticket, 1u, __ATOMIC_RELAXED, __HIP_MEMORY_SCOPE_AGENT);
+    last = tk == gridDim.x - 1 ? 1u : 0u;
+    if (tk == gridDim.x - 1) {
+      __hip_atomic_store(tl.ticket, 0u, __ATOMIC_RELAXED, __HIP_MEMORY_SCOPE_AGENT);
+      __builtin_amdgcn_fence(__ATOMIC_ACQUIRE, "agent");
+      asm volatile("s_waitcnt vmcnt(0)" ::: "memory");
+    }
+  }
+  __syncthreads();
+  if (!last) return;
+  FrWeighted wm;
+  wm.roww = nullptr, wm.scale = 0.0, wm.wsum = wm.value = nullptr;
+  fr_packed_scalar_tail(tl.out != nullptr, (int)threadIdx.x, threadIdx.x < 256, sh3, d, csg, 1, ldz, tl.fpart, tl.n_fpart, tl.S,
+                        tl.theta, tl.n_local_w, tl.n_total, tl.c0, tl.out, 0, wm, tl.mu, tl.mean);
 }
 
 __global__ void __launch_bounds__(256) fr_rowscale_kernel(double* __restrict__ G, int64_t ldz, int64_t n, int d,
@@ -1304,6 +1501,7 @@
   bool fold = false;
   int csplits = 1;
   int cfgc = 0;
+  bool c_unsplit = false;
   int fz_mode = 0;
   FrDense dense = kDenseChain;
   bool model_ksplit = false;
@@ -1407,6 +1605,8 @@
     const GemmArgs sc = gemm_product(nullptr, 0, nullptr, 0, D, D, D, 2);
     if (gemm_count_blocks(sc, 64, 64) * r.csplits <= 4L * n_cu) r.cfgc = 4;
     else r.cfgc = gemm_count_blocks(sc, 128, 64) * r.csplits * 100 >= 190L * n_cu ? 2 : 3;
+    const int T = D / 64;
+    r.c_unsplit = D % 64 == 0 && T * T <= n_cu && wm.scale == 0.0;
   }
   return r;
 }
@@ -1421,6 +1621,12 @@
   double *Sg = nullptr, *svec = nullptr, *csg = nullptr;
   double *Xa = nullptr, *T = nullptr, *sq = nullptr;
   FrSums S;
+};
+
+struct FrOut {
+  const double* theta;
+  double* out;
+  int64_t n_total;
 };
 
 static int fr_carve(vb_ctx* ctx, const FrRoute& r, const NoiseSlot& ns, int set, FrBufs* out) {
@@ -1562,7 +1768,7 @@
   return glm_grad_enqueue(ctx, st, m, b.Rm, r.ldr, Z, b.G, r.ldz, r.n, r.D);
 }
 
-static int fr_grad_folded(vb_ctx* ctx, const FrRoute& r, const FrBufs& b, const ModelDev& m, unsigned* tiles3) {
+static int fr_grad_folded(vb_ctx* ctx, const FrRoute& r, const FrBufs& b, const ModelDev& m, const FrOut& o, unsigned* tiles3) {
   hipStream_t st = ctx->stream;
   const int D = r.D;
   const double* M = b.Mf;
@@ -1599,6 +1805,31 @@
                        m.p0, nb_cs, nb_s, b.Sg, b.svec, b.bvec);
   VB_HIP(ctx, hipGetLastError());
   GemmArgs gc = gemm_product(M, r.ldz, b.Sg, r.ldl, D, D, D, 2);
+  if (r.c_unsplit) {
+    const int T = D / 64, nb = T * T + T + nb_cs;
+    VB_TRY(ensure(ctx, ctx->fr_ticket, 64));
+    static_assert(team_lds >= 2 * 64 * 32 * sizeof(double) && team_lds >= 64 * 4 * sizeof(fr_d2),
+                  "the triangles' and the colsum(G) blocks' LDS is the tiles'");
+    static bool configured_u = false;
+    if (!configured_u) {
+      (void)hipFuncSetAttribute(reinterpret_cast<const void*>(&fr_fold_cunsplit_kernel), hipFuncAttributeMaxDynamicSharedMemorySize,
+                                (int)team_lds);
+      configured_u = true;
+    }
+    const bool fuse = !ctx->comm;
+    const double invN = 1.0 / (double)o.n_total;
+    const EpiFoldPackedF eu{b.bvec, b.svec, b.Lt, r.ldl, o.theta, fuse ? o.out + 1 + D : nullptr, b.S.sums + b.S.off_c, D, invN,
+                            1.0};
+    FoldColsumOut fin;
+    fin.grad = fuse ? o.out + 1 : nullptr, fin.sums = b.S.sums + b.S.off_col, fin.invN = invN;
+    const FoldTail tl{b.fpart, T * T + T, b.S, o.theta, (double)o.n_total, (double)o.n_total, m.c0, fuse ? o.out : nullptr,
+                      b.mu, m.p0, (unsigned*)ctx->fr_ticket.ptr};
+    hipLaunchKernelGGL(fr_fold_cunsplit_kernel, dim3((unsigned)nb), dim3(512), team_lds, st, gc, eu, T, (const double*)b.colpart,
+                       r.splits, r.ldz, D, M, (const double*)b.bvec, (double)r.n, b.csg, fin, tl);
+    VB_HIP(ctx, hipGetLastError());
+    *tiles3 = (unsigned)(T * T + T);
+    return VB_OK;
+  }
   const EpiFoldSlabF ec{b.Cpart, r.ldl, r.slab, b.bvec, b.svec, b.Lt, r.ldl, b.fpart};
   if (r.cfgc == 4) {
     const int gx = (int)gemm_f64_tri2_small_plan(&gc, r.csplits, r.n_cu), nb_tiles = gx * r.csplits;
@@ -1687,11 +1918,11 @@
   return VB_OK;
 }
 
-static int fr_grad_product(vb_ctx* ctx, const FrRoute& r, const FrBufs& b, const ModelDev& m, const double* G,
+static int fr_grad_product(vb_ctx* ctx, const FrRoute& r, const FrBufs& b, const ModelDev& m, const double* G, const FrOut& o,
                            unsigned* tiles3) {
   hipStream_t st = ctx->stream;
   *tiles3 = 0;
-  if (r.fold) return fr_grad_folded(ctx, r, b, m, tiles3);
+  if (r.fold) return fr_grad_folded(ctx, r, b, m, o, tiles3);
   if (!r.grad_launch) return VB_OK;
   GemmArgs g3 = gemm_product(G, r.ldz, b.E, b.lde, r.D, r.D, (int)r.n, r.tri3);
   prof_events(ctx, &g3.ev0, &g3.ev1, 1, VB_PROF_FR_GRAD_GEMM);
@@ -1723,16 +1954,19 @@
   const dim3 red_grid((unsigned)((red_items + 255) / 256) + (r.fold ? 1u : 0u));
   const double *fold_mu = r.fold ? (const double*)b.mu : nullptr, *fold_m = r.fold ? m.p0 : nullptr;
   if (!ctx->comm) {
+    if (r.c_unsplit) return VB_OK;
     hipLaunchKernelGGL(fr_reduce_packed_kernel<true>, red_grid, dim3(256), 0, st, (const double*)b.Cpart, splits, r.slab, D,
                        r.ldl, colpart, n_rb_red, r.ldz, (const double*)b.fpart, n_fpart_red, b.S, theta_dev,
                        (double)n_total, (double)n_total, m.c0, out_dev, r.pd ? 1 : 0, wm, fold_mu, fold_m);
     VB_HIP(ctx, hipGetLastError());
     return VB_OK;
   }
-  hipLaunchKernelGGL(fr_reduce_packed_kernel<false>, red_grid, dim3(256), 0, st, (const double*)b.Cpart, splits, r.slab, D,
-                     r.ldl, colpart, n_rb_red, r.ldz, (const double*)b.fpart, n_fpart_red, b.S, theta_dev,
-                     (double)n_total, (double)n_total, m.c0, out_dev, r.pd ? 1 : 0, wm, fold_mu, fold_m);
-  VB_HIP(ctx, hipGetLastError());
+  if (!r.c_unsplit) {
+    hipLaunchKernelGGL(fr_reduce_packed_kernel<false>, red_grid, dim3(256), 0, st, (const double*)b.Cpart, splits, r.slab, D,
+                       r.ldl, colpart, n_rb_red, r.ldz, (const double*)b.fpart, n_fpart_red, b.S, theta_dev,
+                       (double)n_total, (double)n_total, m.c0, out_dev, r.pd ? 1 : 0, wm, fold_mu, fold_m);
+    VB_HIP(ctx, hipGetLastError());
+  }
   Pipeline& P = ctx->pipe;
   hipStream_t st_post = st;
   if (r.overlap) {
@@ -1814,7 +2048,7 @@
     VB_TRY(fr_colpass(ctx, r, b, m, G, Z, r.two_passes ? 0 : r.fmode, r.colpass_keeps_f ? b.fpart : b.fpart + r.n_fpart,
                       row_scale));
   else if (row_scale) VB_TRY(fr_rowscale(ctx, r, G, row_scale));
-  VB_TRY(fr_grad_product(ctx, r, b, m, G, &tiles3));
+  VB_TRY(fr_grad_product(ctx, r, b, m, G, FrOut{theta_dev, out_dev, n_total}, &tiles3));
 
   if (mvt) return fr_finish_mvt(ctx, r, b, sums_out);
   const int n_fpart_red = r.fold ? (int)tiles3 * r.csplits : r.f_per_tile ? (int)tiles2 : r.n_fpart;
@@ -1876,3 +2110,15 @@
   for (int i = 0; i < 8; ++i) out8[i] = out[i];
   return VB_OK;
 }
+
+int vb_fold_c_block_map(int t, int x, int* out3) {
+  using namespace vb;
+  if (!out3 || t < 1 || t > 32768 || x < 0 || (int64_t)x >= (int64_t)t * t + t) return VB_ERR_INVALID;
+  if (x < t * t) {
+    out3[0] = 0;
+    fr_cunsplit_tile(x, &out3[1], &out3[2]);
+  } else {
+    out3[0] = 1, out3[1] = x - t * t, out3[2] = 2 * (x - t * t) + 1;
+  }
+  return VB_OK;
+}
diff --git a/viabel_amd/csrc/vb_gemm_f64_dma.h b/viabel_amd/csrc/vb_gemm_f64_dma.h
--- a/viabel_amd/csrc/vb_gemm_f64_dma.h
+++ b/viabel_amd/csrc/vb_gemm_f64_dma.h
@@ -707,4 +707,206 @@
   return (size_t)2 * STAGES * (32 * AF * kGemmBK + kGemmBK * 8 * NB) * sizeof(double);
 }
 
+template <int AF, int NB, int STAGES, class Epi, class Dep>
+__device__ __forceinline__ double gemm_f64_dma_team_split_tile(const GemmArgs& g, const Epi& epi, const Dep&, const int m0,
+                                                               const int n0) {
+  static_assert(STAGES == 2 || STAGES == 3, "two or three LDS stages per team");
+  static_assert(AF % 2 == 0 && NB % 2 == 0, "fragments are read in pairs");
+  constexpr int BM = 32 * AF, BN = 8 * NB;
+  constexpr int kStages = STAGES, kAhead = STAGES - 1;
+  constexpr int kATile = BM * kGemmBK, kBTile = kGemmBK * BN;
+  constexpr int kAUnits = kATile / 128, kBUnits = kBTile / 128;
+  static_assert(kAUnits % 4 == 0 && kBUnits % 4 == 0, "whole rounds of A and of B units over the 4 waves of a team");
+  constexpr int UA = kAUnits / 4, UPW = (kAUnits + kBUnits) / 4;
+  constexpr int kTeamLds = kStages * (kATile + kBTile);
+  constexpr int KS = kGemmBK / 4;
+  extern __shared__ double gemm_lds[];
+  const int t = threadIdx.x & 255;
+  const int lane = t & 63, wave = __builtin_amdgcn_readfirstlane(t >> 6);
+  const int team = __builtin_amdgcn_readfirstlane((int)threadIdx.x >> 8);
+  double* lds = gemm_lds + team * kTeamLds;
+  double* As = lds;
+  double* Bs = lds + kStages * kATile;
+  const int wm = wave >> 1, wn = wave & 1;
+
+  const int nslabs = g.K / kGemmBK;
+  const int H = (nslabs + 1) / 2;
+  if (H <= 0) return 0.0;
+  const int first = team * H;
+  const int last = first + H < nslabs ? first + H : nslabs;
+  const int cnt = last > first ? last - first : 0;
+  const int ks0 = cnt > 0 ? first : nslabs - 1;
+
+  double acc[AF][NB];
+#pragma unroll
+  for (int i = 0; i < AF; ++i)
+#pragma unroll
+    for (int j = 0; j < NB; ++j) acc[i][j] = 0.0;
+
+  const double* src[UPW];
+  const int64_t step_a = (int64_t)kGemmBK * g.lda, step_b = (int64_t)kGemmBK * g.ldb;
+#pragma unroll
+  for (int u = 0; u < UPW; ++u) {
+    if (u < UA) {
+      const int q = u * 4 + wave;
+      constexpr int PPR = BM / 2, RPU = 64 / PPR > 0 ? 64 / PPR : 1;
+      constexpr int UPR = PPR >= 64 ? PPR / 64 : 1;
+      const int krow = (PPR >= 64) ? q / UPR : q * RPU + lane / PPR;
+      const int p = (PPR >= 64) ? (q % UPR) * 64 + lane : lane % PPR;
+      int64_t col = m0 + 2 * p;
+      col = col < g.lda - 1 ? col : g.lda - 2;
+      src[u] = g.A + ((int64_t)ks0 * kGemmBK + krow) * g.lda + col;
+    } else {
+      const int qb = (u - UA) * 4 + wave;
+      constexpr int PPR = BN / 2, RPU = 64 / PPR > 0 ? 64 / PPR : 1;
+      constexpr int UPR = PPR >= 64 ? PPR / 64 : 1;
+      const int krow = (PPR >= 64) ? qb / UPR : qb * RPU + lane / PPR;
+      const int p = (PPR >= 64) ? (qb % UPR) * 64 + lane : lane % PPR;
+      int64_t col = n0 + 2 * p;
+      col = col < g.ldb - 1 ? col : g.ldb - 2;
+      src[u] = g.B + ((int64_t)ks0 * kGemmBK + krow) * g.ldb + col;
+    }
+  }
+  auto issue = [&](int st) __attribute__((always_inline)) {
+#pragma unroll
+    for (int u = 0; u < UPW; ++u) {
+      if (u < UA) {
+        double* dst = lds + (u * 4 + wave) * 128 + st * kATile;
+        __builtin_amdgcn_global_load_lds((gemm_gptr)src[u], (gemm_lptr)dst, 16, 0, Dep::kAuxA);
+      } else {
+        double* dst = lds + kStages * kATile + ((u - UA) * 4 + wave) * 128 + st * kBTile;
+        __builtin_amdgcn_global_load_lds((gemm_gptr)src[u], (gemm_lptr)dst, 16, 0, 0);
+      }
+    }
+  };
+  auto advance = [&]() __attribute__((always_inline)) {
+#pragma unroll
+    for (int u = 0; u < UPW; ++u) src[u] += u < UA ? step_a : step_b;
+  };
+
+  const int fi = lane & 15, fk = lane >> 4;
+  const int fblk = (lane >> 2) & 3, fj = lane & 3;
+  auto frag_row = [&](int a, int i) __attribute__((always_inline)) {
+    return wm * (16 * AF) + 32 * (a >> 1) + 2 * i + (a & 1);
+  };
+  auto frag_col = [&](int r, int blk, int j) __attribute__((always_inline)) {
+    return wn * (4 * NB) + 8 * ((blk + (r >> 1)) & (NB / 2 - 1)) + 2 * j + (r & 1);
+  };
+  int a_off[AF], b_off[NB];
+#pragma unroll
+  for (int a = 0; a < AF; ++a) a_off[a] = fk * BM + frag_row(a, fi);
+#pragma unroll
+  for (int r = 0; r < NB; ++r) b_off[r] = fk * BN + frag_col(r, fblk, fj);
+
+  double fa[2][AF], fb[2][NB];
+  auto load_frags = [&](int st, int kk, int set) __attribute__((always_inline)) {
+    const double* as = As + st * kATile;
+    const double* bs = Bs + st * kBTile;
+#pragma unroll
+    for (int a = 0; a < AF; a += 2) {
+      const d2v v = *reinterpret_cast<const d2v*>(as + a_off[a] + 4 * kk * BM);
+      fa[set][a] = v.x, fa[set][a + 1] = v.y;
+    }
+#pragma unroll
+    for (int r = 0; r < NB; r += 2) {
+      const d2v v = *reinterpret_cast<const d2v*>(bs + b_off[r] + 4 * kk * BN);
+      fb[set][r] = v.x, fb[set][r + 1] = v.y;
+    }
+  };
+  auto mfma_step = [&](int set) __attribute__((always_inline)) {
+#pragma unroll
+    for (int a = 0; a < AF; ++a)
+#pragma unroll
+      for (int r = 0; r < NB; ++r)
+        acc[a][r] = __builtin_amdgcn_mfma_f64_4x4x4f64(fa[set][a], fb[set][r], acc[a][r], 0, 0, 0);
+  };
+  constexpr int kReads = AF / 2 + NB / 2, kMfma = AF * NB, kPer = kMfma / kReads;
+  auto interleave = [&]() __attribute__((always_inline)) {
+#pragma unroll
+    for (int i = 0; i < kReads; ++i) {
+      __builtin_amdgcn_sched_group_barrier(0x100, 1, 0);
+      __builtin_amdgcn_sched_group_barrier(0x008, kPer, 0);
+    }
+    __builtin_amdgcn_sched_group_barrier(0x008, kMfma - kPer * kReads, 0);
+  };
+  auto wait_vm = [&](auto n) __attribute__((always_inline)) {
+    constexpr int N = decltype(n)::value;
+    __builtin_amdgcn_s_waitcnt((N & 15) | (7 << 4) | (15 << 8) | ((N >> 4) << 14));
+  };
+
+  issue(0);
+  if (kAhead == 2) {
+    if (1 < cnt) advance();
+    issue(1);
+  }
+  wait_vm(std::integral_constant<int, UPW*(kAhead - 1)>());
+  __asm__ volatile("" ::: "memory");
+  __builtin_amdgcn_s_barrier();
+  __asm__ volatile("" ::: "memory");
+  if (0 < cnt) load_frags(0, 0, 0);
+  int st = 0;
+  for (int s = 0; s < H; ++s) {
+    const int st1 = st == kStages - 1 ? 0 : st + 1;
+    const int st_new = kAhead == 2 ? (st1 == kStages - 1 ? 0 : st1 + 1) : st1;
+    if (s + kAhead < cnt) advance();
+    issue(st_new);
+    const bool on = s < cnt;
+    if (on) {
+#pragma unroll
+      for (int kk = 0; kk < KS - 1; ++kk) {
+        load_frags(st, kk + 1, (kk + 1) & 1);
+        mfma_step(kk & 1);
+        interleave();
+      }
+    }
+    wait_vm(std::integral_constant<int, UPW*(kAhead - 1)>());
+    __builtin_amdgcn_s_waitcnt(0xC07F);
+    __asm__ volatile("" ::: "memory");
+    __builtin_amdgcn_s_barrier();
+    __asm__ volatile("" ::: "memory");
+    if (on) {
+      load_frags(st1, 0, KS & 1);
+      mfma_step((KS - 1) & 1);
+      interleave();
+    }
+    st = st1;
+  }
+  __builtin_amdgcn_s_waitcnt(0);
+  __builtin_amdgcn_s_barrier();
+  __asm__ volatile("" ::: "memory");
+  static_assert(4 * AF * NB * 64 <= kTeamLds, "the hand-off buffer fits a team's stages");
+  double* xch = gemm_lds + kTeamLds + wave * (AF * NB * 64) + lane;
+  if (team == 1) {
+#pragma unroll
+    for (int a = 0; a < AF; ++a)
+#pragma unroll
+      for (int r = 0; r < NB; ++r) xch[(a * NB + r) * 64] = acc[a][r];
+  }
+  __syncthreads();
+  double local = 0.0;
+  if (team == 0) {
+#pragma unroll
+    for (int a = 0; a < AF; ++a)
+#pragma unroll
+      for (int r = 0; r < NB; ++r) acc[a][r] = acc[a][r] + xch[(a * NB + r) * 64];
+#pragma unroll
+    for (int a = 0; a < AF; ++a)
+#pragma unroll
+      for (int r = 0; r < NB; r += 2) {
+        const int row = m0 + frag_row(a, 4 * fblk + fk);
+        const int col = n0 + frag_col(r, fblk, fj);
+        if (row < g.M && col + 1 < g.N) {
+          const d2v v = epi.pair(0, row, col, acc[a][r], acc[a][r + 1]);
+          local += v.x;
+          local += v.y;
+          continue;
+        }
+#pragma unroll
+        for (int q = 0; q < 2; ++q)
+          if (row < g.M && col + q < g.N) local += epi(0, row, col + q, acc[a][r + q]);
+      }
+  }
+  return local;
 }
+
+}
```

Measured after the change: 2937. 0.454x the previous value.
